# davnords/octic-vits

Measured on AMD Instinct MI355X. Metric: images/sec Hybrid Octic ViT-H/14 224² bf16 train step @1/2/4/8 MI355X, higher is better.
Workload: dtype bf16; 1 GPU; hybrid_deit_huge_patch14 (16 octic + 16 standard blocks, drop_path 0.5) DeiT-III train step: bf16-autocast fwd + bwd + LAMB + EMA, 224x224, batch 64/GPU (BASELINE configs[1]), data parallel over 1 GPU(s); global_batch=64, per_gpu_batch=64, accum_steps=1, parallelism=dp1, library_gemm_table=True, launch=hipGraph replay (whole step)

## Files before the change

include/octic_hip.h:

```cpp
#ifndef OCTIC_HIP_H
#define OCTIC_HIP_H

#include <stdint.h>

#ifdef __cplusplus
extern "C" {
#endif

#define OCTIC_ABI_VERSION 20

enum { OCTIC_F32 = 0, OCTIC_BF16 = 1, OCTIC_U8 = 2  };

enum {
  OCTIC_OK = 0,
  OCTIC_ESHAPE = -1,
  OCTIC_EALIGN = -2,
  OCTIC_EDTYPE = -3,
  OCTIC_ENULL = -4,
  OCTIC_EWORKSPACE = -5
};

typedef struct {
  void* ptr[5];
  int64_t ld[5];
} octic_view;

int octic_abi_version(void);
const char* octic_strerror(int code);

enum {
  OCTIC_ROUTE_DENSE_TILE = 0,
  OCTIC_ROUTE_DENSE_SPLIT = 1,
  OCTIC_ROUTE_WGRAD_SLABS = 2,
  OCTIC_ROUTE_WGRAD_TILE = 3,
  OCTIC_ROUTE_LINEAR_RING = 4,
  OCTIC_ROUTE_RING_EVEN = 5,
  OCTIC_ROUTE_ATTN_LEGACY = 6,
  OCTIC_ROUTE_ATTN_ONLINE = 7,
  OCTIC_ROUTE_ATTN_BWD_PAIR = 8,
  OCTIC_ROUTE_DENSE_IMAGE = 9,
  OCTIC_ROUTE_DENSE_CLS2 = 10,
  OCTIC_ROUTE_ATTN_STREAM = 11,
  OCTIC_ROUTE_COUNT = 12
};
int octic_route_override(int knob, int value);

int octic_gelu_d8_fwd(const octic_view* x, const octic_view* y, int64_t M, int c, int dtype, void* stream);
int octic_gelu_d8_bwd(const octic_view* g, const octic_view* x, const octic_view* gin, int64_t M, int c,
                      int dtype, void* stream);
int octic_gelu_d8_fwd_skip(const octic_view* x, const octic_view* y, int64_t M, int c, int dtype,
                           const float* sample_scale, int64_t rows_per_sample, void* stream);
int octic_gelu_d8_bwd_skip(const octic_view* g, const octic_view* x, const octic_view* gin, int64_t M, int c, int dtype,
                           const float* sample_scale, int64_t rows_per_sample, void* stream);

int octic_layernorm_d8_fwd(const octic_view* x, const octic_view* y, const float* const alpha[5],
                           const float* beta, float* stats, int64_t M, int c, float eps, int out_dtype,
                           void* stream);
int octic_layernorm_d8_bwd_blocks(int64_t M);
int octic_layernorm_d8_bwd(const octic_view* g, const octic_view* x, const float* stats,
                           const float* const alpha[5], const octic_view* dres, const octic_view* dx,
                           float* partials, int64_t M, int c, int g_dtype, void* stream);
int octic_layernorm_d8_bwd_cast(const octic_view* g, const octic_view* x, const float* stats, const float* const alpha[5],
                                const octic_view* dres, const octic_view* dx, float* partials, int64_t M, int c,
                                const float* rs, int64_t rows_per_sample, void* gcast, void* stream);
int octic_layernorm_d8_bwd_skip(const octic_view* g, const octic_view* x, const float* stats, const float* const alpha[5],
                                const octic_view* dres, const octic_view* dx, float* partials, int64_t M, int c, int g_dtype,
                                const float* sample_scale, int64_t rows_per_sample, void* stream);
int octic_layernorm_d8_bwd_cast_skip(const octic_view* g, const octic_view* x, const float* stats,
                                     const float* const alpha[5], const octic_view* dres, const octic_view* dx,
                                     float* partials, int64_t M, int c, const float* rs, int64_t rows_per_scale, void* gcast,
                                     const float* sample_scale, int64_t rows_per_sample, void* stream);
int octic_layernorm_d8_bwd_finish(const float* partials, int nblk, int c, float* const dalpha[5], float* dbeta,
                                  void* stream);
typedef struct octic_ln_finish_job {
  const float* partials;
  float* dalpha[5];
  float* dbeta;
  int nblk;
  int c;
} octic_ln_finish_job;
int octic_layernorm_d8_bwd_finish_batch(const octic_ln_finish_job* jobs, int njobs, void* stream);

int octic_sample_blocks(const void* src, void* dst, const int64_t* idx, int64_t n, int64_t block_bytes, int scatter,
                        void* stream);

int octic_linear_d8_fwd(const octic_view* x, const void* const w[5], const float* bias, const octic_view* y,
                        const octic_view* resid, const float* rs, int64_t rows_per_sample,
                        const float* const cs[5], int64_t M, int cin, int cout, int dtype, int out_dtype,
                        void* stream);
int octic_linear_d8_fwd_skip(const octic_view* x, const void* const w[5], const float* bias, const octic_view* y,
                             const octic_view* resid, const float* rs, int64_t rows_per_sample,
                             const float* const cs[5], int64_t M, int cin, int cout, int dtype, int out_dtype,
                             const float* sample_scale, int64_t skip_rows_per_sample, void* stream);
int octic_linear_d8_fwd_dropped(const octic_view* x, const void* const w[5], const float* bias, const octic_view* y,
                                const octic_view* resid, const float* rs, int64_t rows_per_sample,
                                const float* const cs[5], int64_t M, int cin, int cout, int dtype, int out_dtype,
                                const float* dropped, int64_t dropped_rows_per_sample, void* stream);

int octic_linear_d8_prep(const float* const w32[5], const float* const cs[5], int cin, int cout, void* wb, void* wt,
                         int dtype, void* stream);
typedef struct octic_prep_item {
  const float* w[5];
  const float* cs[5];
  void* wb;
  void* wt;
  int32_t cin, cout;
  int32_t block_begin, block_count;
} octic_prep_item;
int octic_linear_d8_prep_batch_blocks(int cin, int cout);
int octic_linear_d8_prep_batch(const octic_prep_item* items_dev, int n_items, int total_blocks, int dtype, void* stream);

int octic_linear_d8_tile_n(int64_t M, int cin, int cout);
enum {
  OCTIC_LINEAR_WREG = 0,
  OCTIC_LINEAR_RING = 1,
  OCTIC_LINEAR_CLASSIC = 2
};
int octic_linear_d8_plan(int64_t M, int cin, int cout, int dtype, int out_dtype, int fused, int out[4]);
int octic_linear_d8_ring_order(int ngroups, const int* items, const int* ksteps, int slots_per_xcd, int* out_group,
                               int* out_item);
int octic_linear_d8_ring_order_dropped(int ngroups, const int* items, const int* ksteps, int slots_per_xcd, const int* n_chunks,
                                       const unsigned char* dead_long, const unsigned char* dead_short, int* out_group,
                                       int* out_item, int* out_dead);

int octic_linear_d8_wgrad_has_colsum(int cin, int cout, int dtype);
enum {
  OCTIC_WGRAD_RING = 0,
  OCTIC_WGRAD_TILED = 1
};
int octic_linear_d8_wgrad_plan(int64_t M, int cin, int cout, int dtype, int out[4]);
int64_t octic_linear_d8_wgrad_workspace_bytes(int cin, int cout, int splits);
int octic_linear_d8_wgrad_splits(int64_t M, int cin, int cout);
int octic_linear_d8_wgrad_tile(int64_t M, int cin, int cout);
int octic_linear_d8_wgrad(const octic_view* x, const octic_view* dy, int64_t M, int cin, int cout, int dtype,
                          float* workspace, int splits, void* stream);
int octic_linear_d8_wgrad_finish(const float* workspace, int splits, int cin, int cout,
                                 const float* const w32[5], const float* const cs[5], const float* bias,
                                 const float* dysum, float* const dw[5], float* const dcs[5], float* dbias,
                                 void* stream);
typedef struct octic_wgrad_finish_job {
  const float* workspace;
  const float* w32[5];
  const float* cs[5];
  const float* bias;
  const float* dysum;
  float* dw[5];
  float* dcs[5];
  float* dbias;
  int splits, cin, cout, has_cs;
} octic_wgrad_finish_job;
int octic_linear_d8_wgrad_finish_batch(const octic_wgrad_finish_job* jobs, int njobs, void* stream);

int octic_colsum_blocks(int64_t M);
int octic_colsum_a1(const octic_view* dy, int64_t M, int c, int dtype, float* partials, float* out, void* stream);
// ... 17 lines not shown
int octic_attn_fwd_f32(const void* q, const void* k, const void* v, void* o, float* lse, int64_t B, int H, int T, int hd,
                       int64_t sB, int64_t sH, int64_t sT, int64_t oB, int64_t oH, int64_t oT, float scale, void* stream);
int octic_attn_bwd_f32(const void* q, const void* k, const void* v, const void* o, const void* dout, const float* lse,
                       float* delta, void* dq, void* dk, void* dv, int64_t B, int H, int T, int hd, int64_t sB, int64_t sH,
                       int64_t sT, int64_t oB, int64_t oH, int64_t oT, int64_t gB, int64_t gH, int64_t gT, float scale,
                       int phase, void* stream);

int octic_attn_fwd_packed(const void* qkv, void* o, float* lse, int64_t B, int H, int T, int c, int64_t ld_qkv,
                          int64_t ld_o, float scale, void* stream);
int octic_attn_bwd_packed(const void* qkv, const void* o, const void* dout, const float* lse, float* delta, void* dqkv,
                          int64_t B, int H, int T, int c, int64_t ld_qkv, int64_t ld_o, int64_t ld_g, float scale,
                          int phase, void* stream);

enum {
  OCTIC_ATTN_FWD_PERSIST = 0,
  OCTIC_ATTN_FWD_A80_ONESHOT = 1,
  OCTIC_ATTN_FWD_A80_ONLINE = 2,
  OCTIC_ATTN_FWD_RESIDENT = 3,
  OCTIC_ATTN_FWD_STREAM = 4,
  OCTIC_ATTN_FWD_F32 = 5
};
enum {
  OCTIC_ATTN_BWD_SINGLE = 0,
  OCTIC_ATTN_BWD_PAIR = 1,
  OCTIC_ATTN_BWD_STREAM = 2,
  OCTIC_ATTN_BWD_F32 = 3
};
int octic_attn_plan(int dtype, int T, int hd, int64_t ld_in, int64_t ld_out, int64_t ld_grad, int out[4]);
int octic_attn_skip_plan(int dtype, int T, int hd, int64_t ld_in, int64_t ld_out, int64_t ld_grad, int out[4]);

int octic_attn_fwd_skip(const void* q, const void* k, const void* v, void* o, float* lse, int64_t B, int H, int T, int hd,
                        int64_t sB, int64_t sH, int64_t sT, int64_t oB, int64_t oH, int64_t oT, float scale,
                        const float* sample_scale, void* stream);
int octic_attn_bwd_skip(const void* q, const void* k, const void* v, const void* o, const void* dout, const float* lse,
                        float* delta, void* dq, void* dk, void* dv, int64_t B, int H, int T, int hd, int64_t sB, int64_t sH,
                        int64_t sT, int64_t oB, int64_t oH, int64_t oT, int64_t gB, int64_t gH, int64_t gT, float scale,
                        int phase, const float* sample_scale, void* stream);
int octic_attn_fwd_packed_skip(const void* qkv, void* o, float* lse, int64_t B, int H, int T, int c, int64_t ld_qkv,
                               int64_t ld_o, float scale, const float* sample_scale, void* stream);
int octic_attn_bwd_packed_skip(const void* qkv, const void* o, const void* dout, const float* lse, float* delta, void* dqkv,
                               int64_t B, int H, int T, int c, int64_t ld_qkv, int64_t ld_o, int64_t ld_g, float scale,
                               int phase, const float* sample_scale, void* stream);

int octic_handoff_cat_fwd(const octic_view* x, void* dense, int64_t M, int c, int out_dtype, void* stream);
int octic_handoff_cat_bwd(const float* ddense, const octic_view* dx, int64_t M, int c, void* stream);
int octic_power_spectrum_fwd(const octic_view* x, void* dense, int64_t M, int c, int out_dtype, void* stream);
int octic_power_spectrum_bwd(const float* ddense, const octic_view* x, const octic_view* dx, int64_t M, int c,
                             void* stream);

int octic_im2col_patches(const float* img, void* patches, int64_t B, int Cin, int Himg, int Wimg, int p,
                         int Kpad, int dtype, void* stream);
int octic_lift_gemm(const void* patches, const void* w, const float* bias, const float* pos, float* out,
                    int64_t B, int64_t n_patches, int tok0, int Kpad, int D, int dtype, void* stream);
int64_t octic_lift_wgrad_workspace_bytes(int Kpad, int D, int splits);
int octic_lift_wgrad(const void* patches, const void* dout, float* dw, float* workspace, int splits, int64_t rows,
                     int Kpad, int D, int dtype, void* stream);

int64_t octic_lamb_workspace_floats(int ntensors, int nchunks);
int octic_lamb_step(void* const* p, void* const* g, void* const* m, void* const* v, void* const* ema, const float* wd,
                    const int* chunk_tensor, const int64_t* chunk_off, const int* chunk_len,
                    const int* tensor_chunk_begin, int ntensors, int nchunks, float* workspace, float lr, float beta1,
                    float beta2, float eps, float max_grad_norm, int step, float ema_decay, void* const* bf16_shadow,
                    void* stream);
int octic_adamw_step(void* const* p, void* const* g, void* const* m, void* const* v, void* const* ema, const float* wd,
                     const int* chunk_tensor, const int64_t* chunk_off, const int* chunk_len,
                     const int* tensor_chunk_begin, int ntensors, int nchunks, float* workspace, float lr, float beta1,
                     float beta2, float eps, float max_grad_norm, int step, float ema_decay, void* const* bf16_shadow,
                     void* stream);
int octic_lamb_step_hp(void* const* p, void* const* g, void* const* m, void* const* v, void* const* ema, const float* wd,
                       const int* chunk_tensor, const int64_t* chunk_off, const int* chunk_len,
                       const int* tensor_chunk_begin, int ntensors, int nchunks, float* workspace, const float* lr,
                       float beta1, float beta2, float eps, float max_grad_norm, int step, const float* ema_decay,
                       void* const* bf16_shadow, void* stream);
int octic_adamw_step_hp(void* const* p, void* const* g, void* const* m, void* const* v, void* const* ema, const float* wd,
                        const int* chunk_tensor, const int64_t* chunk_off, const int* chunk_len,
                        const int* tensor_chunk_begin, int ntensors, int nchunks, float* workspace, const float* lr,
                        float beta1, float beta2, float eps, float max_grad_norm, int step, const float* ema_decay,
                        void* const* bf16_shadow, void* stream);

int octic_dense_blocks(int64_t rows);
int octic_dense_resid_layernorm_fwd(const float* x, const void* yb, int yb_dtype, const float* gamma, const float* rs,
                                    int64_t rows_per_scale, float* xout, void* y, int y_dtype, const float* w,
                                    const float* b, float* stats, int64_t rows, int d, float eps, void* stream);
int octic_dense_layernorm_fwd(const float* x, void* y, int y_dtype, const float* w, const float* b, float* stats,
                              int64_t rows, int d, float eps, void* stream);
int octic_dense_layernorm_bwd(const void* gy, int g_dtype, const float* x, const float* w, const float* stats,
                              const float* dres, float* dx, float* partials, int64_t rows, int d, void* stream);
int octic_dense_finish(const float* partials, int nblocks, int d, float* out0, float* out1, const float* scale1,
                       void* stream);
typedef struct octic_finish_job {
  const float* partials;
  float* out0;
  float* out1;
  const float* scale1;
  int nblocks;
  int d;
} octic_finish_job;
int octic_dense_finish_batch(const octic_finish_job* jobs, int njobs, void* stream);
int octic_dense_layernorm_bwd_tail(const void* gy, const float* x, const float* w, const float* stats, const float* dres,
                                   float* dx, float* partials, const void* yb, const float* gamma, const float* rs,
                                   int64_t rows_per_scale, void* gyb, float* partials2, int64_t rows, int d, void* stream);
int octic_dense_layernorm_bwd_tail_skip(const void* gy, const float* x, const float* w, const float* stats,
                                        const float* dres, float* dx, float* partials, const void* yb, const float* gamma,
                                        const float* rs, int64_t rows_per_scale, void* gyb, float* partials2, int64_t rows,
                                        int d, const float* sample_scale, int64_t rows_per_sample, void* stream);
int octic_dense_gelu_blocks(void);
int octic_dense_gelu_bwd(const void* h, const void* g, void* dh, float* partials, int64_t rows, int d, void* stream);
int octic_dense_colsum(const void* g, int64_t rows, int d, int64_t ld, float* partials, void* stream);
int octic_dense_colsum_skip(const void* g, int64_t rows, int d, int64_t ld, float* partials, const float* sample_scale,
                            int64_t rows_per_sample, void* stream);
int octic_swiglu_blocks(void);
int octic_swiglu_fwd(const void* x12, int64_t ld12, void* a, int64_t lda, int64_t rows, int H, void* stream);
int octic_swiglu_bwd(const void* x12, int64_t ld12, const void* ga, int64_t ldg, void* dx12, int64_t ldd, float* partials,
                     int64_t rows, int H, void* stream);
int octic_scale_residual_fwd(const float* x, const void* y, int y_dtype, const float* gamma, const float* rs,
                             int64_t rows_per_scale, float* out, int64_t rows, int d, void* stream);
int octic_scale_residual_bwd(const float* gout, const void* y, int y_dtype, const float* gamma, const float* rs,
                             int64_t rows_per_scale, void* gy, float* partials, int64_t rows, int d, void* stream);

int octic_dense_layernorm_fwd_rows(const float* x, void* y, int y_dtype, const float* w, const float* b, float* stats,
                                   int64_t rows, int d, float eps, const int* rowmap, float* xcopy, void* stream);
int octic_dense_layernorm_bwd_rows(const void* gy, int g_dtype, const float* x, const float* w, const float* stats,
                                   const float* dres, float* dx, float* partials, int64_t rows, int d, const int* rowmap,
                                   void* stream);
int octic_scale_residual_fwd_rows(const float* x, const void* y, int y_dtype, const float* gamma, const float* rs,
                                  int64_t rows_per_scale, float* out, int64_t rows, int d, const int* rowmap, void* stream);
int octic_scale_residual_bwd_rows(const float* gout, const void* y, int y_dtype, const float* gamma, const float* rs,
                                  int64_t rows_per_scale, void* gy, float* partials, int64_t rows, int d, const int* rowmap,
                                  void* stream);

typedef struct octic_dense_prep_item {
  const void* src;
  void* wb;
  void* wt;
  int32_t N, K;
  int32_t block_begin, pad;
} octic_dense_prep_item;
int octic_dense_prep_batch_blocks(int N, int K);
int octic_dense_prep_batch(const octic_dense_prep_item* items_dev, int n_items, int total_blocks, int src_dtype, void* stream);

int64_t octic_dense_gemm_workspace_bytes(int M, int N, int K);
int octic_dense_gemm_colsum_rows(int M, int N, int K);
int octic_dense_gemm_tile(int M, int N, int K, int mode);
int octic_dense_gemm_nt(const void* A, const void* B, int M, int N, int K, int64_t lda, int64_t ldb, int mode, void* C,
                        void* C2, int64_t ldc, const float* bias, const float* gamma, const float* rs,
                        int64_t rows_per_sample, const float* X, float* OUT, const void* H, float* colsum,
                        void* workspace, void* stream);
int octic_dense_gemm_nt_tokens(const void* A, const void* B, int M, int N, int K, int64_t lda, int64_t ldb, int mode, void* C,
                               void* C2, int64_t ldc, const float* bias, const float* gamma, const float* rs,
                               int64_t rows_per_sample, const float* X, float* OUT, const void* H, float* colsum,
                               void* workspace, int tokens, void* stream);
int octic_dense_gemm_plan(int M, int N, int K, int mode, int tokens, int* out4);
int octic_dense_gemm_nt_tokens_skip(const void* A, const void* B, int M, int N, int K, int64_t lda, int64_t ldb, int mode, void* C,
                                    void* C2, int64_t ldc, const float* bias, const float* gamma, const float* rs,
                                    int64_t rows_per_sample_rs, const float* X, float* OUT, const void* H, float* colsum,
                                    const float* sample_scale, int rows_per_sample, void* workspace, int tokens,
                                    void* stream);
int octic_dense_gemm_plan_dropped(int M, int N, int K, int mode, int tokens, int rows_per_sample, int* out4);
int octic_dense_gemm_order_dropped(int M, int N, int K, int mode, int tokens, const float* sample_scale, int rows_per_sample,
                                   int cap, int* out_tm, int* out_tn, int* out_part, int* out_split, int* out_dead);
int octic_dense_gemm_nt_tokens_adaptive(const void* A, const void* B, int M, int N, int K, int64_t lda, int64_t ldb, int mode,
                                        void* C, void* C2, int64_t ldc, const float* bias, const float* gamma, const float* rs,
                                        int64_t rows_per_sample_rs, const float* X, float* OUT, const void* H, float* colsum,
                                        const float* sample_scale, int rows_per_sample, void* workspace, int tokens,
                                        void* stream);
int octic_dense_gemm_plan_adaptive(int M, int N, int K, int mode, int tokens, int rows_per_sample, int* out5);
int octic_dense_gemm_order_adaptive(int M, int N, int K, int mode, int tokens, const float* sample_scale, int rows_per_sample,
                                    int cap, int* out_tm, int* out_tn, int* out_dead, int* out_width);
int octic_dense_gemm_nt_tokens_adaptive_cls(const void* A, const void* B, int M, int N, int K, int64_t lda, int64_t ldb, int mode,
                                            void* C, void* C2, int64_t ldc, const float* bias, const float* gamma, const float* rs,
                                            int64_t rows_per_sample_rs, const float* X, float* OUT, const void* H, float* colsum,
                                            const float* sample_scale, int rows_per_sample, void* workspace, int tokens,
                                            int fold_cls, void* stream);
int octic_dense_gemm_plan_adaptive_cls(int M, int N, int K, int mode, int tokens, int rows_per_sample, int* out5);
int octic_dense_gemm_order_adaptive_cls(int M, int N, int K, int mode, int tokens, const float* sample_scale, int rows_per_sample,
                                        int cap, int* out_tm, int* out_tn, int* out_dead, int* out_width, int cls_cap,
                                        int* out_cls_rt, int* out_cls_ct);

int octic_dense_gemm_nt_tokens_image(const void* A, const void* B, int M, int N, int K, int64_t lda, int64_t ldb, int mode,
                                     void* C, void* C2, int64_t ldc, const float* bias, const float* gamma, const float* rs,
                                     int64_t rows_per_sample_rs, const float* X, float* OUT, const void* H, float* colsum,
                                     const float* sample_scale, int rows_per_sample, void* workspace, int tokens,
                                     int fold_cls, double drop, void* stream);
int octic_dense_gemm_plan_image(int M, int N, int K, int mode, int tokens, int rows_per_sample, int masked, double drop, int* out8);
int octic_dense_gemm_order_image(int M, int N, int K, int mode, int tokens, const float* sample_scale, int rows_per_sample, double drop,
                                 int cap, int* out_tm, int* out_tn, int* out_dead, int cls_cap, int* out_cls_rt, int* out_cls_ct);

int64_t octic_dense_wgrad_workspace_bytes(int M, int N, int K);
// ... 190 lines not shown
```

octic_vits_amd/_lib.py:

```python
import ctypes
import os
import re

HERE = os.path.dirname(os.path.abspath(__file__))
LIB_PATH = os.environ.get("OCTIC_LIB") or os.path.join(HERE, "liboctic_hip.so")
HEADER_PATH = os.path.join(HERE, "..", "include", "octic_hip.h")

F32, BF16, U8 = 0, 1, 2
ABI_VERSION = 20
(ROUTE_DENSE_TILE, ROUTE_DENSE_SPLIT, ROUTE_WGRAD_SLABS, ROUTE_WGRAD_TILE, ROUTE_LINEAR_RING, ROUTE_RING_EVEN,
 ROUTE_ATTN_LEGACY, ROUTE_ATTN_ONLINE, ROUTE_ATTN_BWD_PAIR, ROUTE_DENSE_IMAGE, ROUTE_DENSE_CLS2, ROUTE_ATTN_STREAM) = range(12)

DENSE_ADAPT_WIDE, DENSE_ADAPT_NARROW = 16, 32
DENSE_IMAGE_ALWAYS, DENSE_IMAGE_CLS_APART, DENSE_IMAGE_NEVER = 4, 8, 16

(ATTN_FWD_PERSIST, ATTN_FWD_A80_ONESHOT, ATTN_FWD_A80_ONLINE, ATTN_FWD_RESIDENT, ATTN_FWD_STREAM, ATTN_FWD_F32) = range(6)
ATTN_BWD_SINGLE, ATTN_BWD_PAIR, ATTN_BWD_STREAM, ATTN_BWD_F32 = range(4)
LINEAR_WREG, LINEAR_RING, LINEAR_CLASSIC = range(3)
WGRAD_RING, WGRAD_TILED = range(2)
DENSE_F32_NT, DENSE_F32_NN, DENSE_F32_TN = range(3)

c_i64, c_int, c_float, c_void_p = ctypes.c_int64, ctypes.c_int, ctypes.c_float, ctypes.c_void_p
c_double = ctypes.c_double


class OcticView(ctypes.Structure):
    _fields_ = [("ptr", c_void_p * 5), ("ld", c_i64 * 5)]


PtrArray5 = c_void_p * 5
VP = ctypes.POINTER(OcticView)

_PROTOS = {
    "octic_abi_version": (c_int, []),
    "octic_strerror": (ctypes.c_char_p, [c_int]),
    "octic_route_override": (c_int, [c_int, c_int]),
    "octic_gelu_d8_fwd": (c_int, [VP, VP, c_i64, c_int, c_int, c_void_p]),
    "octic_gelu_d8_bwd": (c_int, [VP, VP, VP, c_i64, c_int, c_int, c_void_p]),
    "octic_gelu_d8_fwd_skip": (c_int, [VP, VP, c_i64, c_int, c_int, c_void_p, c_i64, c_void_p]),
    "octic_gelu_d8_bwd_skip": (c_int, [VP, VP, VP, c_i64, c_int, c_int, c_void_p, c_i64, c_void_p]),
    "octic_layernorm_d8_fwd": (c_int, [VP, VP, c_void_p, c_void_p, c_void_p, c_i64, c_int, c_float, c_int, c_void_p]),
    "octic_layernorm_d8_bwd_blocks": (c_int, [c_i64]),
    "octic_layernorm_d8_bwd": (c_int, [VP, VP, c_void_p, c_void_p, VP, VP, c_void_p, c_i64, c_int, c_int, c_void_p]),
    "octic_layernorm_d8_bwd_cast": (c_int, [VP, VP, c_void_p, c_void_p, VP, VP, c_void_p, c_i64, c_int, c_void_p, c_i64,
                                            c_void_p, c_void_p]),
    "octic_layernorm_d8_bwd_skip": (c_int, [VP, VP, c_void_p, c_void_p, VP, VP, c_void_p, c_i64, c_int, c_int, c_void_p, c_i64,
                                            c_void_p]),
    "octic_layernorm_d8_bwd_cast_skip": (c_int, [VP, VP, c_void_p, c_void_p, VP, VP, c_void_p, c_i64, c_int, c_void_p, c_i64,
                                                 c_void_p, c_void_p, c_i64, c_void_p]),
    "octic_layernorm_d8_bwd_finish": (c_int, [c_void_p, c_int, c_int, c_void_p, c_void_p, c_void_p]),
    "octic_layernorm_d8_bwd_finish_batch": (c_int, [c_void_p, c_int, c_void_p]),
    "octic_sample_blocks": (c_int, [c_void_p, c_void_p, c_void_p, c_i64, c_i64, c_int, c_void_p]),
    "octic_linear_d8_fwd": (c_int, [VP, c_void_p, c_void_p, VP, VP, c_void_p, c_i64, c_void_p, c_i64, c_int, c_int,
                                    c_int, c_int, c_void_p]),
    "octic_linear_d8_fwd_skip": (c_int, [VP, c_void_p, c_void_p, VP, VP, c_void_p, c_i64, c_void_p, c_i64, c_int, c_int,
                                         c_int, c_int, c_void_p, c_i64, c_void_p]),
    "octic_linear_d8_fwd_dropped": (c_int, [VP, c_void_p, c_void_p, VP, VP, c_void_p, c_i64, c_void_p, c_i64, c_int, c_int,
                                            c_int, c_int, c_void_p, c_i64, c_void_p]),
    "octic_linear_d8_tile_n": (c_int, [c_i64, c_int, c_int]),
    "octic_linear_d8_plan": (c_int, [c_i64, c_int, c_int, c_int, c_int, c_int, ctypes.POINTER(c_int)]),
    "octic_linear_d8_ring_order": (c_int, [c_void_p, c_void_p, c_void_p, c_int, c_void_p, c_void_p]),
    "octic_linear_d8_ring_order_dropped": (c_int, [c_int, c_void_p, c_void_p, c_int, c_void_p, c_void_p, c_void_p, c_void_p,
                                                   c_void_p, c_void_p]),
    "octic_linear_d8_wgrad_tile": (c_int, [c_i64, c_int, c_int]),
    "octic_linear_d8_wgrad_workspace_bytes": (c_i64, [c_int, c_int, c_int]),
    "octic_linear_d8_wgrad_splits": (c_int, [c_i64, c_int, c_int]),
    "octic_linear_d8_wgrad": (c_int, [VP, VP, c_i64, c_int, c_int, c_int, c_void_p, c_int, c_void_p]),
    "octic_linear_d8_wgrad_finish": (c_int, [c_void_p, c_int, c_int, c_int, c_void_p, c_void_p, c_void_p, c_void_p,
                                             c_void_p, c_void_p, c_void_p, c_void_p]),
    "octic_linear_d8_wgrad_finish_batch": (c_int, [c_void_p, c_int, c_void_p]),
    "octic_linear_d8_wgrad_has_colsum": (c_int, [c_int, c_int, c_int]),
    "octic_linear_d8_wgrad_plan": (c_int, [c_i64, c_int, c_int, c_int, ctypes.POINTER(c_int)]),
    "octic_lamb_workspace_floats": (c_i64, [c_int, c_int]),
    "octic_lamb_step": (c_int, [c_void_p] * 10 + [c_int, c_int, c_void_p, c_float, c_float, c_float, c_float, c_float,
                                                  c_int, c_float, c_void_p, c_void_p]),
    "octic_adamw_step": (c_int, [c_void_p] * 10 + [c_int, c_int, c_void_p, c_float, c_float, c_float, c_float, c_float,
                                                   c_int, c_float, c_void_p, c_void_p]),
    "octic_lamb_step_hp": (c_int, [c_void_p] * 10 + [c_int, c_int, c_void_p, c_void_p, c_float, c_float, c_float, c_float,
                                                     c_int, c_void_p, c_void_p, c_void_p]),
    "octic_adamw_step_hp": (c_int, [c_void_p] * 10 + [c_int, c_int, c_void_p, c_void_p, c_float, c_float, c_float, c_float,
                                                      c_int, c_void_p, c_void_p, c_void_p]),
    "octic_dense_blocks": (c_int, [c_i64]),
    "octic_dense_layernorm_fwd": (c_int, [c_void_p, c_void_p, c_int, c_void_p, c_void_p, c_void_p, c_i64, c_int,
                                          c_float, c_void_p]),
    "octic_dense_resid_layernorm_fwd": (c_int, [c_void_p, c_void_p, c_int, c_void_p, c_void_p, c_i64, c_void_p, c_void_p, c_int,
                                                c_void_p, c_void_p, c_void_p, c_i64, c_int, c_float, c_void_p]),
    "octic_dense_layernorm_bwd": (c_int, [c_void_p, c_int, c_void_p, c_void_p, c_void_p, c_void_p, c_void_p, c_void_p,
                                          c_i64, c_int, c_void_p]),
    "octic_dense_layernorm_bwd_tail": (c_int, [c_void_p] * 10 + [c_i64, c_void_p, c_void_p, c_i64, c_int, c_void_p]),
    "octic_dense_layernorm_bwd_tail_skip": (c_int, [c_void_p] * 10 + [c_i64, c_void_p, c_void_p, c_i64, c_int, c_void_p, c_i64,
                                                                      c_void_p]),
    "octic_dense_finish": (c_int, [c_void_p, c_int, c_int, c_void_p, c_void_p, c_void_p, c_void_p]),
    "octic_dense_finish_batch": (c_int, [c_void_p, c_int, c_void_p]),
    "octic_dense_gelu_blocks": (c_int, []),
    "octic_dense_gelu_bwd": (c_int, [c_void_p, c_void_p, c_void_p, c_void_p, c_i64, c_int, c_void_p]),
    "octic_swiglu_blocks": (c_int, []),
    "octic_swiglu_fwd": (c_int, [c_void_p, c_i64, c_void_p, c_i64, c_i64, c_int, c_void_p]),
    "octic_swiglu_bwd": (c_int, [c_void_p, c_i64, c_void_p, c_i64, c_void_p, c_i64, c_void_p, c_i64, c_int, c_void_p]),
    "octic_dense_layernorm_fwd_rows": (c_int, [c_void_p, c_void_p, c_int, c_void_p, c_void_p, c_void_p, c_i64, c_int, c_float,
                                               c_void_p, c_void_p, c_void_p]),
    "octic_dense_layernorm_bwd_rows": (c_int, [c_void_p, c_int, c_void_p, c_void_p, c_void_p, c_void_p, c_void_p, c_void_p, c_i64,
                                               c_int, c_void_p, c_void_p]),
    "octic_scale_residual_fwd_rows": (c_int, [c_void_p, c_void_p, c_int, c_void_p, c_void_p, c_i64, c_void_p, c_i64, c_int,
                                              c_void_p, c_void_p]),
    "octic_scale_residual_bwd_rows": (c_int, [c_void_p, c_void_p, c_int, c_void_p, c_void_p, c_i64, c_void_p, c_void_p, c_i64,
                                              c_int, c_void_p, c_void_p]),
    "octic_softmax_center": (c_int, [c_void_p, c_int, c_i64, c_void_p, c_float, c_void_p, c_i64, c_int, c_void_p]),
    "octic_soft_ce_fwd": (c_int, [c_void_p, c_int, c_i64, c_void_p, c_i64, c_float, c_void_p, c_void_p, c_void_p, c_i64, c_int,
                                  c_void_p]),
    "octic_soft_ce_bwd": (c_int, [c_void_p, c_int, c_i64, c_void_p, c_i64, c_float, c_void_p, c_void_p, c_void_p, c_void_p, c_i64,
                                  c_i64, c_int, c_void_p]),
    "octic_sinkhorn_slabs": (c_int, [c_i64]),
    "octic_sinkhorn_protos": (c_int, [c_void_p, c_int, c_i64, c_float, c_void_p, c_void_p, c_void_p, c_void_p, c_i64, c_int,
                                      c_void_p]),
    "octic_sinkhorn_rows": (c_int, [c_void_p, c_int, c_i64, c_float, c_void_p, c_void_p, c_void_p, c_i64, c_int, c_void_p]),
    "octic_sinkhorn_final": (c_int, [c_void_p, c_int, c_i64, c_float, c_void_p, c_void_p, c_i64, c_int, c_void_p]),
    "octic_scale_residual_fwd": (c_int, [c_void_p, c_void_p, c_int, c_void_p, c_void_p, c_i64, c_void_p, c_i64, c_int,
                                         c_void_p]),
    "octic_scale_residual_bwd": (c_int, [c_void_p, c_void_p, c_int, c_void_p, c_void_p, c_i64, c_void_p, c_void_p,
                                         c_i64, c_int, c_void_p]),
    "octic_colsum_blocks": (c_int, [c_i64]),
    "octic_colsum_a1": (c_int, [VP, c_i64, c_int, c_int, c_void_p, c_void_p, c_void_p]),
    "octic_cast_rowscale": (c_int, [VP, VP, c_void_p, c_i64, c_i64, c_int, c_int, c_void_p]),
    "octic_linear_d8_prep": (c_int, [c_void_p, c_void_p, c_int, c_int, c_void_p, c_void_p, c_int, c_void_p]),
    "octic_linear_d8_prep_batch_blocks": (c_int, [c_int, c_int]),
    "octic_linear_d8_prep_batch": (c_int, [c_void_p, c_int, c_int, c_int, c_void_p]),
    "octic_attn_fwd": (c_int, [c_void_p, c_void_p, c_void_p, c_void_p, c_void_p, c_i64, c_int, c_int, c_int,
                               c_i64, c_i64, c_i64, c_i64, c_i64, c_i64, c_float, c_void_p]),
    "octic_attn_fwd_packed": (c_int, [c_void_p] * 3 + [c_i64, c_int, c_int, c_int, c_i64, c_i64, c_float, c_void_p]),
    "octic_attn_bwd_packed": (c_int, [c_void_p] * 6 + [c_i64, c_int, c_int, c_int, c_i64, c_i64, c_i64, c_float, c_int, c_void_p]),
    "octic_attn_bwd": (c_int, [c_void_p] * 10 + [c_i64, c_int, c_int, c_int] + [c_i64] * 9 + [c_float, c_int, c_void_p]),
    "octic_attn_fwd_skip": (c_int, [c_void_p] * 5 + [c_i64, c_int, c_int, c_int] + [c_i64] * 6 + [c_float, c_void_p, c_void_p]),
    "octic_attn_bwd_skip": (c_int, [c_void_p] * 10 + [c_i64, c_int, c_int, c_int] + [c_i64] * 9 + [c_float, c_int, c_void_p, c_void_p]),
    "octic_attn_fwd_packed_skip": (c_int, [c_void_p] * 3 + [c_i64, c_int, c_int, c_int, c_i64, c_i64, c_float, c_void_p, c_void_p]),
    "octic_attn_bwd_packed_skip": (c_int, [c_void_p] * 6 + [c_i64, c_int, c_int, c_int, c_i64, c_i64, c_i64, c_float, c_int, c_void_p, c_void_p]),
    "octic_attn_fwd_f32": (c_int, [c_void_p] * 5 + [c_i64, c_int, c_int, c_int] + [c_i64] * 6 + [c_float, c_void_p]),
    "octic_attn_bwd_f32": (c_int, [c_void_p] * 10 + [c_i64, c_int, c_int, c_int] + [c_i64] * 9 + [c_float, c_int, c_void_p]),
    "octic_attn_plan": (c_int, [c_int, c_int, c_int, c_i64, c_i64, c_i64, ctypes.POINTER(c_int)]),
    "octic_attn_skip_plan": (c_int, [c_int, c_int, c_int, c_i64, c_i64, c_i64, ctypes.POINTER(c_int)]),
    "octic_attn_pack_heads": (c_int, [VP, c_void_p, c_i64, c_i64, c_int, c_int, c_int, c_int, c_void_p]),
    "octic_attn_unpack_heads": (c_int, [c_void_p, VP, c_i64, c_i64, c_int, c_int, c_int, c_int, c_void_p]),
    "octic_handoff_cat_fwd": (c_int, [VP, c_void_p, c_i64, c_int, c_int, c_void_p]),
    "octic_handoff_cat_bwd": (c_int, [c_void_p, VP, c_i64, c_int, c_void_p]),
    "octic_power_spectrum_fwd": (c_int, [VP, c_void_p, c_i64, c_int, c_int, c_void_p]),
    "octic_power_spectrum_bwd": (c_int, [c_void_p, VP, VP, c_i64, c_int, c_void_p]),
    "octic_im2col_patches": (c_int, [c_void_p, c_void_p, c_i64, c_int, c_int, c_int, c_int, c_int, c_int, c_void_p]),
    "octic_lift_gemm": (c_int, [c_void_p, c_void_p, c_void_p, c_void_p, c_void_p, c_i64, c_i64, c_int, c_int, c_int,
                                c_int, c_void_p]),
    "octic_lift_wgrad_workspace_bytes": (c_i64, [c_int, c_int, c_int]),
    "octic_lift_wgrad": (c_int, [c_void_p, c_void_p, c_void_p, c_void_p, c_int, c_i64, c_int, c_int, c_int, c_void_p]),
    "octic_dense_prep_batch_blocks": (c_int, [c_int, c_int]),
    "octic_dense_prep_batch": (c_int, [c_void_p, c_int, c_int, c_int, c_void_p]),
    "octic_dense_gemm_workspace_bytes": (c_i64, [c_int, c_int, c_int]),
    "octic_dense_gemm_colsum_rows": (c_int, [c_int, c_int, c_int]),
    "octic_dense_gemm_tile": (c_int, [c_int, c_int, c_int, c_int]),
    "octic_dense_gemm_nt": (c_int, [c_void_p, c_void_p, c_int, c_int, c_int, c_i64, c_i64, c_int, c_void_p, c_void_p, c_i64,
                                    c_void_p, c_void_p, c_void_p, c_i64, c_void_p, c_void_p, c_void_p, c_void_p, c_void_p,
                                    c_void_p]),
    "octic_dense_gemm_nt_tokens": (c_int, [c_void_p, c_void_p, c_int, c_int, c_int, c_i64, c_i64, c_int, c_void_p, c_void_p,
                                           c_i64, c_void_p, c_void_p, c_void_p, c_i64, c_void_p, c_void_p, c_void_p, c_void_p,
                                           c_void_p, c_int, c_void_p]),
    "octic_dense_gemm_plan": (c_int, [c_int, c_int, c_int, c_int, c_int, ctypes.POINTER(c_int)]),
    "octic_dense_gemm_nt_tokens_skip": (c_int, [c_void_p, c_void_p, c_int, c_int, c_int, c_i64, c_i64, c_int, c_void_p, c_void_p,
                                                c_i64, c_void_p, c_void_p, c_void_p, c_i64, c_void_p, c_void_p, c_void_p, c_void_p,
                                                c_void_p, c_int, c_void_p, c_int, c_void_p]),
    "octic_dense_gemm_plan_dropped": (c_int, [c_int, c_int, c_int, c_int, c_int, c_int, ctypes.POINTER(c_int)]),
    "octic_dense_gemm_order_dropped": (c_int, [c_int, c_int, c_int, c_int, c_int, c_void_p, c_int, c_int, c_void_p, c_void_p,
                                               c_void_p, c_void_p, c_void_p]),
    "octic_dense_gemm_nt_tokens_adaptive": (c_int, [c_void_p, c_void_p, c_int, c_int, c_int, c_i64, c_i64, c_int, c_void_p, c_void_p,
                                                    c_i64, c_void_p, c_void_p, c_void_p, c_i64, c_void_p, c_void_p, c_void_p,
                                                    c_void_p, c_void_p, c_int, c_void_p, c_int, c_void_p]),
    "octic_dense_gemm_plan_adaptive": (c_int, [c_int, c_int, c_int, c_int, c_int, c_int, ctypes.POINTER(c_int)]),
    "octic_dense_gemm_order_adaptive": (c_int, [c_int, c_int, c_int, c_int, c_int, c_void_p, c_int, c_int, c_void_p, c_void_p,
                                                c_void_p, c_void_p]),
# ... 168 lines not shown
```

octic_vits_amd/csrc/dense.hip:

```cpp
#include "octic_common.hpp"

namespace octic {

constexpr int kDenseWaves = 16;
constexpr int kDenseMaxBlocks = 256;

template <typename T> struct Row4;
template <> struct Row4<float> {
  typedef f32x4 vec;
  static __device__ inline f32x4 load(const float* p) { return *(const f32x4*)p; }
  static __device__ inline f32x4 load_raw(const float* p) { return *(const f32x4*)p; }
  static __device__ inline f32x4 widen(f32x4 v) { return v; }
  static __device__ inline void store(float* p, f32x4 v) { *(f32x4*)p = v; }
};
template <> struct Row4<bf16> {
  typedef bf16x4 vec;
  static __device__ inline f32x4 load(const bf16* p) {
    bf16x4 h = *(const bf16x4*)p;
    return f32x4{(float)h[0], (float)h[1], (float)h[2], (float)h[3]};
  }
  static __device__ inline bf16x4 load_raw(const bf16* p) { return *(const bf16x4*)p; }
  static __device__ inline f32x4 widen(bf16x4 h) { return f32x4{(float)h[0], (float)h[1], (float)h[2], (float)h[3]}; }
  static __device__ inline void store(bf16* p, f32x4 v) {
    *(bf16x4*)p = bf16x4{(bf16)v[0], (bf16)v[1], (bf16)v[2], (bf16)v[3]};
  }
};

__device__ inline float hsum(f32x4 v) { return (v[0] + v[1]) + (v[2] + v[3]); }

template <typename TOUT, int NV>
__global__ __launch_bounds__(256) void dense_ln_fwd_kernel(const float* __restrict__ x, TOUT* __restrict__ y,
                                                           const float* __restrict__ w, const float* __restrict__ b,
                                                           float* __restrict__ stats, long rows, int d, float eps,
                                                           const int* __restrict__ rowmap = nullptr,
                                                           float* __restrict__ xcopy = nullptr) {
  const int lane = threadIdx.x & 63;
  const long nw = (long)gridDim.x * 4;
  f32x4 wv[NV], bv[NV];
  bool ok[NV];
#pragma unroll
  for (int i = 0; i < NV; ++i) {
    const int col = (i * 64 + lane) * 4;
    ok[i] = col < d;
    wv[i] = (ok[i] && w) ? *(const f32x4*)(w + col) : f32x4{1.f, 1.f, 1.f, 1.f};
    bv[i] = (ok[i] && b) ? *(const f32x4*)(b + col) : f32x4{0.f, 0.f, 0.f, 0.f};
  }
  const float inv_d = 1.0f / (float)d;
  for (long r = (long)blockIdx.x * 4 + (threadIdx.x >> 6); r < rows; r += nw) {
    const float* xr = x + (rowmap ? (long)rowmap[r] : r) * d;
    f32x4 xv[NV];
    float s = 0.f;
#pragma unroll
    for (int i = 0; i < NV; ++i) {
      xv[i] = ok[i] ? *(const f32x4*)(xr + (i * 64 + lane) * 4) : f32x4{0.f, 0.f, 0.f, 0.f};
      s += hsum(xv[i]);
    }
    if (xcopy) {
#pragma unroll
      for (int i = 0; i < NV; ++i)
        if (ok[i]) *(f32x4*)(xcopy + r * d + (i * 64 + lane) * 4) = xv[i];
    }
    const float mean = wave_total(s) * inv_d;
    float q = 0.f;
#pragma unroll
    for (int i = 0; i < NV; ++i) {
      f32x4 c = xv[i] - mean;
      xv[i] = c;
      if (ok[i]) q += hsum(c * c);
    }
    const float rstd = rsqrtf(wave_total(q) * inv_d + eps);
    TOUT* yr = y + r * d;
#pragma unroll
    for (int i = 0; i < NV; ++i)
      if (ok[i]) Row4<TOUT>::store(yr + (i * 64 + lane) * 4, xv[i] * rstd * wv[i] + bv[i]);
    if (lane == 0) {
      stats[2 * r] = mean;
      stats[2 * r + 1] = rstd;
    }
  }
}

template <typename TY, typename TOUT, int NV>
__global__ __launch_bounds__(256) void dense_resid_ln_fwd_kernel(const float* __restrict__ x, const TY* __restrict__ yb,
                                                                 const float* __restrict__ gamma, const float* __restrict__ rs,
                                                                 long rps, float* __restrict__ xout, TOUT* __restrict__ y,
                                                                 const float* __restrict__ w, const float* __restrict__ b,
                                                                 float* __restrict__ stats, long rows, int d, float eps) {
  const int lane = threadIdx.x & 63;
  const long nw = (long)gridDim.x * 4;
  f32x4 wv[NV], bv[NV], gm[NV];
  bool ok[NV];
#pragma unroll
  for (int i = 0; i < NV; ++i) {
    const int col = (i * 64 + lane) * 4;
    ok[i] = col < d;
    wv[i] = (ok[i] && w) ? *(const f32x4*)(w + col) : f32x4{1.f, 1.f, 1.f, 1.f};
    bv[i] = (ok[i] && b) ? *(const f32x4*)(b + col) : f32x4{0.f, 0.f, 0.f, 0.f};
    gm[i] = (ok[i] && gamma) ? *(const f32x4*)(gamma + col) : f32x4{1.f, 1.f, 1.f, 1.f};
  }
  const float inv_d = 1.0f / (float)d;
  for (long r = (long)blockIdx.x * 4 + (threadIdx.x >> 6); r < rows; r += nw) {
    const float* xr = x + r * d;
    const TY* yr_in = yb + r * d;
    float* xo = xout + r * d;
    f32x4 xv[NV];
    float s = 0.f;
    const float rsv = rs ? rs[r / rps] : 1.f;
    if (NV <= 6 && d == NV * 256) {
      typename Row4<TY>::vec yv[NV];
#pragma unroll
      for (int i = 0; i < NV; ++i) xv[i] = *(const f32x4*)(xr + (i * 64 + lane) * 4);
#pragma unroll
      for (int i = 0; i < NV; ++i) yv[i] = Row4<TY>::load_raw(yr_in + (i * 64 + lane) * 4);
#pragma unroll
      for (int i = 0; i < NV; ++i) {
        f32x4 sc = gm[i];
        if (rs) sc *= rsv;
        xv[i] = xv[i] + sc * Row4<TY>::widen(yv[i]);
        *(f32x4*)(xo + (i * 64 + lane) * 4) = xv[i];
        s += hsum(xv[i]);
      }
    } else {
#pragma unroll
      for (int i = 0; i < NV; ++i) {
        xv[i] = f32x4{0.f, 0.f, 0.f, 0.f};
        if (ok[i]) {
          const int col = (i * 64 + lane) * 4;
          f32x4 sc = gm[i];
          if (rs) sc *= rsv;
          xv[i] = *(const f32x4*)(xr + col) + sc * Row4<TY>::load(yr_in + col);
          *(f32x4*)(xo + col) = xv[i];
        }
        s += hsum(xv[i]);
      }
    }
    const float mean = wave_total(s) * inv_d;
    float q = 0.f;
#pragma unroll
    for (int i = 0; i < NV; ++i) {
      f32x4 c = xv[i] - mean;
      xv[i] = c;
      if (ok[i]) q += hsum(c * c);
    }
    const float rstd = rsqrtf(wave_total(q) * inv_d + eps);
    TOUT* yr = y + r * d;
#pragma unroll
    for (int i = 0; i < NV; ++i)
      if (ok[i]) Row4<TOUT>::store(yr + (i * 64 + lane) * 4, xv[i] * rstd * wv[i] + bv[i]);
    if (lane == 0) {
      stats[2 * r] = mean;
      stats[2 * r + 1] = rstd;
    }
  }
}

template <int NV>
__device__ inline void slab_reduce(float* lds, float* slab, const f32x4 (&p0)[NV], const f32x4 (&p1)[NV],
                                   const bool (&ok)[NV], int d) {
  const int lane = threadIdx.x & 63, wave = threadIdx.x >> 6, nwaves = blockDim.x >> 6;
  for (int wv = 0; wv < nwaves; ++wv) {
    if (wave == wv) {
#pragma unroll
      for (int i = 0; i < NV; ++i)
        if (ok[i]) {
          const int col = (i * 64 + lane) * 4;
          f32x4* a = (f32x4*)(lds + col);
          f32x4* c = (f32x4*)(lds + d + col);
          if (wv == 0) {
            *a = p0[i];
            *c = p1[i];
          } else {
            *a += p0[i];
            *c += p1[i];
          }
        }
    }
    __syncthreads();
  }
  for (int j = threadIdx.x * 4; j < 2 * d; j += blockDim.x * 4) *(f32x4*)(slab + j) = *(const f32x4*)(lds + j);
}

template <typename TG, int NV>
__global__ __launch_bounds__(kDenseWaves * 64, 4) void dense_ln_bwd_kernel(
    const TG* __restrict__ gy, const float* __restrict__ x, const float* __restrict__ w,
    const float* __restrict__ stats, const float* __restrict__ dres, float* __restrict__ dx,
    float* __restrict__ partials, long rows, int d, const int* __restrict__ rowmap = nullptr) {
  extern __shared__ float lds[];
  const int lane = threadIdx.x & 63;
  const long nw = (long)gridDim.x * kDenseWaves;
  float* wl = lds + 2 * d;
  for (int j = threadIdx.x; j < d; j += kDenseWaves * 64) wl[j] = w ? w[j] : 1.f;
  f32x4 pw[NV], pb[NV];
  bool ok[NV];
#pragma unroll
  for (int i = 0; i < NV; ++i) {
    ok[i] = (i * 64 + lane) * 4 < d;
    pw[i] = pb[i] = f32x4{0.f, 0.f, 0.f, 0.f};
  }
  __syncthreads();
  const float inv_d = 1.0f / (float)d;
  for (long r = (long)blockIdx.x * kDenseWaves + (threadIdx.x >> 6); r < rows; r += nw) {
    const float mean = stats[2 * r], rstd = stats[2 * r + 1];
    f32x4 xh[NV], g[NV];
    float s1 = 0.f, s2 = 0.f;
#pragma unroll
    for (int i = 0; i < NV; ++i) {
      const long o = r * d + (i * 64 + lane) * 4;
      if (ok[i]) {
        xh[i] = (*(const f32x4*)(x + o) - mean) * rstd;
        f32x4 gyv = Row4<TG>::load(gy + o);
        pw[i] += gyv * xh[i];
        pb[i] += gyv;
        g[i] = gyv * *(const f32x4*)(wl + (i * 64 + lane) * 4);
        s1 += hsum(g[i]);
        s2 += hsum(g[i] * xh[i]);
      }
    }
    const float m1 = wave_total(s1) * inv_d, m2 = wave_total(s2) * inv_d;
#pragma unroll
    for (int i = 0; i < NV; ++i)
      if (ok[i]) {
        const long o = (rowmap ? (long)rowmap[r] : r) * d + (i * 64 + lane) * 4;
        f32x4 v = (g[i] - m1 - xh[i] * m2) * rstd;
        if (dres) v += *(const f32x4*)(dres + o);
        *(f32x4*)(dx + o) = v;
      }
  }
  if (partials) slab_reduce<NV>(lds, partials + (long)blockIdx.x * 2 * d, pw, pb, ok, d);
}

template <typename TG, int NV>
#ifndef OCTIC_DLNBWD_WAVES
#define OCTIC_DLNBWD_WAVES 8
#endif
__global__ __launch_bounds__(OCTIC_DLNBWD_WAVES * 64, OCTIC_DLNBWD_WAVES / 4) void dense_ln_bwd_wide_kernel(
    const TG* __restrict__ gy, const float* __restrict__ x, const float* __restrict__ w,
    const float* __restrict__ stats, const float* __restrict__ dres, float* __restrict__ dx,
    float* __restrict__ partials, long rows, int d, const int* __restrict__ rowmap = nullptr) {
  extern __shared__ float lds[];
  const int lane = threadIdx.x & 63, nwaves = blockDim.x >> 6;
  const long nw = (long)gridDim.x * nwaves;
  float* wl = lds + 2 * d;
  for (int j = threadIdx.x; j < d; j += blockDim.x) wl[j] = w ? w[j] : 1.f;
  f32x4 pw[NV], pb[NV];
  bool ok[NV];
#pragma unroll
  for (int i = 0; i < NV; ++i) {
    ok[i] = true;
    pw[i] = pb[i] = f32x4{0.f, 0.f, 0.f, 0.f};
  }
  __syncthreads();
  const float inv_d = 1.0f / (float)d;
  for (long r = (long)blockIdx.x * nwaves + (threadIdx.x >> 6); r < rows; r += nw) {
    const long o = r * d + lane * 4;
    const long om = (rowmap ? (long)rowmap[r] : r) * d + lane * 4;
    f32x4 xh[NV], g[NV], dr[NV];
    typename Row4<TG>::vec gr[NV];
#pragma unroll
    for (int i = 0; i < NV; ++i) xh[i] = *(const f32x4*)(x + o + i * 256);
#pragma unroll
    for (int i = 0; i < NV; ++i) gr[i] = Row4<TG>::load_raw(gy + o + i * 256);
#pragma unroll
    for (int i = 0; i < NV; ++i) dr[i] = dres ? *(const f32x4*)(dres + om + i * 256) : f32x4{0.f, 0.f, 0.f, 0.f};
    const float mean = stats[2 * r], rstd = stats[2 * r + 1];
    float s1 = 0.f, s2 = 0.f;
#pragma unroll
    for (int i = 0; i < NV; ++i) {
      xh[i] = (xh[i] - mean) * rstd;
      const f32x4 gyv = Row4<TG>::widen(gr[i]);
      pw[i] += gyv * xh[i];
      pb[i] += gyv;
      g[i] = gyv * *(const f32x4*)(wl + (i * 64 + lane) * 4);
      s1 += hsum(g[i]);
      s2 += hsum(g[i] * xh[i]);
    }
    const float m1 = wave_total(s1) * inv_d, m2 = wave_total(s2) * inv_d;
#pragma unroll
    for (int i = 0; i < NV; ++i) {
      f32x4 v = (g[i] - m1 - xh[i] * m2) * rstd;
      if (dres) v += dr[i];
      *(f32x4*)(dx + om + i * 256) = v;
    }
  }
  if (partials) slab_reduce<NV>(lds, partials + (long)blockIdx.x * 2 * d, pw, pb, ok, d);
}

template <typename TG, int NV, bool SKIP = false, typename... MASK>
__global__ __launch_bounds__(512, 2) void dense_ln_bwd_tail_kernel(
    const TG* __restrict__ gy, const float* __restrict__ x, const float* __restrict__ w,
    const float* __restrict__ stats, const float* __restrict__ dres, float* __restrict__ dx,
    float* __restrict__ partials, const TG* __restrict__ yb, const float* __restrict__ gamma,
    const float* __restrict__ rs, long rps, TG* __restrict__ gyb, float* __restrict__ partials2, long rows, int d,
    MASK... mask) {
  extern __shared__ float lds[];
  const float* __restrict__ ns = mask_scale(mask...);
  const long nrps = mask_rows(mask...);
  const int lane = threadIdx.x & 63, nwaves = blockDim.x >> 6;
  const long nw = (long)gridDim.x * nwaves;
  float* wl = lds + 2 * d;
  float* gl = lds + 3 * d;
  for (int j = threadIdx.x; j < d; j += blockDim.x) {
    wl[j] = w ? w[j] : 1.f;
    gl[j] = gamma ? gamma[j] : 1.f;
  }
  f32x4 pw[NV], pb[NV], p0[NV], p1[NV];
  bool ok[NV];
#pragma unroll
  for (int i = 0; i < NV; ++i) {
    ok[i] = true;
    pw[i] = pb[i] = p0[i] = p1[i] = f32x4{0.f, 0.f, 0.f, 0.f};
  }
  __syncthreads();
  const float inv_d = 1.0f / (float)d;
  for (long r = (long)blockIdx.x * nwaves + (threadIdx.x >> 6); r < rows; r += nw) {
    const long o = r * d + lane * 4;
    f32x4 xh[NV], g[NV], dr[NV];
    typename Row4<TG>::vec gr[NV], yr[NV];
    float mean = 0.f, rstd = 0.f, sc = 1.f;
    bool live = true, tail = true;
    if constexpr (SKIP) {
      sc = rs ? rs[r / rps] : 1.f;
      live = mask_live(ns[r / nrps]);
      tail = mask_live(sc);
    }
    if (live) {
#pragma unroll
      for (int i = 0; i < NV; ++i) xh[i] = *(const f32x4*)(x + o + i * 256);
#pragma unroll
      for (int i = 0; i < NV; ++i) gr[i] = Row4<TG>::load_raw(gy + o + i * 256);
    } else {
#pragma unroll
      for (int i = 0; i < NV; ++i) {
        xh[i] = f32x4{0.f, 0.f, 0.f, 0.f};
        gr[i] = typename Row4<TG>::vec{};
      }
    }
#pragma unroll
    for (int i = 0; i < NV; ++i) dr[i] = dres ? *(const f32x4*)(dres + o + i * 256) : f32x4{0.f, 0.f, 0.f, 0.f};
    if (tail) {
#pragma unroll
      for (int i = 0; i < NV; ++i) yr[i] = Row4<TG>::load_raw(yb + o + i * 256);
    } else {
#pragma unroll
      for (int i = 0; i < NV; ++i) yr[i] = typename Row4<TG>::vec{};
    }
    if (live) {
      mean = stats[2 * r];
      rstd = stats[2 * r + 1];
    }
    if constexpr (!SKIP) sc = rs ? rs[r / rps] : 1.f;
    float s1 = 0.f, s2 = 0.f;
#pragma unroll
    for (int i = 0; i < NV; ++i) {
      xh[i] = (xh[i] - mean) * rstd;
      const f32x4 gyv = Row4<TG>::widen(gr[i]);
      pw[i] += gyv * xh[i];
      pb[i] += gyv;
      g[i] = gyv * *(const f32x4*)(wl + (i * 64 + lane) * 4);
      s1 += hsum(g[i]);
      s2 += hsum(g[i] * xh[i]);
    }
    const float m1 = wave_total(s1) * inv_d, m2 = wave_total(s2) * inv_d;
#pragma unroll
    for (int i = 0; i < NV; ++i) {
      f32x4 v = (g[i] - m1 - xh[i] * m2) * rstd;
      if (dres) v += dr[i];
      *(f32x4*)(dx + o + i * 256) = v;
      const f32x4 t = v * sc;
      p1[i] += t;
      p0[i] += t * Row4<TG>::widen(yr[i]);
      Row4<TG>::store(gyb + o + i * 256, t * *(const f32x4*)(gl + (i * 64 + lane) * 4));
    }
  }
  if (partials) slab_reduce<NV>(lds, partials + (long)blockIdx.x * 2 * d, pw, pb, ok, d);
  __syncthreads();
  if (partials2) slab_reduce<NV>(lds, partials2 + (long)blockIdx.x * 2 * d, p0, p1, ok, d);
}

template <typename TY>
__global__ __launch_bounds__(256) void scale_residual_fwd_kernel(const float* __restrict__ x, const TY* __restrict__ y,
                                                                 const float* __restrict__ gamma,
                                                                 const float* __restrict__ rs, long rps,
                                                                 float* __restrict__ out, long rows, int d,
                                                                 const int* __restrict__ rowmap = nullptr) {
  const int d4 = d >> 2;
  const long n4 = rows * d4;
  for (long i = (long)blockIdx.x * blockDim.x + threadIdx.x; i < n4; i += (long)gridDim.x * blockDim.x) {
    const long r = i / d4;
    const int col = (int)(i - r * d4) * 4;
    f32x4 s = gamma ? *(const f32x4*)(gamma + col) : f32x4{1.f, 1.f, 1.f, 1.f};
    if (rs) s *= rs[r / rps];
    const long io = rowmap ? (long)rowmap[r] * d + col : i * 4;
    *(f32x4*)(out + io) = *(const f32x4*)(x + i * 4) + s * Row4<TY>::load(y + i * 4);
  }
}

template <typename TY, int NV>
__global__ __launch_bounds__(kDenseWaves * 64) void scale_residual_bwd_kernel(
    const float* __restrict__ gout, const TY* __restrict__ y, const float* __restrict__ gamma,
    const float* __restrict__ rs, long rps, TY* __restrict__ gy, float* __restrict__ partials, long rows, int d,
    const int* __restrict__ rowmap = nullptr) {
  extern __shared__ float lds[];
  const int lane = threadIdx.x & 63;
  const long nw = (long)gridDim.x * kDenseWaves;
  f32x4 gm[NV], p0[NV], p1[NV];
  bool ok[NV];
#pragma unroll
  for (int i = 0; i < NV; ++i) {
    const int col = (i * 64 + lane) * 4;
    ok[i] = col < d;
    gm[i] = (ok[i] && gamma) ? *(const f32x4*)(gamma + col) : f32x4{1.f, 1.f, 1.f, 1.f};
    p0[i] = p1[i] = f32x4{0.f, 0.f, 0.f, 0.f};
  }
  if (NV <= 5 && d == NV * 256 && partials) {
    for (long r = (long)blockIdx.x * kDenseWaves + (threadIdx.x >> 6); r < rows; r += nw) {
      const float s = rs ? rs[r / rps] : 1.f;
      const long o = r * d + lane * 4;
      const long og = (rowmap ? (long)rowmap[r] : r) * d + lane * 4;
      f32x4 g[NV];
      typename Row4<TY>::vec yv[NV];
#pragma unroll
      for (int i = 0; i < NV; ++i) g[i] = *(const f32x4*)(gout + og + i * 256);
#pragma unroll
      for (int i = 0; i < NV; ++i) yv[i] = Row4<TY>::load_raw(y + o + i * 256);
#pragma unroll
      for (int i = 0; i < NV; ++i) {
        g[i] *= s;
        p1[i] += g[i];
        p0[i] += g[i] * Row4<TY>::widen(yv[i]);
        Row4<TY>::store(gy + o + i * 256, g[i] * gm[i]);
      }
    }
  } else {
    for (long r = (long)blockIdx.x * kDenseWaves + (threadIdx.x >> 6); r < rows; r += nw) {
      const float s = rs ? rs[r / rps] : 1.f;
#pragma unroll
      for (int i = 0; i < NV; ++i)
        if (ok[i]) {
          const long o = r * d + (i * 64 + lane) * 4;
          f32x4 g = *(const f32x4*)(gout + (rowmap ? (long)rowmap[r] : r) * d + (i * 64 + lane) * 4) * s;
          p1[i] += g;
          if (partials) p0[i] += g * Row4<TY>::load(y + o);
          Row4<TY>::store(gy + o, g * gm[i]);
        }
    }
  }
  if (partials) slab_reduce<NV>(lds, partials + (long)blockIdx.x * 2 * d, p0, p1, ok, d);
}

__global__ __launch_bounds__(256) void dense_finish_kernel(const float* __restrict__ partials, int nblocks, int d,
                                                           float* __restrict__ out0, float* __restrict__ out1,
                                                           const float* __restrict__ scale1) {
  __shared__ float red[16][17];
  const int cx = threadIdx.x & 15, gy = threadIdx.x >> 4;
// ... 159 lines not shown
  switch (nv) {                   \
    case 1: { constexpr int NV = 1; CALL; } break; \
    case 2: { constexpr int NV = 2; CALL; } break; \
    case 3: { constexpr int NV = 3; CALL; } break; \
    case 4: { constexpr int NV = 4; CALL; } break; \
    case 5: { constexpr int NV = 5; CALL; } break; \
    case 6: { constexpr int NV = 6; CALL; } break; \
    case 7: { constexpr int NV = 7; CALL; } break; \
    default: { constexpr int NV = 8; CALL; } break; \
  }

template <typename TS>
__global__ __launch_bounds__(256) void dense_prep_batch_kernel(const octic_dense_prep_item* __restrict__ items, int n_items) {
  __shared__ float tile[64][65];
  const int b = blockIdx.x;
  int cnt = 0;
  for (int i0 = 0; i0 < n_items; i0 += 256) {
    const int i = i0 + (int)threadIdx.x;
    cnt += __syncthreads_count(i < n_items && b >= items[i].block_begin);
  }
  const int it = cnt > 0 ? cnt - 1 : 0;
  const octic_dense_prep_item& I = items[it];
  const int N = I.N, K = I.K;
  const int lt = b - I.block_begin;
  const int kt = (K + 63) / 64;
  const int n0 = (lt / kt) * 64, k0 = (lt % kt) * 64;
  const TS* w = (const TS*)I.src;
  bf16* wb = (bf16*)I.wb;
  bf16* wt = (bf16*)I.wt;
  const bool vec = (N % 8) == 0 && (K % 8) == 0;
  if (vec) {
    const int c8 = (threadIdx.x & 7) * 8, r = threadIdx.x >> 3;
#pragma unroll
    for (int h = 0; h < 2; ++h) {
      const int n = n0 + r + 32 * h, k = k0 + c8;
      float v[8] = {0, 0, 0, 0, 0, 0, 0, 0};
      if (n < N && k < K) {
        load8<TS>(w + (int64_t)n * K + k, v);
        if (wb) store8<bf16>(wb + (int64_t)n * K + k, v);
      }
#pragma unroll
      for (int e = 0; e < 8; ++e) tile[r + 32 * h][c8 + e] = v[e];
    }
    __syncthreads();
    if (wt) {
#pragma unroll
      for (int h = 0; h < 2; ++h) {
        const int k = k0 + r + 32 * h, n = n0 + c8;
        if (k < K && n < N) {
          float v[8];
#pragma unroll
          for (int e = 0; e < 8; ++e) v[e] = tile[c8 + e][r + 32 * h];
          store8<bf16>(wt + (int64_t)k * N + n, v);
        }
      }
    }
    return;
  }
  const int tx = threadIdx.x & 63, ty = threadIdx.x >> 6;
#pragma unroll 4
  for (int r = ty; r < 64; r += 4) {
    const int n = n0 + r, k = k0 + tx;
    float v = 0.f;
    if (n < N && k < K) {
      v = (float)w[(int64_t)n * K + k];
      if (wb) wb[(int64_t)n * K + k] = (bf16)v;
    }
    tile[r][tx] = v;
  }
  __syncthreads();
  if (wt) {
#pragma unroll 4
    for (int r = ty; r < 64; r += 4) {
      const int k = k0 + r, n = n0 + tx;
      if (k < K && n < N) wt[(int64_t)k * N + n] = (bf16)tile[tx][r];
    }
  }
}

}

using namespace octic;

extern "C" {

int octic_dense_layernorm_fwd(const float* x, void* y, int y_dtype, const float* w, const float* b, float* stats,
                              int64_t rows, int d, float eps, void* stream) {
  return octic_dense_layernorm_fwd_rows(x, y, y_dtype, w, b, stats, rows, d, eps, nullptr, nullptr, stream);
}

int octic_dense_layernorm_fwd_rows(const float* x, void* y, int y_dtype, const float* w, const float* b, float* stats,
                                   int64_t rows, int d, float eps, const int* rowmap, float* xcopy, void* stream) {
  if (rows == 0) return OCTIC_OK;
  if (!x || !y || !stats) return OCTIC_ENULL;
  if (int e = dense_check(rows, d)) return e;
  if (y_dtype != OCTIC_F32 && y_dtype != OCTIC_BF16) return OCTIC_EDTYPE;
  long blocks = (rows + 15) / 16;
  if (blocks > 4096) blocks = 4096;
  hipStream_t s = (hipStream_t)stream;
  if (y_dtype == OCTIC_BF16) {
    DENSE_NV_SWITCH(dense_nv(d), (dense_ln_fwd_kernel<bf16, NV><<<dim3((unsigned)blocks), dim3(256), 0, s>>>(x, (bf16*)y, w, b, stats, rows, d, eps, rowmap, xcopy)));
  } else {
    DENSE_NV_SWITCH(dense_nv(d), (dense_ln_fwd_kernel<float, NV><<<dim3((unsigned)blocks), dim3(256), 0, s>>>(x, (float*)y, w, b, stats, rows, d, eps, rowmap, xcopy)));
  }
  return launch_status();
}

int octic_dense_resid_layernorm_fwd(const float* x, const void* yb, int yb_dtype, const float* gamma, const float* rs,
                                    int64_t rows_per_scale, float* xout, void* y, int y_dtype, const float* w,
                                    const float* b, float* stats, int64_t rows, int d, float eps, void* stream) {
  if (rows == 0) return OCTIC_OK;
  if (!x || !yb || !xout || !y || !stats) return OCTIC_ENULL;
  if (int e = dense_check(rows, d)) return e;
  if ((yb_dtype != OCTIC_F32 && yb_dtype != OCTIC_BF16) || (y_dtype != OCTIC_F32 && y_dtype != OCTIC_BF16)) return OCTIC_EDTYPE;
  if (rs && rows_per_scale <= 0) return OCTIC_ESHAPE;
  long blocks = (rows + 7) / 8;
  if (blocks > 8192) blocks = 8192;
  hipStream_t s = (hipStream_t)stream;
  const long rps = rs ? rows_per_scale : 1;
#define OCTIC_RLN(TYB, TO) \
  DENSE_NV_SWITCH(dense_nv(d), (dense_resid_ln_fwd_kernel<TYB, TO, NV><<<dim3((unsigned)blocks), dim3(256), 0, s>>>( \
      x, (const TYB*)yb, gamma, rs, rps, xout, (TO*)y, w, b, stats, rows, d, eps)))
  if (yb_dtype == OCTIC_BF16 && y_dtype == OCTIC_BF16) { OCTIC_RLN(bf16, bf16); }
  else if (yb_dtype == OCTIC_BF16) { OCTIC_RLN(bf16, float); }
  else if (y_dtype == OCTIC_BF16) { OCTIC_RLN(float, bf16); }
  else { OCTIC_RLN(float, float); }
#undef OCTIC_RLN
  return launch_status();
}

int octic_dense_blocks(int64_t rows) { return dense_blocks(rows); }

int octic_dense_layernorm_bwd(const void* gy, int g_dtype, const float* x, const float* w, const float* stats,
                              const float* dres, float* dx, float* partials, int64_t rows, int d, void* stream) {
  return octic_dense_layernorm_bwd_rows(gy, g_dtype, x, w, stats, dres, dx, partials, rows, d, nullptr, stream);
}

int octic_dense_layernorm_bwd_rows(const void* gy, int g_dtype, const float* x, const float* w, const float* stats,
                                   const float* dres, float* dx, float* partials, int64_t rows, int d, const int* rowmap,
                                   void* stream) {
  if (rows == 0) return OCTIC_OK;
  if (!gy || !x || !stats || !dx) return OCTIC_ENULL;
  if (int e = dense_check(rows, d)) return e;
  if (g_dtype != OCTIC_F32 && g_dtype != OCTIC_BF16) return OCTIC_EDTYPE;
  const int blocks = dense_blocks(rows);
  const size_t lds = (size_t)3 * d * sizeof(float);
  hipStream_t s = (hipStream_t)stream;
  if (d == dense_nv(d) * 256 && dense_nv(d) <= 6) {
    if (g_dtype == OCTIC_BF16) {
      DENSE_NV_SWITCH(dense_nv(d), (dense_ln_bwd_wide_kernel<bf16, NV><<<dim3(blocks), dim3(OCTIC_DLNBWD_WAVES * 64), lds, s>>>((const bf16*)gy, x, w, stats, dres, dx,
                                                            partials, rows, d, rowmap)));
    } else {
      DENSE_NV_SWITCH(dense_nv(d), (dense_ln_bwd_wide_kernel<float, NV><<<dim3(blocks), dim3(OCTIC_DLNBWD_WAVES * 64), lds, s>>>((const float*)gy, x, w, stats, dres, dx,
                                                             partials, rows, d, rowmap)));
    }
    return launch_status();
  }
  if (g_dtype == OCTIC_BF16) {
    DENSE_NV_SWITCH(dense_nv(d), (dense_ln_bwd_kernel<bf16, NV><<<dim3(blocks), dim3(kDenseWaves * 64), lds, s>>>((const bf16*)gy, x, w, stats, dres,
                                                     dx, partials, rows, d, rowmap)));
  } else {
    DENSE_NV_SWITCH(dense_nv(d), (dense_ln_bwd_kernel<float, NV><<<dim3(blocks), dim3(kDenseWaves * 64), lds, s>>>((const float*)gy, x, w, stats,
                                                     dres, dx, partials, rows, d, rowmap)));
  }
  return launch_status();
}

int octic_dense_layernorm_bwd_tail(const void* gy, const float* x, const float* w, const float* stats, const float* dres,
                                   float* dx, float* partials, const void* yb, const float* gamma, const float* rs,
                                   int64_t rows_per_scale, void* gyb, float* partials2, int64_t rows, int d, void* stream) {
  return octic_dense_layernorm_bwd_tail_skip(gy, x, w, stats, dres, dx, partials, yb, gamma, rs, rows_per_scale, gyb,
                                             partials2, rows, d, nullptr, 0, stream);
}

int octic_dense_layernorm_bwd_tail_skip(const void* gy, const float* x, const float* w, const float* stats,
                                        const float* dres, float* dx, float* partials, const void* yb, const float* gamma,
                                        const float* rs, int64_t rows_per_scale, void* gyb, float* partials2, int64_t rows,
                                        int d, const float* sample_scale, int64_t rows_per_sample, void* stream) {
  if (sample_scale && (rows_per_sample <= 0 || rows % rows_per_sample)) return OCTIC_ESHAPE;
  if (rows == 0) return OCTIC_OK;
  if (!gy || !x || !stats || !dx || !yb || !gyb) return OCTIC_ENULL;
  if (int e = dense_check(rows, d)) return e;
  if (d != dense_nv(d) * 256 || dense_nv(d) > 5) return OCTIC_ESHAPE;
  if (rs && rows_per_scale <= 0) return OCTIC_ESHAPE;
  const int blocks = dense_blocks(rows);
  const size_t lds = (size_t)4 * d * sizeof(float);
  hipStream_t s = (hipStream_t)stream;
  const long rps = rs ? rows_per_scale : 1;
  if (sample_scale) {
    DENSE_NV_SWITCH(dense_nv(d), (dense_ln_bwd_tail_kernel<bf16, NV, true><<<dim3(blocks), dim3(512), lds, s>>>(
        (const bf16*)gy, x, w, stats, dres, dx, partials, (const bf16*)yb, gamma, rs, rps, (bf16*)gyb, partials2, rows, d,
        sample_scale, (long)rows_per_sample)));
    return launch_status();
  }
  DENSE_NV_SWITCH(dense_nv(d), (dense_ln_bwd_tail_kernel<bf16, NV><<<dim3(blocks), dim3(512), lds, s>>>(
      (const bf16*)gy, x, w, stats, dres, dx, partials, (const bf16*)yb, gamma, rs, rps, (bf16*)gyb, partials2, rows, d)));
  return launch_status();
}

int octic_dense_finish(const float* partials, int nblocks, int d, float* out0, float* out1, const float* scale1,
                       void* stream) {
  if (!partials) return OCTIC_ENULL;
  if (nblocks <= 0 || d <= 0) return OCTIC_ESHAPE;
  hipLaunchKernelGGL(dense_finish_kernel, dim3((2 * d + 15) / 16), dim3(256), 0, (hipStream_t)stream, partials, nblocks,
                     d, out0, out1, scale1);
  return launch_status();
}

int octic_dense_finish_batch(const octic_finish_job* jobs, int njobs, void* stream) {
  if (!jobs) return OCTIC_ENULL;
  if (njobs < 0) return OCTIC_ESHAPE;
  for (int i = 0; i < njobs; ++i) {
    if (!jobs[i].partials) return OCTIC_ENULL;
    if (jobs[i].nblocks <= 0 || jobs[i].d <= 0) return OCTIC_ESHAPE;
  }
  for (int i0 = 0; i0 < njobs; i0 += 64) {
    const int n = njobs - i0 < 64 ? njobs - i0 : 64;
    FinishPack pack = {};
    int dmax = 0;
    for (int i = 0; i < n; ++i) {
      pack.j[i] = jobs[i0 + i];
      dmax = jobs[i0 + i].d > dmax ? jobs[i0 + i].d : dmax;
    }
    hipLaunchKernelGGL(dense_finish_batch_kernel, dim3((2 * dmax + 15) / 16, n), dim3(256), 0, (hipStream_t)stream, pack);
  }
  return launch_status();
}

int octic_dense_gelu_blocks(void) { return kGeluRowBlocks; }

int octic_dense_colsum(const void* g, int64_t rows, int d, int64_t ld, float* partials, void* stream) {
  return octic_dense_colsum_skip(g, rows, d, ld, partials, nullptr, 0, stream);
}

int octic_dense_colsum_skip(const void* g, int64_t rows, int d, int64_t ld, float* partials, const float* sample_scale,
                            int64_t rows_per_sample, void* stream) {
  if (!g || !partials) return OCTIC_ENULL;
  if (rows <= 0 || d <= 0 || (d & 7) || (ld & 7) || ld < d) return OCTIC_ESHAPE;
  if (sample_scale && (rows_per_sample <= 0 || rows % rows_per_sample)) return OCTIC_ESHAPE;
  if (((uintptr_t)g) & 15) return OCTIC_EALIGN;
  const dim3 grid((d / 8 + 63) / 64, kGeluRowBlocks);
  if (sample_scale && rows < ((int64_t)1 << 32))
    dense_colsum_kernel<true><<<grid, dim3(256), 0, (hipStream_t)stream>>>((const bf16*)g, partials, rows, d, ld,
                                                                           sample_scale, (unsigned)rows_per_sample);
  else
    dense_colsum_kernel<false><<<grid, dim3(256), 0, (hipStream_t)stream>>>((const bf16*)g, partials, rows, d, ld);
  return launch_status();
}

int octic_dense_gelu_bwd(const void* h, const void* g, void* dh, float* partials, int64_t rows, int d, void* stream) {
  if (rows == 0) return OCTIC_OK;
  if (!h || !g || !dh) return OCTIC_ENULL;
  if (rows < 0 || d <= 0 || (d & 7)) return OCTIC_ESHAPE;
  if ((((uintptr_t)h) | ((uintptr_t)g) | ((uintptr_t)dh)) & 15) return OCTIC_EALIGN;
  dense_gelu_bwd_kernel<<<dim3((d / 8 + 63) / 64, kGeluRowBlocks), dim3(256), 0, (hipStream_t)stream>>>(
      (const bf16*)h, (const bf16*)g, (bf16*)dh, partials, rows, d);
  return launch_status();
}

int octic_scale_residual_fwd(const float* x, const void* y, int y_dtype, const float* gamma, const float* rs,
                             int64_t rows_per_scale, float* out, int64_t rows, int d, void* stream) {
  return octic_scale_residual_fwd_rows(x, y, y_dtype, gamma, rs, rows_per_scale, out, rows, d, nullptr, stream);
}

int octic_scale_residual_fwd_rows(const float* x, const void* y, int y_dtype, const float* gamma, const float* rs,
                                  int64_t rows_per_scale, float* out, int64_t rows, int d, const int* rowmap, void* stream) {
  if (rows == 0) return OCTIC_OK;
  if (!x || !y || !out) return OCTIC_ENULL;
  if (int e = dense_check(rows, d)) return e;
  if (y_dtype != OCTIC_F32 && y_dtype != OCTIC_BF16) return OCTIC_EDTYPE;
  if (rs && rows_per_scale <= 0) return OCTIC_ESHAPE;
  const long n4 = rows * (d >> 2);
  long blocks = (n4 + 1023) / 1024;
  if (blocks > 8192) blocks = 8192;
  hipStream_t s = (hipStream_t)stream;
  if (y_dtype == OCTIC_BF16)
    scale_residual_fwd_kernel<bf16><<<dim3((unsigned)blocks), dim3(256), 0, s>>>(x, (const bf16*)y,
                       gamma, rs, rows_per_scale, out, rows, d, rowmap);
  else
    scale_residual_fwd_kernel<float><<<dim3((unsigned)blocks), dim3(256), 0, s>>>(x, (const float*)y,
                       gamma, rs, rows_per_scale, out, rows, d, rowmap);
  return launch_status();
// ... 41 lines not shown
```

octic_vits_amd/csrc/layernorm.hip:

```cpp
#include <stdlib.h>
#include <type_traits>
#include "octic_common.hpp"

namespace octic {

template <typename T>
__device__ inline f32x4 load4(const T* p);
template <>
__device__ inline f32x4 load4<float>(const float* p) { return *(const f32x4*)p; }
template <>
__device__ inline f32x4 load4<bf16>(const bf16* p) {
  bf16x4 a = *(const bf16x4*)p;
  f32x4 r = {(float)a[0], (float)a[1], (float)a[2], (float)a[3]};
  return r;
}
template <typename T>
__device__ inline void store4(T* p, f32x4 v);
template <>
__device__ inline void store4<float>(float* p, f32x4 v) { *(f32x4*)p = v; }
template <>
__device__ inline void store4<bf16>(bf16* p, f32x4 v) {
  bf16x4 a = {(bf16)v[0], (bf16)v[1], (bf16)v[2], (bf16)v[3]};
  *(bf16x4*)p = a;
}
// ... 279 lines not shown
struct LnFinishPack {
  octic_ln_finish_job j[48];
};
__global__ __launch_bounds__(256) void ln_bwd_finish_batch_kernel(LnFinishPack pack) {
  const octic_ln_finish_job& job = pack.j[blockIdx.y];
  if ((int)blockIdx.x * 16 >= 7 * job.c) return;
  ln_bwd_finish_body(job.partials, job.nblk, job.c, job.dalpha[0], job.dalpha[1], job.dalpha[2], job.dalpha[3], job.dalpha[4],
                     job.dbeta);
}

struct LaneGroup {
  bool isE;
  int seg, col0, acol0;
  static constexpr int step4 = 32;
};
__device__ inline LaneGroup lane_group(int lane, int c) {
  LaneGroup lg;
  const int o = lane >> 3, j = lane & 7;
  lg.isE = o >= 4;
  lg.seg = lg.isE ? 4 + ((o - 4) >> 1) : o;
  lg.col0 = o * c + j * 4;
  lg.acol0 = (lg.isE ? (o & 1) * c : 0) + j * 4;
  return lg;
}
__device__ inline const float* pick_alpha(const LaneGroup& lg, const float* a0, const float* a1, const float* a2,
                                          const float* a3, const float* a4) {
  const float* p = a0;
  p = lg.seg == 1 ? a1 : p;
  p = lg.seg == 2 ? a2 : p;
  p = lg.seg == 3 ? a3 : p;
  return lg.seg >= 4 ? a4 : p;
}

template <typename TOUT, int NV>
__global__ __launch_bounds__(256, 4) void ln_fwd_g8_kernel(const float* __restrict__ x, int64_t ldx,
                                                           TOUT* __restrict__ y, int64_t ldy, const float* a0,
                                                           const float* a1, const float* a2, const float* a3,
                                                           const float* a4, const float* beta,
                                                           float* __restrict__ stats, int64_t M, int c, float eps) {
  const int lane = threadIdx.x & 63;
  const int64_t nwaves = (int64_t)gridDim.x * 4;
  const LaneGroup lg = lane_group(lane, c);
  const float* ap = pick_alpha(lg, a0, a1, a2, a3, a4);
  f32x4 av[NV], bv[NV];
#pragma unroll
  for (int i = 0; i < NV; ++i) {
    av[i] = a0 ? *(const f32x4*)(ap + lg.acol0 + i * lg.step4) : f32x4{1.f, 1.f, 1.f, 1.f};
    bv[i] = (beta && lg.seg == 0) ? *(const f32x4*)(beta + lg.acol0 + i * lg.step4) : f32x4{0.f, 0.f, 0.f, 0.f};
  }
  const float inv_n = lg.isE ? 1.0f / (float)(2 * c) : 1.0f / (float)c;
  const float wq = lg.isE ? 0.5f * inv_n : inv_n;
  const int stat_idx = (lg.acol0 == 0) ? lg.seg : (lane == 1 ? 6 : (lane == 2 ? 7 : -1));
  for (int64_t m = (int64_t)blockIdx.x * 4 + (threadIdx.x >> 6); m < M; m += nwaves) {
    const float* xr = x + m * ldx + lg.col0;
    f32x4 xv[NV];
    float s = 0.f;
#pragma unroll
    for (int i = 0; i < NV; ++i) {
      xv[i] = *(const f32x4*)(xr + i * lg.step4);
      s += (xv[i][0] + xv[i][1]) + (xv[i][2] + xv[i][3]);
    }
    const float s8 = sum8(s);
    const float s16 = sum16_from8(s8);
    const float mean = (lg.isE ? s16 : s8) * inv_n;
    float q = 0.f;
#pragma unroll
    for (int i = 0; i < NV; ++i) {
      xv[i] -= mean;
      const f32x4 sq = xv[i] * xv[i];
      q += (sq[0] + sq[1]) + (sq[2] + sq[3]);
    }
    const float S = eps + wave_total(q * wq);
    const float rstd = 1.0f / (kSqrt2Over4 * sqrtf(S));
    TOUT* yr = y + m * ldy + lg.col0;
#pragma unroll
    for (int i = 0; i < NV; ++i) store4<TOUT>(yr + i * lg.step4, xv[i] * rstd * av[i] + bv[i]);
    if (stats && stat_idx >= 0) stats[m * 8 + stat_idx] = (stat_idx == 6) ? rstd : (stat_idx == 7 ? 0.f : mean);
  }
}

#ifndef OCTIC_LNBWD_WIDE
#define OCTIC_LNBWD_WIDE 1
#endif
template <typename TG, int NV, bool WIDE = false, bool SKIP = false, typename... MASK>
__global__ __launch_bounds__(kLnBwdWaves * 64, WIDE ? 2 : OCTIC_LNBWD_OCC) void ln_bwd_g8_kernel(
    const TG* __restrict__ g, int64_t ldg, const float* __restrict__ x, int64_t ldx, const float* __restrict__ stats,
    const float* a0, const float* a1, const float* a2, const float* a3, const float* a4,
    const float* __restrict__ dres, int64_t ldr, float* __restrict__ dx, int64_t ldd, float* __restrict__ partials,
    int64_t M, int c, const float* __restrict__ crs = nullptr, int64_t crps = 1, bf16* __restrict__ cg = nullptr,
    int64_t ldc = 0, MASK... mask) {
  static_assert(WIDE || !SKIP, "the sample mask exists in the wide kernel only");
  const float* __restrict__ ns = mask_scale(mask...);
  const int64_t nrps = mask_rows(mask...);
  extern __shared__ __attribute__((aligned(16))) float smem[];
  const int lane = threadIdx.x & 63, wid = threadIdx.x >> 6;
  const int64_t nwaves = (int64_t)gridDim.x * kLnBwdWaves;
  const int D = 8 * c;
  float* alds = smem + 2 * D;
  float* pbl = smem + 3 * D + wid * c;
  const LaneGroup lg = lane_group(lane, c);
  for (int e = threadIdx.x; e < D; e += kLnBwdWaves * 64) {
    float v = 1.f;
    if (a0) {
      const int sg = e < 4 * c ? e / c : 4;
      const float* ap = sg == 0 ? a0 : (sg == 1 ? a1 : (sg == 2 ? a2 : (sg == 3 ? a3 : a4)));
      v = ap[sg < 4 ? e - sg * c : (e - 4 * c) % (2 * c)];
    }
    alds[e] = v;
  }
  f32x4 pa[NV];
#pragma unroll
  for (int i = 0; i < NV; ++i) {
    pa[i] = f32x4{0.f, 0.f, 0.f, 0.f};
    if (lg.seg == 0) *(f32x4*)(pbl + lg.acol0 + i * 32) = f32x4{0.f, 0.f, 0.f, 0.f};
  }
  __syncthreads();
  const float inv_n = lg.isE ? 1.0f / (float)(2 * c) : 1.0f / (float)c;
  const float coefw = lg.isE ? inv_n : 2.0f * inv_n;
  for (int64_t m = (int64_t)blockIdx.x * kLnBwdWaves + wid; m < M; m += nwaves) {
    bool live = true;
    if constexpr (SKIP) live = mask_live(ns[m / nrps]);
    float mu = 0.f, rstd = 0.f;
    if (live) {
      mu = stats[m * 8 + lg.seg];
      rstd = stats[m * 8 + 6];
    }
    f32x4 xc[NV], gh[NV];
    f32x4 dr[WIDE ? NV : 1];
    typedef typename std::conditional<std::is_same<TG, float>::value, f32x4, bf16x4>::type graw;
    graw gr[WIDE ? NV : 1];
    if constexpr (WIDE) {
      if (live) {
#pragma unroll
        for (int i = 0; i < NV; ++i) xc[i] = *(const f32x4*)(x + m * ldx + lg.col0 + i * lg.step4);
#pragma unroll
        for (int i = 0; i < NV; ++i) gr[i] = *(const graw*)(g + m * ldg + lg.col0 + i * lg.step4);
      } else {
#pragma unroll
        for (int i = 0; i < NV; ++i) {
          xc[i] = f32x4{0.f, 0.f, 0.f, 0.f};
          gr[i] = graw{};
        }
      }
#pragma unroll
      for (int i = 0; i < NV; ++i)
        dr[i] = dres ? *(const f32x4*)(dres + m * ldr + lg.col0 + i * lg.step4) : f32x4{0.f, 0.f, 0.f, 0.f};
    }
    float dot = 0.f, t = 0.f;
#pragma unroll
    for (int i = 0; i < NV; ++i) {
      f32x4 gv;
      if constexpr (WIDE) {
        xc[i] = xc[i] - mu;
        if constexpr (std::is_same<TG, float>::value) gv = gr[i];
        else gv = f32x4{(float)gr[i][0], (float)gr[i][1], (float)gr[i][2], (float)gr[i][3]};
      } else {
        xc[i] = *(const f32x4*)(x + m * ldx + lg.col0 + i * lg.step4) - mu;
        gv = load4<TG>(g + m * ldg + lg.col0 + i * lg.step4);
      }
      const f32x4 xh = xc[i] * rstd;
      gh[i] = *(const f32x4*)(alds + lg.col0 + i * lg.step4) * gv;
      pa[i] += gv * xh;
      if (lg.seg == 0) *(f32x4*)(pbl + lg.acol0 + i * 32) += gv;
      const f32x4 d = gh[i] * xh;
      dot += (d[0] + d[1]) + (d[2] + d[3]);
      t += (gh[i][0] + gh[i][1]) + (gh[i][2] + gh[i][3]);
    }
    const float t8 = sum8(t);
    const float mg = (lg.isE ? sum16_from8(t8) : t8) * inv_n;
    const float dS = -rstd * wave_total(dot) * rstd * (1.0f / 16.0f);
    const float coef = coefw * dS;
#pragma unroll
    for (int i = 0; i < NV; ++i) {
      f32x4 o = (gh[i] - mg) * rstd + xc[i] * coef;
      if constexpr (WIDE) {
        o += dr[i];
        if (cg) {
          const float cs_ = crs ? crs[m / crps] : 1.0f;
          const f32x4 sc = o * cs_;
          *(bf16x4*)(cg + m * ldc + lg.col0 + i * lg.step4) = bf16x4{(bf16)sc[0], (bf16)sc[1], (bf16)sc[2], (bf16)sc[3]};
        }
      } else {
        if (dres) o += *(const f32x4*)(dres + m * ldr + lg.col0 + i * lg.step4);
      }
      *(f32x4*)(dx + m * ldd + lg.col0 + i * lg.step4) = o;
    }
  }
  for (int w = 0; w < kLnBwdWaves; ++w) {
    if (wid == w) {
#pragma unroll
      for (int i = 0; i < NV; ++i) {
        f32x4* qa = (f32x4*)(smem + lg.col0 + i * lg.step4);
        if (w == 0) *qa = pa[i];
        else *qa += pa[i];
        if (lg.seg == 0) {
          f32x4* qb = (f32x4*)(smem + D + lg.acol0 + i * 32);
          const f32x4 mine = *(const f32x4*)(pbl + lg.acol0 + i * 32);
          if (w == 0) *qb = mine;
          else *qb += mine;
        }
      }
    }
    __syncthreads();
  }
  float* outp = partials + (size_t)blockIdx.x * 2 * D;
  for (int e = threadIdx.x * 4; e < D + c; e += kLnBwdWaves * 64 * 4) *(f32x4*)(outp + e) = *(const f32x4*)(smem + e);
}

inline int ln_blocks(int64_t M) {
  int64_t b = (M + kLnBwdWaves - 1) / kLnBwdWaves;
#ifndef OCTIC_LNBWD_CAP
#define OCTIC_LNBWD_CAP 256
#endif
  const int64_t cap = OCTIC_LNBWD_CAP;
  return (int)(b < 1 ? 1 : (b > cap ? cap : b));
}
inline int ln_fwd_blocks(int64_t M) {
  int64_t b = (M + 15) / 16;
  return (int)(b < 1 ? 1 : (b > 4096 ? 4096 : b));
}

inline int pick_nv(int c) {
  const int need = (2 * c + 63) / 64;
  return need <= 2 ? 2 : (need <= 4 ? 4 : (need <= 5 ? 5 : (need <= 8 ? 8 : 0)));
}

inline bool view_is_packed(const View& v, int c, int es) {
  for (int g = 1; g < 5; ++g)
    if (v.ld[g] != v.ld[0] || v.p[g] != v.p[0] + (int64_t)g * c * es) return false;
  return true;
}

template <typename TOUT, bool PK>
void launch_ln_fwd(int nv, int grid, hipStream_t s, View vx, View vy, const float* const a[5], const float* beta,
                   float* stats, int64_t M, int c, float eps) {
  switch (nv) {
    case 2: ln_fwd_kernel<TOUT, 2, PK><<<grid, 256, 0, s>>>(vx, vy, a[0], a[1], a[2], a[3], a[4], beta, stats, M, c, eps); break;
    case 4: ln_fwd_kernel<TOUT, 4, PK><<<grid, 256, 0, s>>>(vx, vy, a[0], a[1], a[2], a[3], a[4], beta, stats, M, c, eps); break;
    case 5: ln_fwd_kernel<TOUT, 5, PK><<<grid, 256, 0, s>>>(vx, vy, a[0], a[1], a[2], a[3], a[4], beta, stats, M, c, eps); break;
    default: ln_fwd_kernel<TOUT, 8, PK><<<grid, 256, 0, s>>>(vx, vy, a[0], a[1], a[2], a[3], a[4], beta, stats, M, c, eps); break;
  }
}

template <typename TG, bool PK>
void launch_ln_bwd(int nv, int grid, size_t smem, hipStream_t s, View vg, View vx, const float* stats,
                   const float* const a[5], View vr, int has_dres, View vd, float* partials, int64_t M, int c) {
  switch (nv) {
    case 2: ln_bwd_kernel<TG, 2, PK><<<grid, kLnBwdWaves * 64, smem, s>>>(vg, vx, stats, a[0], a[1], a[2], a[3], a[4], vr, has_dres, vd, partials, M, c); break;
    case 4: ln_bwd_kernel<TG, 4, PK><<<grid, kLnBwdWaves * 64, smem, s>>>(vg, vx, stats, a[0], a[1], a[2], a[3], a[4], vr, has_dres, vd, partials, M, c); break;
    case 5: ln_bwd_kernel<TG, 5, PK><<<grid, kLnBwdWaves * 64, smem, s>>>(vg, vx, stats, a[0], a[1], a[2], a[3], a[4], vr, has_dres, vd, partials, M, c); break;
    default: ln_bwd_kernel<TG, 8, PK><<<grid, kLnBwdWaves * 64, smem, s>>>(vg, vx, stats, a[0], a[1], a[2], a[3], a[4], vr, has_dres, vd, partials, M, c); break;
  }
}

}

using namespace octic;

extern "C" {

int octic_layernorm_d8_fwd(const octic_view* x, const octic_view* y, const float* const alpha[5], const float* beta,
                           float* stats, int64_t M, int c, float eps, int out_dtype, void* stream) {
  int e;
  if ((e = check_c(c)) || (e = check_view(x, c, OCTIC_F32)) || (e = check_view(y, c, out_dtype))) return e;
  const int nv = pick_nv(c);
  if (M <= 0 || nv == 0) return OCTIC_ESHAPE;
  const float* a[5] = {nullptr, nullptr, nullptr, nullptr, nullptr};
  if (alpha && alpha[0]) {
    for (int i = 0; i < 5; ++i) {
      if (!alpha[i]) return OCTIC_ENULL;
      a[i] = alpha[i];
    }
  }
  View vx = make_view<void>(x), vy = make_view<void>(y);
  const int grid = ln_fwd_blocks(M);
  hipStream_t s = (hipStream_t)stream;
  if (out_dtype != OCTIC_F32 && out_dtype != OCTIC_BF16) return OCTIC_EDTYPE;
  const bool pk = view_is_packed(vx, c, 4) && view_is_packed(vy, c, elem_size(out_dtype));
  if (pk && (c % 32) == 0 && c <= 256) {
    const float* xp = (const float*)vx.p[0];
#define LN_FWD_G8(T, N) ln_fwd_g8_kernel<T, N><<<grid, 256, 0, s>>>(xp, vx.ld[0], (T*)vy.p[0], vy.ld[0], a[0], a[1], a[2], a[3], a[4], beta, stats, M, c, eps)
#define LN_FWD_G8_NV(T) switch (c / 32) { case 1: LN_FWD_G8(T, 1); break; case 2: LN_FWD_G8(T, 2); break; case 3: LN_FWD_G8(T, 3); break; \
    case 4: LN_FWD_G8(T, 4); break; case 5: LN_FWD_G8(T, 5); break; case 6: LN_FWD_G8(T, 6); break; case 7: LN_FWD_G8(T, 7); break; default: LN_FWD_G8(T, 8); break; }
    if (out_dtype == OCTIC_F32) { LN_FWD_G8_NV(float) } else { LN_FWD_G8_NV(bf16) }
    return launch_status();
  }
  if (out_dtype == OCTIC_F32) {
    if (pk) launch_ln_fwd<float, true>(nv, grid, s, vx, vy, a, beta, stats, M, c, eps);
    else launch_ln_fwd<float, false>(nv, grid, s, vx, vy, a, beta, stats, M, c, eps);
  } else {
    if (pk) launch_ln_fwd<bf16, true>(nv, grid, s, vx, vy, a, beta, stats, M, c, eps);
    else launch_ln_fwd<bf16, false>(nv, grid, s, vx, vy, a, beta, stats, M, c, eps);
  }
  return launch_status();
}

int octic_layernorm_d8_bwd_blocks(int64_t M) { return ln_blocks(M); }

static int ln_bwd_impl(const octic_view* g, const octic_view* x, const float* stats, const float* const alpha[5],
                       const octic_view* dres, const octic_view* dx, float* partials, int64_t M, int c, int g_dtype,
                       void* stream, const float* crs, int64_t crps, void* cg, const float* ns = nullptr,
                       int64_t nrps = 0) {
  int e;
  if (ns && (nrps <= 0 || M % nrps)) return OCTIC_ESHAPE;
  if ((e = check_c(c)) || (e = check_view(g, c, g_dtype)) || (e = check_view(x, c, OCTIC_F32)) ||
      (e = check_view(dx, c, OCTIC_F32)))
    return e;
  if (dres && (e = check_view(dres, c, OCTIC_F32))) return e;
  if (!stats || !partials) return OCTIC_ENULL;
  const int nv = pick_nv(c);
  if (M <= 0 || nv == 0) return OCTIC_ESHAPE;
  const float* a[5] = {nullptr, nullptr, nullptr, nullptr, nullptr};
  if (alpha && alpha[0]) {
    for (int i = 0; i < 5; ++i) {
      if (!alpha[i]) return OCTIC_ENULL;
      a[i] = alpha[i];
    }
  }
  View vg = make_view<void>(g), vx = make_view<void>(x), vd = make_view<void>(dx);
  View vr = dres ? make_view<void>(dres) : vd;
  const int grid = ln_blocks(M);
  const size_t smem = (size_t)2 * 8 * c * sizeof(float);
  hipStream_t s = (hipStream_t)stream;
  if (g_dtype != OCTIC_F32 && g_dtype != OCTIC_BF16) return OCTIC_EDTYPE;
  const bool pk = view_is_packed(vg, c, elem_size(g_dtype)) && view_is_packed(vx, c, 4) && view_is_packed(vd, c, 4) &&
                  view_is_packed(vr, c, 4);
  const int hd = dres ? 1 : 0;
  if (pk && (c % 32) == 0 && c <= 256) {
    const float* rp = dres ? (const float*)vr.p[0] : nullptr;
    const size_t smem_g8 = (size_t)(3 * 8 * c + kLnBwdWaves * c) * sizeof(float);
#define LN_BWD_G8(T, N) ln_bwd_g8_kernel<T, N><<<grid, kLnBwdWaves * 64, smem_g8, s>>>((const T*)vg.p[0], vg.ld[0], (const float*)vx.p[0], vx.ld[0], stats, a[0], a[1], a[2], a[3], a[4], rp, vr.ld[0], (float*)vd.p[0], vd.ld[0], partials, M, c)
#define LN_BWD_G8_NV(T) switch (c / 32) { case 1: LN_BWD_G8(T, 1); break; case 2: LN_BWD_G8(T, 2); break; case 3: LN_BWD_G8(T, 3); break; \
    case 4: LN_BWD_G8(T, 4); break; case 5: LN_BWD_G8(T, 5); break; case 6: LN_BWD_G8(T, 6); break; case 7: LN_BWD_G8(T, 7); break; default: LN_BWD_G8(T, 8); break; }
    if (OCTIC_LNBWD_WIDE && g_dtype == OCTIC_BF16 && c / 32 <= 5) {
#define LN_BWD_G8W(N) ln_bwd_g8_kernel<bf16, N, true><<<grid, kLnBwdWaves * 64, smem_g8, s>>>((const bf16*)vg.p[0], vg.ld[0], (const float*)vx.p[0], vx.ld[0], stats, a[0], a[1], a[2], a[3], a[4], rp, vr.ld[0], (float*)vd.p[0], vd.ld[0], partials, M, c, crs, crs ? crps : 1, (bf16*)cg, (int64_t)8 * c)
#define LN_BWD_G8S(N) ln_bwd_g8_kernel<bf16, N, true, true><<<grid, kLnBwdWaves * 64, smem_g8, s>>>((const bf16*)vg.p[0], vg.ld[0], (const float*)vx.p[0], vx.ld[0], stats, a[0], a[1], a[2], a[3], a[4], rp, vr.ld[0], (float*)vd.p[0], vd.ld[0], partials, M, c, crs, crs ? crps : 1, (bf16*)cg, (int64_t)8 * c, ns, nrps)
      if (ns) {
        switch (c / 32) { case 1: LN_BWD_G8S(1); break; case 2: LN_BWD_G8S(2); break; case 3: LN_BWD_G8S(3); break;
                          case 4: LN_BWD_G8S(4); break; default: LN_BWD_G8S(5); break; }
        return launch_status();
      }
      switch (c / 32) { case 1: LN_BWD_G8W(1); break; case 2: LN_BWD_G8W(2); break; case 3: LN_BWD_G8W(3); break;
                        case 4: LN_BWD_G8W(4); break; default: LN_BWD_G8W(5); break; }
#undef LN_BWD_G8S
#undef LN_BWD_G8W
      return launch_status();
    }
    if (cg) return OCTIC_ESHAPE;
    if (g_dtype == OCTIC_F32) { LN_BWD_G8_NV(float) } else { LN_BWD_G8_NV(bf16) }
    return launch_status();
  }
  if (cg) return OCTIC_ESHAPE;
  if (g_dtype == OCTIC_F32) {
    if (pk) launch_ln_bwd<float, true>(nv, grid, smem, s, vg, vx, stats, a, vr, hd, vd, partials, M, c);
    else launch_ln_bwd<float, false>(nv, grid, smem, s, vg, vx, stats, a, vr, hd, vd, partials, M, c);
  } else {
    if (pk) launch_ln_bwd<bf16, true>(nv, grid, smem, s, vg, vx, stats, a, vr, hd, vd, partials, M, c);
    else launch_ln_bwd<bf16, false>(nv, grid, smem, s, vg, vx, stats, a, vr, hd, vd, partials, M, c);
  }
  return launch_status();
}

int octic_layernorm_d8_bwd(const octic_view* g, const octic_view* x, const float* stats, const float* const alpha[5],
                           const octic_view* dres, const octic_view* dx, float* partials, int64_t M, int c, int g_dtype,
                           void* stream) {
  return ln_bwd_impl(g, x, stats, alpha, dres, dx, partials, M, c, g_dtype, stream, nullptr, 1, nullptr);
}

int octic_layernorm_d8_bwd_skip(const octic_view* g, const octic_view* x, const float* stats, const float* const alpha[5],
                                const octic_view* dres, const octic_view* dx, float* partials, int64_t M, int c, int g_dtype,
                                const float* sample_scale, int64_t rows_per_sample, void* stream) {
  return ln_bwd_impl(g, x, stats, alpha, dres, dx, partials, M, c, g_dtype, stream, nullptr, 1, nullptr, sample_scale,
                     rows_per_sample);
}

int octic_layernorm_d8_bwd_cast(const octic_view* g, const octic_view* x, const float* stats, const float* const alpha[5],
                                const octic_view* dres, const octic_view* dx, float* partials, int64_t M, int c,
                                const float* rs, int64_t rows_per_sample, void* gcast, void* stream) {
  return octic_layernorm_d8_bwd_cast_skip(g, x, stats, alpha, dres, dx, partials, M, c, rs, rows_per_sample, gcast, nullptr,
                                          0, stream);
}

int octic_layernorm_d8_bwd_cast_skip(const octic_view* g, const octic_view* x, const float* stats,
                                     const float* const alpha[5], const octic_view* dres, const octic_view* dx,
                                     float* partials, int64_t M, int c, const float* rs, int64_t rows_per_scale, void* gcast,
                                     const float* sample_scale, int64_t rows_per_sample, void* stream) {
  if (!gcast) return OCTIC_ENULL;
  if (rs && rows_per_scale <= 0) return OCTIC_ESHAPE;
  if (((uintptr_t)gcast) & 15) return OCTIC_EALIGN;
  return ln_bwd_impl(g, x, stats, alpha, dres, dx, partials, M, c, OCTIC_BF16, stream, rs, rows_per_scale, gcast,
                     sample_scale, rows_per_sample);
}

int octic_layernorm_d8_bwd_finish(const float* partials, int nblk, int c, float* const dalpha[5], float* dbeta,
                                  void* stream) {
  if (!partials) return OCTIC_ENULL;
  if (nblk <= 0 || check_c(c)) return OCTIC_ESHAPE;
  float* d[5] = {nullptr, nullptr, nullptr, nullptr, nullptr};
  if (dalpha)
    for (int i = 0; i < 5; ++i) d[i] = dalpha[i];
  ln_bwd_finish_kernel<<<(7 * c + 15) / 16, 256, 0, (hipStream_t)stream>>>(partials, nblk, c, d[0], d[1], d[2], d[3], d[4], dbeta);
  return launch_status();
}

int octic_layernorm_d8_bwd_finish_batch(const octic_ln_finish_job* jobs, int njobs, void* stream) {
  if (!jobs) return OCTIC_ENULL;
  if (njobs < 0) return OCTIC_ESHAPE;
  for (int i = 0; i < njobs; ++i) {
    if (!jobs[i].partials) return OCTIC_ENULL;
    if (jobs[i].nblk <= 0 || check_c(jobs[i].c)) return OCTIC_ESHAPE;
  }
  for (int i0 = 0; i0 < njobs; i0 += 48) {
    const int n = njobs - i0 < 48 ? njobs - i0 : 48;
    LnFinishPack pack = {};
    int cmax = 0;
    for (int i = 0; i < n; ++i) {
      pack.j[i] = jobs[i0 + i];
      cmax = jobs[i0 + i].c > cmax ? jobs[i0 + i].c : cmax;
    }
    ln_bwd_finish_batch_kernel<<<dim3((7 * cmax + 15) / 16, n), 256, 0, (hipStream_t)stream>>>(pack);
  }
  return launch_status();
}

}
```

octic_vits_amd/functional.py:

```python
import os

import torch

from . import ops


class Octic(tuple):

    def __new__(cls, packed: torch.Tensor, c: int):
        self = super().__new__(cls, ops.split_packed(packed, c))
        self.packed, self.c = packed, c
        return self


def as_packed(xs):
    if isinstance(xs, Octic):
        return xs.packed, xs.c
    if len(xs) != 5:
        raise AssertionError("Input should be a 5-tuple")
    c = xs[0].shape[-1]
    if xs[4].shape[-2:] != (2, 2 * c):
        raise ValueError(f"E irrep must be [..., 2, {2 * c}], got {tuple(xs[4].shape)}")
    return torch.cat([xs[0], xs[1], xs[2], xs[3], xs[4].flatten(-2)], dim=-1), c

# ... 219 lines not shown
        if dx.dtype != x_in_dtype:
            dx = dx.to(x_in_dtype)
    dysum = ops.colsum_a1(gv, M, cout, dtype, x) if (has_bias and not ops.wgrad_has_colsum(cin, cout, dtype)) else None
    w32 = [_c(w.detach().float()) for w in w5] if has_cs else None
    f32_masters = all(w.dtype == torch.float32 for w in w5)
    dw, dcs, dbias = ops.linear_wgrad(xv, gv, M, cin, cout, dtype, x, w32=w32, cs5=cs32, bias=b32, dysum=dysum,
                                      want_bias=has_bias, may_defer=f32_masters, wparams=w5 if f32_masters else None)
    if not f32_masters:
        dw = [d.to(w.dtype) for d, w in zip(dw, w5)]
    return dx, dw, dbias, (dcs if has_cs else [None] * 5)


class LinearD8Fn(torch.autograd.Function):

    @staticmethod
    def forward(ctx, x, wA1, wA2, wB1, wB2, wE, bias, resid, rs, sA1, sA2, sB1, sB2, sE, cin, cout, rps, dtype, prep,
                skip_out=None, skip_dx=None, zero_dx=None):
        w5 = (wA1, wA2, wB1, wB2, wE)
        cs5 = None if sA1 is None else (sA1, sA2, sB1, sB2, sE)
        fused = resid is not None
        out_dtype = resid.dtype if fused else dtype
        handed = x
        x, wb, M, y, b32, cs32, rs32 = _linear_d8_fwd_prep(ctx, x, w5, cs5, bias, rs, cin, cout, rps, dtype, out_dtype, prep)
        rv = ops.pview(_c(resid), cout) if fused else None
        plain = not fused and rs32 is None and cs32 is None
        ss_out = linear_skip_scale(skip_out, rps, M) if plain else None
        dropped = ring_skip_scale(rs32, rps, M) if fused else None
        ops.linear_fwd(ops.pview(x, cin), wb, b32, ops.pview(y, cout), M, cin, cout, dtype, out_dtype, x,
                       resid_v=rv, rs=rs32, rps=rps, cs5=cs32, sample_scale=ss_out, skip_rps=rps, dropped=dropped, dropped_rps=rps)
        ss_dx = linear_skip_scale(skip_dx, rps, M)
        z_dx = ring_skip_scale(zero_dx, rps, M) if (plain and ss_dx is None) else None
        row_skip_fill(handed, row_skip_scale(zero_dx, rps, M) if (plain and ss_dx is None) else None, rps, M)
        ctx.save_for_backward(x, rs32, b32, ss_dx, z_dx, *w5, *(cs32 or []))
        ctx.fused = fused
        return y

    @staticmethod
    def backward(ctx, dy):
        cin, cout, rps, dtype, has_cs = ctx.lin[:5]
        x, rs32, b32, ss_dx, z_dx, *rest = ctx.saved_tensors
        w5, cs32 = rest[:5], (rest[5:] if has_cs else None)
        dy = _c(dy)
        if ctx.fused or rs32 is not None or dy.dtype != dtype:
            g = ops.cast_rowscale(_c(dy.float()), rs32, rps, dtype, cout)
        else:
            g = dy
        dx, dw, dbias, dcs = _linear_d8_grads(ctx, x, g, w5, cs32, b32, ss_dx, z_dx)
        return (dx, *dw, dbias, dy if ctx.fused else None, None, *dcs, None, None, None, None, None, None, None, None)


class LinearD8NormFn(torch.autograd.Function):

    @staticmethod
    def forward(ctx, x, wA1, wA2, wB1, wB2, wE, bias, resid, rs, sA1, sA2, sB1, sB2, sE, cin, cout, rps, dtype, prep,
                a1, a2, b1, b2, ae, beta, eps, skip_dx=None):
        w5 = (wA1, wA2, wB1, wB2, wE)
        cs5 = None if sA1 is None else (sA1, sA2, sB1, sB2, sE)
        x, wb, M, y, b32, cs32, rs32 = _linear_d8_fwd_prep(ctx, x, w5, cs5, bias, rs, cin, cout, rps, dtype, resid.dtype, prep)
        ops.linear_fwd(ops.pview(x, cin), wb, b32, ops.pview(y, cout), M, cin, cout, dtype, resid.dtype, x,
                       resid_v=ops.pview(_c(resid), cout), rs=rs32, rps=rps, cs5=cs32, dropped=ring_skip_scale(rs32, rps, M),
                       dropped_rps=rps)
        alpha = None if a1 is None else [_c(t.float()) for t in (a1, a2, b1, b2, ae)]
        yn, stats = ops.layernorm_fwd(y, alpha, None if beta is None else _c(beta.float()), eps, dtype, cout)
        ctx.save_for_backward(x, rs32, b32, y, stats, linear_skip_scale(skip_dx, rps, M), *w5, *(cs32 or []), *(alpha or []))
        ctx.has_affine, ctx.has_beta = alpha is not None, beta is not None
        ctx.set_materialize_grads(False)
        row_skip_attach(ctx, yn)
        return y, yn

    @staticmethod
    def backward(ctx, dy, dyn):
        cin, cout, rps, dtype, has_cs = ctx.lin[:5]
        has_affine = ctx.has_affine
        x, rs32, b32, y, stats, ss_dx, *rest = ctx.saved_tensors
        w5 = rest[:5]
        cs32 = rest[5:10] if has_cs else None
        alpha = rest[(10 if has_cs else 5):] if has_affine else None
        M = x.numel() // (8 * cin)
        dal, dbeta, g = [None] * 5, None, None
        if dyn is not None:
            dres = None if dy is None else _c(dy.float())
            gn = _c(dyn)
            ns, nrps = row_skip_get(ctx, M)
            if ops.layernorm_bwd_cast_ok(gn, y, cout) and dtype == torch.bfloat16:
                dy, dal_, dbeta, g = ops.layernorm_bwd_cast(gn, y, stats, alpha, dres, cout, rs32, rps,
                                                            want_param_grads=has_affine, sample_scale=ns, rows_per_sample=nrps)
            else:
                dy, dal_, dbeta = ops.layernorm_bwd(gn, y, stats, alpha, dres, cout, want_param_grads=has_affine,
                                                    sample_scale=ns, rows_per_sample=nrps)
            dal = dal_ if dal_ is not None else dal
        dy = _c(dy)
        if g is None:
            g = ops.cast_rowscale(_c(dy.float()), rs32, rps, dtype, cout)
        dx, dw, dbias, dcs = _linear_d8_grads(ctx, x, g, w5, cs32, b32, ss_dx)
        return (dx, *dw, dbias, dy, None, *dcs, None, None, None, None, None, *dal, dbeta if ctx.has_beta else None, None, None)


class PackHeadsFn(torch.autograd.Function):

    @staticmethod
    def forward(ctx, qkv, H, c):
        B, T = qkv.shape[0], qkv.shape[1]
        ctx.meta = (B, T, H, c)
        q, k, v = ops.pack_heads(_c(qkv), B, T, H, c, 3)
        return q, k, v

    @staticmethod
    def backward(ctx, gq, gk, gv):
        B, T, H, c = ctx.meta
        return ops.unpack_heads([gq, gk, gv], B, T, H, c), None, None


class UnpackHeadsFn(torch.autograd.Function):
    @staticmethod
    def forward(ctx, o, c):
        B, H, T, _ = o.shape
        ctx.meta = (B, T, H, c)
        return ops.unpack_heads([o], B, T, H, c)

    @staticmethod
    def backward(ctx, g):
        B, T, H, c = ctx.meta
        return ops.pack_heads(_c(g), B, T, H, c, 1)[0], None


class AttnFn(torch.autograd.Function):

    @staticmethod
    def forward(ctx, q, k, v, scale):
        q, k, v = _c(q), _c(k), _c(v)
        o, lse = ops.attn_fwd(q, k, v, scale)
        ctx.save_for_backward(q, k, v, o, lse)
        ctx.scale = scale
        return o

    @staticmethod
    def backward(ctx, do):
        q, k, v, o, lse = ctx.saved_tensors
        do = _c(do)
        dq, dk, dv = torch.empty_like(q), torch.empty_like(k), torch.empty_like(v)
        ops.attn_bwd(q, k, v, o, do, lse, ctx.scale, dq, dk, dv)
        return dq, dk, dv, None


def _skip_from_env(name):
    return os.environ.get(name, "1").strip() != "0"


ATTN_SKIP_DROPPED = _skip_from_env("OCTIC_ATTN_SKIP")


def skip_scale(rs, B):
    if (not ATTN_SKIP_DROPPED or rs is None or not rs.is_cuda or rs.dtype != torch.float32 or rs.dim() != 1
            or rs.numel() != B or not rs.is_contiguous()):
        return None
    return rs.detach()


WGRAD_SKIP_DROPPED = _skip_from_env("OCTIC_WGRAD_SKIP")


def whole_sample_mask(rs, rps, M, rows_to=None):
    if (rs is None or rows_to is not None or torch.compiler.is_compiling() or not rs.is_cuda
            or rs.dtype != torch.float32 or rs.dim() != 1 or not rs.is_contiguous() or rps < 2 or rs.numel() * rps != M):
        return None
    return rs.detach()


def wgrad_skip_scale(rs, rps, M, rows_to=None):
    return whole_sample_mask(rs, rps, M, rows_to) if WGRAD_SKIP_DROPPED else None


DENSE_NT_SKIP_DROPPED = _skip_from_env("OCTIC_DENSE_SKIP")


DENSE_NARROW_DROPPED = _skip_from_env("OCTIC_DENSE_NARROW")


DENSE_CLS_FOLD = _skip_from_env("OCTIC_DENSE_CLS_FOLD")
DENSE_CLS_FOLD_MIN_DROP = 0.4


def dense_cls_fold(drop_prob):
    return bool(DENSE_CLS_FOLD and DENSE_NARROW_DROPPED and drop_prob is not None and float(drop_prob) >= DENSE_CLS_FOLD_MIN_DROP)


DENSE_IMAGE_DROPPED = _skip_from_env("OCTIC_DENSE_IMAGE_SKIP")


def dense_skip_scale(rs, rps, M, rows_to=None):
    return whole_sample_mask(rs, rps, M, rows_to) if DENSE_NT_SKIP_DROPPED else None


LINEAR_SKIP_DROPPED = _skip_from_env("OCTIC_LINEAR_SKIP")


def linear_skip_scale(rs, rps, M, rows_to=None):
    return whole_sample_mask(rs, rps, M, rows_to) if LINEAR_SKIP_DROPPED else None


RING_SKIP_DROPPED = _skip_from_env("OCTIC_RING_SKIP")


def ring_skip_scale(rs, rps, M):
    return linear_skip_scale(rs, rps, M) if RING_SKIP_DROPPED else None


ROW_SKIP_DROPPED = _skip_from_env("OCTIC_ROW_SKIP")


def row_skip_scale(rs, rps, M, rows_to=None):
    return whole_sample_mask(rs, rps, M, rows_to) if ROW_SKIP_DROPPED else None


class RowSkipSlot:
    __slots__ = ("scale", "rps", "rows", "fills")

    def __init__(self):
        self.scale, self.rps, self.rows, self.fills = None, 0, 0, 0

    def get(self, rows):
        if self.fills != 1 or self.scale is None or self.rows != rows:
            return None, 0
        return self.scale, self.rps


def row_skip_attach(ctx, yn):
    ctx.row_skip = yn._octic_row_skip = RowSkipSlot()


def row_skip_fill(x, scale, rps, rows):
    slot = getattr(x, "_octic_row_skip", None)
    if slot is not None:
        slot.fills += 1
        slot.scale, slot.rps, slot.rows = scale, rps, rows


def row_skip_get(ctx, rows):
    slot = getattr(ctx, "row_skip", None)
    return (None, 0) if slot is None else slot.get(rows)


class AttnPackedFn(torch.autograd.Function):

    @staticmethod
    def forward(ctx, qkv, H, c, scale, sample_scale=None):
        qkv = _c(qkv)
        ss = skip_scale(sample_scale, qkv.shape[0])
        o, lse = ops.attn_fwd_packed(qkv, H, c, scale, sample_scale=ss)
        ctx.save_for_backward(qkv, o, lse, ss)
        ctx.meta = (H, c, scale)
        return o

    @staticmethod
    def backward(ctx, do):
        qkv, o, lse, ss = ctx.saved_tensors
        H, c, scale = ctx.meta
        return ops.attn_bwd_packed(qkv, o, _c(do), lse, H, c, scale, sample_scale=ss), None, None, None, None


class AttnFusedQKVFn(torch.autograd.Function):

    @staticmethod
    def forward(ctx, qkv, scale, sample_scale=None):
        qkv = _c(qkv)
        B, T, _, H, hd = qkv.shape
        ss = skip_scale(sample_scale, B) if qkv.dtype == torch.bfloat16 else None
        q, k, v = (qkv[:, :, i].permute(0, 2, 1, 3) for i in range(3))
        o = torch.empty((B, T, H, hd), dtype=qkv.dtype, device=qkv.device)
        ov = o.permute(0, 2, 1, 3)
        _, lse = ops.attn_fwd(q, k, v, scale, out=ov, sample_scale=ss)
        ctx.save_for_backward(qkv, o, lse, ss)
        ctx.scale = scale
        return o.view(B, T, H * hd)

    @staticmethod
    def backward(ctx, do):
        qkv, o, lse, ss = ctx.saved_tensors
        B, T, _, H, hd = qkv.shape
        do = _c(do).view(B, T, H, hd)
        dqkv = torch.empty_like(qkv)
        q, k, v = (qkv[:, :, i].permute(0, 2, 1, 3) for i in range(3))
        dq, dk, dv = (dqkv[:, :, i].permute(0, 2, 1, 3) for i in range(3))
        ops.attn_bwd(q, k, v, o.permute(0, 2, 1, 3), do.permute(0, 2, 1, 3), lse, ctx.scale, dq, dk, dv, sample_scale=ss)
        return dqkv, None, None


def attention_core(q, k, v, dropout_p=0.0):
    B, H, T, hd = q.shape
    if dropout_p == 0.0 and q.is_cuda and (ops.attn_supported(T, hd, q.dtype) or ops.attn_f32_supported(T, hd, q.dtype)):
        return AttnFn.apply(q, k, v, hd ** -0.5)
    o = torch.nn.functional.scaled_dot_product_attention(q, k, v, dropout_p=dropout_p)
    return o if o.dtype == q.dtype else o.to(q.dtype)


class DenseWeightCache:

    def __init__(self):
        self.key = None
        self.w = self.b = None
        self.wt = self.wt_key = None
        self.static = False
        self.static_wt = False

    def static_nt(self):
        if self.static and self.w is not None and self.w.dtype == torch.bfloat16:
            return self.w, (self.wt if self.static_wt else None)
        return None, None

    @staticmethod
    def _key(w, b, dtype):
        return (dtype, w.data_ptr(), w._version, None if b is None else (b.data_ptr(), b._version))

    def get(self, w, b, dtype):
        key = self._key(w, b, dtype)
        if key != self.key:
            with torch.no_grad():
                self.w = _c(w.detach().to(dtype))
                self.b = None if b is None else _c(b.detach().to(dtype))
            self.key = key
            self.wt, self.wt_key = None, None
            self.static = self.static_wt = False
        return self.w, self.b
# ... 313 lines not shown
        return _timed_lib("dgrad", lambda: a2 @ b, a2.shape[0], b.shape[1], b.shape[0])


def _linear_lib(x2, wb, bias):
    if dense_f32_hip_ok(x2.shape[0], wb.shape[0], wb.shape[-1], x2, wb) and (bias is None or bias.dtype == torch.float32):
        return ops.dense_f32_nt(x2, wb, None if bias is None else _c(bias))
    with torch.autocast("cuda", enabled=False):
        return _timed_lib("fwd", lambda: torch.nn.functional.linear(x2, wb, bias), x2.shape[0], wb.shape[0], wb.shape[1])


WGRAD_PAIRED = True
GELU_FACTOR = True


class WgradPair:
    __slots__ = ("pending",)

    def __init__(self):
        self.pending = None

    def park(self, g2, x2, wparam=None, sample_scale=None, rps=0):
        shape = (g2.shape[1], x2.shape[1])
        dw = ops.grad_dest(wparam, shape)
        landed = wparam if dw is not None else None
        if dw is None:
            dw = torch.empty(shape, dtype=torch.float32, device=g2.device)
        self.pending = (g2, x2, dw.untyped_storage(), dw.data_ptr(), tuple(dw.shape), dw.storage_offset(), landed,
                        sample_scale, rps)
        ops.DEFERRED_FINISHES.add_pair(self)
        return dw

    def take(self):
        p, self.pending = self.pending, None
        if p is None:
            return None
        g2, x2, storage, ptr, shape, offset, landed, ss, rps = p
        dw = torch.empty(0, dtype=torch.float32, device=g2.device).set_(storage, offset, shape)
        assert dw.data_ptr() == ptr
        return g2, x2, dw, landed, ss, rps

    def flush(self):
        p = self.take()
        if p is not None:
            g2, x2, dw, landed, ss, rps = p
            dw.copy_(_wgrad_lib(g2, x2, sample_scale=ss, rps=rps))
            ops.grad_written(landed)


def _pair_ready(pair, g2, x2):
    return (pair is not None and WGRAD_PAIRED and WGRAD_HIP and ops.DEFERRED_FINISHES.enabled
            and ops.DEFERRED_FINISHES.allow_pairs and ops._in_backward()
            and g2.is_cuda and g2.dtype == torch.bfloat16 and x2.dtype == torch.bfloat16 and g2.stride(1) == 1
            and x2.stride(1) == 1)


def _tok(shape):
    return int(shape[-2]) if len(shape) >= 3 else 0


def _gemm_fwd(tag, x2, wb, b, cache, name, tokens, ss=None, rps=0, drop=None):
    if tag in DENSE_HIP:
        return ops.dense_gemm_nt(x2, wb, 0, bias=_f32(b), name=f"dense_nt_kernel<{name}>", tokens=tokens, sample_scale=ss,
                                 rows_per_sample=rps, fold_cls=ss is not None and dense_cls_fold(drop), drop=drop)
    return _linear_lib(x2, wb, None if b is None else cache.b)


def _gemm_dgrad(g2, wt, wb, shape, dtype, ss=None, rps=0, drop=None):
    gx = (ops.dense_gemm_nt(g2, wt, 0, name="dense_nt_kernel<dgrad>", tokens=_tok(shape), sample_scale=ss, rows_per_sample=rps,
                            fold_cls=ss is not None and dense_cls_fold(drop))
          if wt is not None else _mm_lib(g2, wb))
    return gx.view(shape).to(dtype)


def _resid_tail_fwd(ctx, x, tag, a2, wb, b, cache, tokens, g32, rs32, rps, nw, nb, neps, rows_to, stream, ds, drop=None):
    ctx.rows_to, ctx.x_shape = rows_to, x.shape
    ctx.tail = (neps is not None, rps, b is not None, nw is not None, nb is not None)
    x2 = x.view(-1, wb.shape[0])
    if neps is None and rows_to is None and tag in DENSE_HIP and DENSE_RESID_FUSED:
        br, out = ops.dense_gemm_nt(a2, wb, 2, bias=_f32(b), gamma=g32, rs=rs32, rps=rps, x=x2, name="dense_nt_kernel<resid>")
        return out.view(x.shape), (br, g32, rs32)
    br = _gemm_fwd(tag, a2, wb, b, cache, tag, tokens, ds, rps, drop)
    if neps is not None:
        nw32, nb32 = _f32(nw), _f32(nb)
        out, yn, stats = ops.dense_resid_layernorm_fwd(x2, br, g32, rs32, rps, nw32, nb32, neps, torch.bfloat16)
        ctx.set_materialize_grads(False)
        yn = yn.view(x.shape)
        row_skip_attach(ctx, yn)
        return (out.view(x.shape), yn), (br, g32, rs32, out, stats, nw32)
    if rows_to is not None:
        ops.scale_residual_fwd_rows_(stream, rows_to.rowmap, x2, br, g32, rs32, rps)
        ctx.mark_dirty(stream)
        return stream, (br, g32, rs32, rows_to.rowmap)
    return ops.scale_residual_fwd(x2, br, g32, rs32, rps).view(x.shape), (br, g32, rs32)


def _resid_tail_bwd(ctx, tail, gout, gyn, want_norm):
    norm, rps, has_b, has_nw, has_nb = ctx.tail
    br, g32, rs32, *rest = tail
    has_gamma = g32 is not None
    dnw = dnb = gbr = None
    if norm:
        out, stats, nw32 = rest
        if gyn is not None:
            want = has_nw and want_norm
            dres = None if gout is None else _c(gout.float()).view(out.shape)
            g2 = _c(gyn).view(out.shape)
            if LN_TAIL_FUSED and ops.dense_ln_bwd_tail_ok(g2, br, out.shape[-1]):
                ns, nrps = row_skip_get(ctx, g2.shape[0])
                gout, dnw, dnb, gbr, dgamma, colsum = ops.dense_layernorm_bwd_tail(
                    g2, out, nw32, stats, dres, br, g32, rs32, rps, want_param_grads=want, want_gamma=has_gamma,
                    want_colsum=has_b, sample_scale=ns, rows_per_sample=nrps)
            else:
                gout, dnw, dnb = ops.dense_layernorm_bwd(g2, out, nw32, stats, dres, want_param_grads=want)
            dnw, dnb = (dnw if has_nw else None), (dnb if has_nb else None)
    elif ctx.rows_to is not None:
        gout = _c(gout.float())
        ctx.rows_to.link.g = gout
        gbr, dgamma, colsum = ops.scale_residual_bwd(gout, br, g32, rs32, rps, want_gamma=has_gamma, want_colsum=has_b,
                                                     rowmap=rest[0])
    if gbr is None:
        gout = _c(gout.float())
        gbr, dgamma, colsum = ops.scale_residual_bwd(gout.view(br.shape), br, g32, rs32, rps, want_gamma=has_gamma,
                                                     want_colsum=has_b)
    gx = None if ctx.rows_to is not None else gout.view(ctx.x_shape)
    return gx, gbr, dgamma, colsum, dnw, dnb


class DenseLinearNTFn(torch.autograd.Function):

    @staticmethod
    def forward(ctx, x, w, b, cache, tag, pair=None, rs=None, rps=0, drop=None):
        ctx.pair = pair
        ctx.drop = drop
        ctx.wparam = w
        xb = _c(x if x.dtype == torch.bfloat16 else x.to(torch.bfloat16))
        wb, wt = cache.get_nt(w, b, ("d" + tag) in DENSE_HIP and ctx.needs_input_grad[0])
        x2 = xb.reshape(-1, wb.shape[1])
        mask = whole_sample_mask(rs, rps, x2.shape[0])
        ds = mask if DENSE_NT_SKIP_DROPPED else None
        y = _gemm_fwd(tag, x2, wb, b, cache, "plain", _tok(x.shape), ds, rps, drop)
        ss = mask if WGRAD_SKIP_DROPPED else None
        rk = mask if ROW_SKIP_DROPPED else None
        row_skip_fill(x, rk, rps, x2.shape[0])
        ctx.rps = rps
        ctx.save_for_backward(x2, wb, wt, ss, ds, rk)
        ctx.meta = (b is not None, x.dtype, x.shape, tag)
        return y.view(*x.shape[:-1], wb.shape[0])

    @staticmethod
    def backward(ctx, gy):
        x2, wb, wt, ss, ds, rk = ctx.saved_tensors
        has_b, x_dtype, x_shape, tag = ctx.meta
        g2 = _c(gy).reshape(-1, wb.shape[0])
        gx = _gemm_dgrad(g2, wt, wb, x_shape, x_dtype, ds, ctx.rps, ctx.drop) if ctx.needs_input_grad[0] else None
        gb = None
        if has_b:
            gb = (ops.dense_colsum(g2, rk, ctx.rps)
                  if g2.is_cuda and g2.dtype == torch.bfloat16 and g2.shape[1] % 8 == 0
                  else g2.sum(0, dtype=torch.float32))
        pair = ctx.pair
        if pair is not None and pair.pending is not None:
            pg, px = pair.pending[0], pair.pending[1]
            if (_pair_ready(pair, g2, x2) and pg.shape[0] == g2.shape[0] and px.shape[1] == x2.shape[1]
                    and ops.dense_wgrad_pair_ok(g2.shape[0], g2.shape[1], pg.shape[1], x2.shape[1])):
                pg, px, pdw, landed, pss, prps = pair.take()
                dest = ops.grad_dest(ctx.wparam, (g2.shape[1], x2.shape[1]))
                both = ss if (ss is not None and pss is not None and prps == ctx.rps and pss.data_ptr() == ss.data_ptr()
                              and pss.numel() == ss.numel()) else None
                dw, _ = ops.dense_wgrad_tn_pair(g2, x2, pg, px, dw1=pdw, dw0=dest, sample_scale=both, rows_per_sample=ctx.rps)
                ops.grad_written(landed, ctx.wparam if dest is not None else None)
                return gx, dw, gb, None, None, None, None, None, None
            pair.flush()
        return gx, _wgrad_lib(g2, x2, ctx.wparam, ss, ctx.rps), gb, None, None, None, None, None, None


class DenseProjResidFn(torch.autograd.Function):

    @staticmethod
    def forward(ctx, x, a, w, b, gamma, rs, rps, cache, nw=None, nb=None, neps=None, pair=None, rows_to=None, stream=None,
                drop=None):
        ctx.pair = pair
        ctx.drop = drop
        ctx.wparam = w
        x = _c(x)
        ab = _c(a if a.dtype == torch.bfloat16 else a.to(torch.bfloat16))
        wb, wt = cache.get_nt(w, b, "dproj" in DENSE_HIP and ctx.needs_input_grad[1])
        a2 = ab.reshape(-1, wb.shape[1])
        rs32 = _f32(rs)
        outs, tail = _resid_tail_fwd(ctx, x, "proj", a2, wb, b, cache, _tok(a.shape), _f32(gamma), rs32, rps,
                                     nw, nb, neps, rows_to, stream, dense_skip_scale(rs32, rps, a2.shape[0], rows_to), drop)
        ctx.save_for_backward(a2, wb, wt, *tail)
        ctx.meta = (a.dtype, a.shape)
        return outs

# ... 183 lines not shown
```

octic_vits_amd/ops.py:

```python
import ctypes
import operator

import torch

from . import _lib
from ._lib import BF16, F32, OcticView, PtrArray5, check, lib

_DT = {torch.float32: F32, torch.bfloat16: BF16}
_DTN = {torch.float32: "f32", torch.bfloat16: "bf16"}


class KernelTimer:

    def __init__(self):
        self.on = False
        self.records = []
        self.overhead_us = 0.0

    def enable(self):
        self.on, self.records = True, []
        pairs = []
        for _ in range(64):
            e0, e1 = torch.cuda.Event(enable_timing=True), torch.cuda.Event(enable_timing=True)
            e0.record()
# ... 149 lines not shown
                         "operands' device")
    return sample_scale, rps


def gelu_fwd(xv, yv, M, c, dtype, ref, sample_scale=None, rows_per_sample=0):
    ss, rps = _sample_scale(sample_scale, rows_per_sample, M, ref, "gelu_fwd")
    t = KERNEL_TIMER.start()
    check(lib().octic_gelu_d8_fwd_skip(ctypes.byref(xv), ctypes.byref(yv), M, c, dt_code(dtype), _p(ss), rps, _stream(ref)))
    KERNEL_TIMER.stop(t, f"gelu_fwd_kernel<{_DTN[dtype]}>", 2 * M * 8 * c * ref.element_size())


def gelu_bwd(gv, xv, ov, M, c, dtype, ref, sample_scale=None, rows_per_sample=0):
    ss, rps = _sample_scale(sample_scale, rows_per_sample, M, ref, "gelu_bwd")
    t = KERNEL_TIMER.start()
    check(lib().octic_gelu_d8_bwd_skip(ctypes.byref(gv), ctypes.byref(xv), ctypes.byref(ov), M, c, dt_code(dtype), _p(ss), rps,
                                       _stream(ref)))
    KERNEL_TIMER.stop(t, f"gelu_bwd_kernel<{_DTN[dtype]}>", 3 * M * 8 * c * ref.element_size())


def layernorm_fwd(x, alpha5, beta, eps, out_dtype, c, want_stats=True):
    M = x.numel() // (8 * c)
    y = torch.empty(x.shape, dtype=out_dtype, device=x.device)
    stats = torch.empty((M, 8), dtype=torch.float32, device=x.device) if want_stats else None
    xv, yv = pview(x, c), pview(y, c)
    t = KERNEL_TIMER.start()
    check(lib().octic_layernorm_d8_fwd(ctypes.byref(xv), ctypes.byref(yv), _arr5(alpha5), _p(beta), _p(stats), M, c,
                                       float(eps), dt_code(out_dtype), _stream(x)))
    KERNEL_TIMER.stop(t, f"ln_fwd_kernel<{_DTN[out_dtype]}>", M * 8 * c * (4 + y.element_size()))
    return y, stats


def layernorm_bwd(g, x, stats, alpha5, dres, c, want_param_grads=True, sample_scale=None, rows_per_sample=0):
    M = x.numel() // (8 * c)
    ss, srps = _sample_scale(sample_scale, rows_per_sample, M, x, "layernorm_bwd")
    dx = torch.empty_like(x)
    nblk = lib().octic_layernorm_d8_bwd_blocks(M)
    partials = torch.empty((nblk, 2, 8 * c), dtype=torch.float32, device=x.device)
    gv, xv, dv = pview(g, c), pview(x, c), pview(dx, c)
    rv = pview(dres, c) if dres is not None else None
    t = KERNEL_TIMER.start()
    check(lib().octic_layernorm_d8_bwd_skip(ctypes.byref(gv), ctypes.byref(xv), _p(stats), _arr5(alpha5),
                                            ctypes.byref(rv) if rv is not None else None, ctypes.byref(dv), _p(partials),
                                            M, c, dt_code(g.dtype), _p(ss), srps, _stream(x)))
    KERNEL_TIMER.stop(t, f"ln_bwd_kernel<{_DTN[g.dtype]}>", M * 8 * c * (g.element_size() + 8 + (4 if dres is not None else 0)))
    if not want_param_grads or alpha5 is None:
        return dx, None, None
    dal = [torch.empty_like(a) for a in alpha5]
    dbeta = torch.empty(c, dtype=torch.float32, device=x.device)
    _ln_finish(partials, nblk, c, dal, dbeta, _stream(x))
    return dx, dal, dbeta


def sample_blocks_ok(full, compact, idx):
    return (full.is_cuda and full.is_contiguous() and compact.is_contiguous() and full.dtype == compact.dtype
            and idx.dtype == torch.int64 and idx.is_cuda and full.dim() >= 2 and full.shape[1:] == compact.shape[1:]
            and (full[0].numel() * full.element_size()) % 16 == 0 and 0 < idx.numel() == compact.shape[0] <= 65535)


def gather_samples(full, idx, out=None):
    if out is None:
        out = torch.empty((idx.numel(),) + tuple(full.shape[1:]), dtype=full.dtype, device=full.device)
    check(lib().octic_sample_blocks(_p(full), _p(out), _p(idx), idx.numel(), full[0].numel() * full.element_size(), 0,
                                    _stream(full)))
    return out


def scatter_samples_(full, idx, compact):
    check(lib().octic_sample_blocks(_p(compact), _p(full), _p(idx), idx.numel(), full[0].numel() * full.element_size(), 1,
                                    _stream(full)))
    return full


def _ln_finish(partials, nblk, c, dal, dbeta, stream):
    if DEFERRED_FINISHES.enabled and _in_backward():
        DEFERRED_FINISHES.add_ln(partials, nblk, c, dal, dbeta, stream)
        return
    check(lib().octic_layernorm_d8_bwd_finish(_p(partials), nblk, c, _arr5(dal), _p(dbeta), stream))


def layernorm_bwd_cast_ok(g, x, c):
    return g.dtype == torch.bfloat16 and x.dtype == torch.float32 and c % 32 == 0 and c <= 160


def layernorm_bwd_cast(g, x, stats, alpha5, dres, c, rs, rps, want_param_grads=True, sample_scale=None, rows_per_sample=0):
    M = x.numel() // (8 * c)
    ss, srps = _sample_scale(sample_scale, rows_per_sample, M, x, "layernorm_bwd_cast")
    dx = torch.empty_like(x)
    gc = torch.empty(x.shape, dtype=torch.bfloat16, device=x.device)
    nblk = lib().octic_layernorm_d8_bwd_blocks(M)
    partials = torch.empty((nblk, 2, 8 * c), dtype=torch.float32, device=x.device)
    gv, xv, dv = pview(g, c), pview(x, c), pview(dx, c)
    rv = pview(dres, c) if dres is not None else None
    t = KERNEL_TIMER.start()
    check(lib().octic_layernorm_d8_bwd_cast_skip(ctypes.byref(gv), ctypes.byref(xv), _p(stats), _arr5(alpha5),
                                                 ctypes.byref(rv) if rv is not None else None, ctypes.byref(dv), _p(partials),
                                                 M, c, _p(rs), int(rps), _p(gc), _p(ss), srps, _stream(x)))
    KERNEL_TIMER.stop(t, "ln_bwd_kernel<bf16>", M * 8 * c * (2 + 8 + (4 if dres is not None else 0) + 2))
    if not want_param_grads or alpha5 is None:
        return dx, None, None, gc
    dal = [torch.empty_like(a) for a in alpha5]
    dbeta = torch.empty(c, dtype=torch.float32, device=x.device)
    _ln_finish(partials, nblk, c, dal, dbeta, _stream(x))
    return dx, dal, dbeta, gc


_DW_WS = {}


def dense_gemm_ok(rows, N, K):
    return K % 64 == 0 and K >= 128 and N % 64 == 0 and N >= 128 and rows * max(N, K) * 2 < 2 ** 31


DENSE_WGRAD_MAX_BLOCKS = 256


@torch.compiler.assume_constant_result
def _dense_wgrad_query(M, N0, N1, K, ld_max):
    return _lib.plan("octic_dense_wgrad_plan", M, N0, N1, K, ld_max)


def _dense_wgrad_plan(M, N0, N1, K, ld_max):
    return _dense_wgrad_query(operator.index(M), N0, N1, K, ld_max)


def dense_wgrad_ok(M, N, K, ld_max=0):
    plan = _dense_wgrad_plan(M, N, 0, K, ld_max)
    return plan is not None and (plan[0] == 64 or (N // 256) * (K // 256) <= DENSE_WGRAD_MAX_BLOCKS)


GRAD_DEST = None


def grad_dest(param, shape):
    if GRAD_DEST is None or param is None:
        return None
    d = GRAD_DEST.get(param.data_ptr())
    if d is None or param.grad is not None or tuple(d.shape) != tuple(shape) or d.dtype != torch.float32 or not d.is_contiguous():
        return None
    return d.detach()


def grad_written(*params):
    w = getattr(GRAD_DEST, "written", None)
    if w is not None:
        for prm in params:
            if prm is not None:
                w(prm.data_ptr())


def dense_wgrad_tn(dy, x, name=None, out=None, sample_scale=None, rows_per_sample=0):
    _require_cuda(dy)
    M, N = dy.shape
    K = x.shape[1]
    if dy.stride(1) != 1 or x.stride(1) != 1 or x.shape[0] != M:
        raise ValueError("dense_wgrad_tn: operands must be [M,N] / [M,K] row-major")
    ss, rps = _sample_scale(sample_scale, rows_per_sample, M, dy, "dense_wgrad_tn")
    need = int(lib().octic_dense_wgrad_workspace_bytes(M, N, K))
    ws = _DW_WS.get(dy.device)
    if ws is None or ws.numel() < need:
        ws = _DW_WS[dy.device] = torch.zeros(need, dtype=torch.uint8, device=dy.device)
    dw = out if out is not None else torch.empty((N, K), dtype=torch.float32, device=dy.device)
    t = KERNEL_TIMER.start()
    check(lib().octic_dense_wgrad_tn_skip(_p(dy), _p(x), M, N, K, dy.stride(0), x.stride(0), _p(dw), _p(ss), rps, _p(ws),
                                          _stream(dy)))
    KERNEL_TIMER.stop(t, name or f"dense_tn_kernel<{N}x{K}>", 2 * (M * N + M * K) + 4 * N * K, 2.0 * M * N * K)
    return dw


def dense_wgrad_pair_ok(M, N0, N1, K):
    return (N1 > 0 and _dense_wgrad_plan(M, N0, N1, K, 0) is not None
            and ((N0 + N1) // 256) * (K // 256) <= DENSE_WGRAD_MAX_BLOCKS)


def dense_wgrad_tn_pair(dy0, x0, dy1, x1, dw1=None, dw0=None, sample_scale=None, rows_per_sample=0):
    _require_cuda(dy0)
    M, N0 = dy0.shape
    N1, K = dy1.shape[1], x0.shape[1]
    if not (dy1.shape[0] == M and x0.shape[0] == M and x1.shape == (M, K) and all(t.stride(1) == 1 for t in (dy0, x0, dy1, x1))):
        raise ValueError("dense_wgrad_tn_pair: operands must be [M,N0] / [M,K] / [M,N1] / [M,K] row-major")
# ... 426 lines not shown
            arr[i].partials = partials.data_ptr()
            arr[i].out0 = o0
            arr[i].out1 = o1
            arr[i].scale1 = sc.data_ptr() if sc is not None else None
            arr[i].nblocks = nblk
            arr[i].d = d
        t = KERNEL_TIMER.start()
        check(lib().octic_dense_finish_batch(ctypes.cast(arr, ctypes.c_void_p), len(jobs), jobs[0][7]))
        KERNEL_TIMER.stop(t, "dense_finish_batch_kernel", sum(j[1] * 2 * j[2] * 4 for j in jobs))


DEFERRED_FINISHES = _DeferredFinishes()


def _in_backward():
    try:
        return torch._C._current_graph_task_id() != -1
    except Exception:
        return False


def _finish(partials, nblk, d, out0, out1, scale1, stream, out1_ptr=None):
    o0 = out0.data_ptr() if out0 is not None else None
    o1 = out1_ptr if out1_ptr is not None else (out1.data_ptr() if out1 is not None else None)
    if DEFERRED_FINISHES.enabled and _in_backward():
        keep = tuple(t.untyped_storage() for t in (out0, out1) if t is not None)
        DEFERRED_FINISHES.add(partials, nblk, d, o0, o1, scale1, keep, stream)
        return
    check(lib().octic_dense_finish(_p(partials), nblk, d, ctypes.c_void_p(o0) if o0 else None,
                                   ctypes.c_void_p(o1) if o1 else None, _p(scale1), stream))


def dense_layernorm_fwd(x, w, b, eps, out_dtype):
    _require_cuda(x)
    d = x.shape[-1]
    rows = x.numel() // d
    y = torch.empty(x.shape, dtype=out_dtype, device=x.device)
    stats = torch.empty((rows, 2), dtype=torch.float32, device=x.device)
    t = KERNEL_TIMER.start()
    check(lib().octic_dense_layernorm_fwd(_p(x), _p(y), dt_code(out_dtype), _p(w), _p(b), _p(stats), rows, d, float(eps),
                                          _stream(x)))
    KERNEL_TIMER.stop(t, f"dense_ln_fwd_kernel<{_DTN[out_dtype]}>", rows * d * (4 + y.element_size()))
    return y, stats


def _check_rowmap(rowmap, rows):
    if rowmap.dtype != torch.int32 or not rowmap.is_contiguous() or rowmap.numel() != rows:
        raise ValueError("row map: a contiguous int32 tensor with one entry per compact row")


def dense_layernorm_fwd_rows(x, rowmap, w, b, eps, out_dtype):
    _require_cuda(x)
    d = x.shape[-1]
    rows = rowmap.numel()
    _check_rowmap(rowmap, rows)
    y = torch.empty((1, rows, d), dtype=out_dtype, device=x.device)
    xa = torch.empty((1, rows, d), dtype=torch.float32, device=x.device)
    stats = torch.empty((rows, 2), dtype=torch.float32, device=x.device)
    t = KERNEL_TIMER.start()
    check(lib().octic_dense_layernorm_fwd_rows(_p(x), _p(y), dt_code(out_dtype), _p(w), _p(b), _p(stats), rows, d, float(eps),
                                               _p(rowmap), _p(xa), _stream(x)))
    KERNEL_TIMER.stop(t, f"dense_ln_fwd_kernel<{_DTN[out_dtype]},rows>", rows * d * (8 + y.element_size()))
    return y, stats, xa


def dense_layernorm_bwd_rows_(gy, xa, w, stats, g, rowmap, want_param_grads=True):
    d = xa.shape[-1]
    rows = rowmap.numel()
    _check_rowmap(rowmap, rows)
    nblk = lib().octic_dense_blocks(rows)
    partials = torch.empty((nblk, 2, d), dtype=torch.float32, device=xa.device) if want_param_grads else None
    t = KERNEL_TIMER.start()
    check(lib().octic_dense_layernorm_bwd_rows(_p(gy), dt_code(gy.dtype), _p(xa), _p(w), _p(stats), _p(g), _p(g), _p(partials),
                                               rows, d, _p(rowmap), _stream(xa)))
    KERNEL_TIMER.stop(t, f"dense_ln_bwd_kernel<{_DTN[gy.dtype]},rows>", rows * d * (gy.element_size() + 12))
    if not want_param_grads:
        return None, None
    dw = torch.empty(d, dtype=torch.float32, device=xa.device)
    db = torch.empty(d, dtype=torch.float32, device=xa.device)
    _finish(partials, nblk, d, dw, db, None, _stream(xa))
    return dw, db


def dense_resid_layernorm_fwd(x, yb, gamma, rs, rps, w, b, eps, out_dtype):
    _require_cuda(x)
    d = x.shape[-1]
    rows = x.numel() // d
    xout = torch.empty_like(x)
    y = torch.empty(x.shape, dtype=out_dtype, device=x.device)
    stats = torch.empty((rows, 2), dtype=torch.float32, device=x.device)
    t = KERNEL_TIMER.start()
    check(lib().octic_dense_resid_layernorm_fwd(_p(x), _p(yb), dt_code(yb.dtype), _p(gamma), _p(rs), int(rps), _p(xout), _p(y),
                                                dt_code(out_dtype), _p(w), _p(b), _p(stats), rows, d, float(eps), _stream(x)))
    KERNEL_TIMER.stop(t, f"dense_resid_ln_fwd_kernel<{_DTN[out_dtype]}>", rows * d * (8 + yb.element_size() + y.element_size()))
    return xout, y, stats


def dense_layernorm_bwd(gy, x, w, stats, dres, want_param_grads=True):
    d = x.shape[-1]
    rows = x.numel() // d
    dx = torch.empty_like(x)
    nblk = lib().octic_dense_blocks(rows)
    partials = torch.empty((nblk, 2, d), dtype=torch.float32, device=x.device) if want_param_grads else None
    t = KERNEL_TIMER.start()
    check(lib().octic_dense_layernorm_bwd(_p(gy), dt_code(gy.dtype), _p(x), _p(w), _p(stats), _p(dres), _p(dx),
                                          _p(partials), rows, d, _stream(x)))
    KERNEL_TIMER.stop(t, f"dense_ln_bwd_kernel<{_DTN[gy.dtype]}>",
                      rows * d * (gy.element_size() + 8 + (4 if dres is not None else 0)))
    if not want_param_grads:
        return dx, None, None
    dw = torch.empty(d, dtype=torch.float32, device=x.device)
    db = torch.empty(d, dtype=torch.float32, device=x.device)
    _finish(partials, nblk, d, dw, db, None, _stream(x))
    return dx, dw, db


def dense_ln_bwd_tail_ok(gy, yb, d):
    return gy.dtype == torch.bfloat16 and yb.dtype == torch.bfloat16 and d % 256 == 0 and d <= 1280


def dense_layernorm_bwd_tail(gy, x, w, stats, dres, yb, gamma, rs, rps, want_param_grads=True, want_gamma=True,
                             want_colsum=True, sample_scale=None, rows_per_sample=0):
    d = x.shape[-1]
    rows = x.numel() // d
    ss, srps = _sample_scale(sample_scale, rows_per_sample, rows, x, "dense_layernorm_bwd_tail")
    dx = torch.empty_like(x)
    gyb = torch.empty(x.shape, dtype=yb.dtype, device=x.device)
    nblk = lib().octic_dense_blocks(rows)
    p1 = torch.empty((nblk, 2, d), dtype=torch.float32, device=x.device) if want_param_grads else None
    want2 = want_gamma or want_colsum
    p2 = torch.empty((nblk, 2, d), dtype=torch.float32, device=x.device) if want2 else None
    t = KERNEL_TIMER.start()
    check(lib().octic_dense_layernorm_bwd_tail_skip(_p(gy), _p(x), _p(w), _p(stats), _p(dres), _p(dx), _p(p1), _p(yb), _p(gamma),
                                                    _p(rs), int(rps), _p(gyb), _p(p2), rows, d, _p(ss), srps, _stream(x)))
    KERNEL_TIMER.stop(t, "dense_ln_bwd_tail_kernel<bf16>", rows * d * (2 + 8 + (4 if dres is not None else 0) + 4))
    dw = db = dgamma = colsum = None
    if want_param_grads:
        dw = torch.empty(d, dtype=torch.float32, device=x.device)
        db = torch.empty(d, dtype=torch.float32, device=x.device)
        _finish(p1, nblk, d, dw, db, None, _stream(x))
    if want2:
        dgamma = torch.empty(d, dtype=torch.float32, device=x.device) if want_gamma else None
        colsum = torch.empty(d, dtype=torch.float32, device=x.device) if want_colsum else None
        _finish(p2, nblk, d, dgamma, colsum, gamma, _stream(x))
    return dx, dw, db, gyb, dgamma, colsum


def _rows2d(t):
    K = t.shape[-1]
    t2 = t.reshape(-1, K)
    if t2.stride(1) != 1 or (t2.shape[0] > 1 and t2.stride(0) % 8):
        t2 = t2.contiguous()
    return t2, t2.shape[0], K, (t2.stride(0) if t2.shape[0] > 1 else K)


def softmax_center(t, center, inv_temp):
    _require_cuda(t)
    t2, rows, K, ld = _rows2d(t)
    out = torch.empty(t.shape, dtype=torch.float32, device=t.device)
    c = None if center is None else center.reshape(-1).float().contiguous()
    tk = KERNEL_TIMER.start()
    check(lib().octic_softmax_center(_p(t2), dt_code(t2.dtype), ld, _p(c), float(inv_temp), _p(out), rows, K, _stream(t)))
    KERNEL_TIMER.stop(tk, f"softmax_center_kernel<{_DTN[t2.dtype]}>", rows * K * (2 * t2.element_size() + 4))
    return out


def soft_ce_fwd(s, tprob, inv_temp):
    _require_cuda(s)
    s2, rows, K, ld = _rows2d(s)
    if tprob.dtype != torch.float32 or not tprob.is_contiguous() or tprob.shape[-1] != K:
        raise ValueError("soft_ce_fwd: tprob must be a contiguous f32 [Nt, K] tensor")
    nt = tprob.numel() // K
    loss, lse, tsum = (torch.empty(rows, dtype=torch.float32, device=s.device) for _ in range(3))
    tk = KERNEL_TIMER.start()
    check(lib().octic_soft_ce_fwd(_p(s2), dt_code(s2.dtype), ld, _p(tprob), nt, float(inv_temp), _p(loss), _p(lse), _p(tsum),
                                  rows, K, _stream(s)))
    KERNEL_TIMER.stop(tk, f"soft_ce_fwd_kernel<{_DTN[s2.dtype]}>", rows * K * (s2.element_size() + 4))
    return loss, lse, tsum


def soft_ce_bwd(s, tprob, inv_temp, g, lse, tsum):
    s2, rows, K, ld = _rows2d(s)
    nt = tprob.numel() // K
    ds = torch.empty((rows, K), dtype=s2.dtype, device=s.device)
    g = g.reshape(-1).float().contiguous()
    tk = KERNEL_TIMER.start()
    check(lib().octic_soft_ce_bwd(_p(s2), dt_code(s2.dtype), ld, _p(tprob), nt, float(inv_temp), _p(g), _p(lse), _p(tsum),
                                  _p(ds), K, rows, K, _stream(s)))
    KERNEL_TIMER.stop(tk, f"soft_ce_bwd_kernel<{_DTN[s2.dtype]}>", rows * K * (2 * s2.element_size() + 4))
    return ds.view(s.shape)


def _sinkhorn_rows2d(x):
    _require_cuda(x)
    if x.dim() != 2:
        raise ValueError("sinkhorn passes take 2-D logits [rows, K]")
    if x.data_ptr() % 16:
        x = x.clone(memory_format=torch.contiguous_format)
    return _rows2d(x)


def sinkhorn_rows(x, inv_temp, u=None):
    x2, rows, K, ld = _sinkhorn_rows2d(x)
    rowmax, c = (torch.empty(rows, dtype=torch.float32, device=x.device) for _ in range(2))
    tk = KERNEL_TIMER.start()
    check(lib().octic_sinkhorn_rows(_p(x2), dt_code(x2.dtype), ld, float(inv_temp), _p(u), _p(rowmax), _p(c), rows, K,
                                    _stream(x)))
    KERNEL_TIMER.stop(tk, f"sinkhorn_rows_kernel<{_DTN[x2.dtype]}>", rows * K * x2.element_size())
    return rowmax, c


def sinkhorn_protos(x, inv_temp, shift, weight):
    x2, rows, K, ld = _sinkhorn_rows2d(x)
    slabs = lib().octic_sinkhorn_slabs(rows)
    if slabs < 0:
        check(slabs)
    r = torch.empty(K, dtype=torch.float32, device=x.device)
# ... 976 lines not shown
```

Baseline: 1287 images/s.

## Update residual-stream grads in place and skip branch loads for dropped samples

Adds in-place variants of the dense and octic layernorm backward tail kernels. They reuse the incoming residual gradient buffer as dx and write back only the rows of live (non-dropped) samples, which saves an allocation and a full write for dropped rows. A Python ownership tracker hands the gradient buffer from one block's backward to the next within the same autograd task. The forward residual+layernorm kernel also skips loading the branch output for samples dropped by drop_path. The cost is aliasing risk: correctness depends on the ownership checks in the tracker and on the sample mask.

Measured after the change: 1301 images/s, median of 6. 1.1% higher.

```diff
diff --git a/include/octic_hip.h b/include/octic_hip.h
--- a/include/octic_hip.h
+++ b/include/octic_hip.h
@@ -70,6 +70,10 @@
                                      const float* const alpha[5], const octic_view* dres, const octic_view* dx,
                                      float* partials, int64_t M, int c, const float* rs, int64_t rows_per_scale, void* gcast,
                                      const float* sample_scale, int64_t rows_per_sample, void* stream);
+int octic_layernorm_d8_bwd_cast_inplace(const octic_view* g, const octic_view* x, const float* stats,
+                                        const float* const alpha[5], const octic_view* dx, float* partials, int64_t M, int c,
+                                        const float* rs, int64_t rows_per_scale, void* gcast, const float* sample_scale,
+                                        int64_t rows_per_sample, void* stream);
 int octic_layernorm_d8_bwd_finish(const float* partials, int nblk, int c, float* const dalpha[5], float* dbeta,
                                   void* stream);
 typedef struct octic_ln_finish_job {
@@ -253,6 +257,9 @@
 int octic_dense_resid_layernorm_fwd(const float* x, const void* yb, int yb_dtype, const float* gamma, const float* rs,
                                     int64_t rows_per_scale, float* xout, void* y, int y_dtype, const float* w,
                                     const float* b, float* stats, int64_t rows, int d, float eps, void* stream);
+int octic_dense_resid_layernorm_fwd_skip(const float* x, const void* yb, int yb_dtype, const float* gamma, const float* rs,
+                                         int64_t rows_per_scale, float* xout, void* y, int y_dtype, const float* w,
+                                         const float* b, float* stats, int64_t rows, int d, float eps, void* stream);
 int octic_dense_layernorm_fwd(const float* x, void* y, int y_dtype, const float* w, const float* b, float* stats,
                               int64_t rows, int d, float eps, void* stream);
 int octic_dense_layernorm_bwd(const void* gy, int g_dtype, const float* x, const float* w, const float* stats,
@@ -275,6 +282,10 @@
                                         const float* dres, float* dx, float* partials, const void* yb, const float* gamma,
                                         const float* rs, int64_t rows_per_scale, void* gyb, float* partials2, int64_t rows,
                                         int d, const float* sample_scale, int64_t rows_per_sample, void* stream);
+int octic_dense_layernorm_bwd_tail_inplace(const void* gy, const float* x, const float* w, const float* stats, float* dx,
+                                           float* partials, const void* yb, const float* gamma, const float* rs,
+                                           int64_t rows_per_scale, void* gyb, float* partials2, int64_t rows, int d,
+                                           const float* sample_scale, int64_t rows_per_sample, void* stream);
 int octic_dense_gelu_blocks(void);
 int octic_dense_gelu_bwd(const void* h, const void* g, void* dh, float* partials, int64_t rows, int d, void* stream);
 int octic_dense_colsum(const void* g, int64_t rows, int d, int64_t ld, float* partials, void* stream);
diff --git a/octic_vits_amd/_lib.py b/octic_vits_amd/_lib.py
--- a/octic_vits_amd/_lib.py
+++ b/octic_vits_amd/_lib.py
@@ -48,6 +48,8 @@
                                             c_void_p]),
     "octic_layernorm_d8_bwd_cast_skip": (c_int, [VP, VP, c_void_p, c_void_p, VP, VP, c_void_p, c_i64, c_int, c_void_p, c_i64,
                                                  c_void_p, c_void_p, c_i64, c_void_p]),
+    "octic_layernorm_d8_bwd_cast_inplace": (c_int, [VP, VP, c_void_p, c_void_p, VP, c_void_p, c_i64, c_int, c_void_p, c_i64,
+                                                    c_void_p, c_void_p, c_i64, c_void_p]),
     "octic_layernorm_d8_bwd_finish": (c_int, [c_void_p, c_int, c_int, c_void_p, c_void_p, c_void_p]),
     "octic_layernorm_d8_bwd_finish_batch": (c_int, [c_void_p, c_int, c_void_p]),
     "octic_sample_blocks": (c_int, [c_void_p, c_void_p, c_void_p, c_i64, c_i64, c_int, c_void_p]),
@@ -85,11 +87,15 @@
                                           c_float, c_void_p]),
     "octic_dense_resid_layernorm_fwd": (c_int, [c_void_p, c_void_p, c_int, c_void_p, c_void_p, c_i64, c_void_p, c_void_p, c_int,
                                                 c_void_p, c_void_p, c_void_p, c_i64, c_int, c_float, c_void_p]),
+    "octic_dense_resid_layernorm_fwd_skip": (c_int, [c_void_p, c_void_p, c_int, c_void_p, c_void_p, c_i64, c_void_p, c_void_p,
+                                                     c_int, c_void_p, c_void_p, c_void_p, c_i64, c_int, c_float, c_void_p]),
     "octic_dense_layernorm_bwd": (c_int, [c_void_p, c_int, c_void_p, c_void_p, c_void_p, c_void_p, c_void_p, c_void_p,
                                           c_i64, c_int, c_void_p]),
     "octic_dense_layernorm_bwd_tail": (c_int, [c_void_p] * 10 + [c_i64, c_void_p, c_void_p, c_i64, c_int, c_void_p]),
     "octic_dense_layernorm_bwd_tail_skip": (c_int, [c_void_p] * 10 + [c_i64, c_void_p, c_void_p, c_i64, c_int, c_void_p, c_i64,
                                                                       c_void_p]),
+    "octic_dense_layernorm_bwd_tail_inplace": (c_int, [c_void_p] * 9 + [c_i64, c_void_p, c_void_p, c_i64, c_int, c_void_p, c_i64,
+                                                                        c_void_p]),
     "octic_dense_finish": (c_int, [c_void_p, c_int, c_int, c_void_p, c_void_p, c_void_p, c_void_p]),
     "octic_dense_finish_batch": (c_int, [c_void_p, c_int, c_void_p]),
     "octic_dense_gelu_blocks": (c_int, []),
diff --git a/octic_vits_amd/csrc/dense.hip b/octic_vits_amd/csrc/dense.hip
--- a/octic_vits_amd/csrc/dense.hip
+++ b/octic_vits_amd/csrc/dense.hip
@@ -80,7 +80,7 @@
   }
 }
 
-template <typename TY, typename TOUT, int NV>
+template <typename TY, typename TOUT, int NV, bool SKIPY = false>
 __global__ __launch_bounds__(256) void dense_resid_ln_fwd_kernel(const float* __restrict__ x, const TY* __restrict__ yb,
                                                                  const float* __restrict__ gamma, const float* __restrict__ rs,
                                                                  long rps, float* __restrict__ xout, TOUT* __restrict__ y,
@@ -106,12 +106,19 @@
     f32x4 xv[NV];
     float s = 0.f;
     const float rsv = rs ? rs[r / rps] : 1.f;
+    bool tail = true;
+    if constexpr (SKIPY) tail = mask_live(rsv);
     if (NV <= 6 && d == NV * 256) {
       typename Row4<TY>::vec yv[NV];
 #pragma unroll
       for (int i = 0; i < NV; ++i) xv[i] = *(const f32x4*)(xr + (i * 64 + lane) * 4);
-#pragma unroll
-      for (int i = 0; i < NV; ++i) yv[i] = Row4<TY>::load_raw(yr_in + (i * 64 + lane) * 4);
+      if (tail) {
+#pragma unroll
+        for (int i = 0; i < NV; ++i) yv[i] = Row4<TY>::load_raw(yr_in + (i * 64 + lane) * 4);
+      } else {
+#pragma unroll
+        for (int i = 0; i < NV; ++i) yv[i] = typename Row4<TY>::vec{};
+      }
 #pragma unroll
       for (int i = 0; i < NV; ++i) {
         f32x4 sc = gm[i];
@@ -128,7 +135,13 @@
           const int col = (i * 64 + lane) * 4;
           f32x4 sc = gm[i];
           if (rs) sc *= rsv;
-          xv[i] = *(const f32x4*)(xr + col) + sc * Row4<TY>::load(yr_in + col);
+          if constexpr (SKIPY) {
+            typename Row4<TY>::vec yv = typename Row4<TY>::vec{};
+            if (tail) yv = Row4<TY>::load_raw(yr_in + col);
+            xv[i] = *(const f32x4*)(xr + col) + sc * Row4<TY>::widen(yv);
+          } else {
+            xv[i] = *(const f32x4*)(xr + col) + sc * Row4<TY>::load(yr_in + col);
+          }
           *(f32x4*)(xo + col) = xv[i];
         }
         s += hsum(xv[i]);
@@ -285,13 +298,16 @@
   if (partials) slab_reduce<NV>(lds, partials + (long)blockIdx.x * 2 * d, pw, pb, ok, d);
 }
 
-template <typename TG, int NV, bool SKIP = false, typename... MASK>
+template <bool INPLACE> struct StreamPtr { typedef float* __restrict__ type; };
+template <> struct StreamPtr<true> { typedef float* type; };
+template <typename TG, int NV, bool SKIP = false, bool INPLACE = false, typename... MASK>
 __global__ __launch_bounds__(512, 2) void dense_ln_bwd_tail_kernel(
     const TG* __restrict__ gy, const float* __restrict__ x, const float* __restrict__ w,
-    const float* __restrict__ stats, const float* __restrict__ dres, float* __restrict__ dx,
+    const float* __restrict__ stats, const float* __restrict__ dres, typename StreamPtr<INPLACE>::type dx,
     float* __restrict__ partials, const TG* __restrict__ yb, const float* __restrict__ gamma,
     const float* __restrict__ rs, long rps, TG* __restrict__ gyb, float* __restrict__ partials2, long rows, int d,
     MASK... mask) {
+  static_assert(SKIP || !INPLACE, "only the sample mask tells which rows keep their dres");
   extern __shared__ float lds[];
   const float* __restrict__ ns = mask_scale(mask...);
   const long nrps = mask_rows(mask...);
@@ -335,8 +351,18 @@
         gr[i] = typename Row4<TG>::vec{};
       }
     }
-#pragma unroll
-    for (int i = 0; i < NV; ++i) dr[i] = dres ? *(const f32x4*)(dres + o + i * 256) : f32x4{0.f, 0.f, 0.f, 0.f};
+    if constexpr (INPLACE) {
+      if (live || tail) {
+#pragma unroll
+        for (int i = 0; i < NV; ++i) dr[i] = *(const f32x4*)(dx + o + i * 256);
+      } else {
+#pragma unroll
+        for (int i = 0; i < NV; ++i) dr[i] = f32x4{0.f, 0.f, 0.f, 0.f};
+      }
+    } else {
+#pragma unroll
+      for (int i = 0; i < NV; ++i) dr[i] = dres ? *(const f32x4*)(dres + o + i * 256) : f32x4{0.f, 0.f, 0.f, 0.f};
+    }
     if (tail) {
 #pragma unroll
       for (int i = 0; i < NV; ++i) yr[i] = Row4<TG>::load_raw(yb + o + i * 256);
@@ -364,12 +390,21 @@
 #pragma unroll
     for (int i = 0; i < NV; ++i) {
       f32x4 v = (g[i] - m1 - xh[i] * m2) * rstd;
-      if (dres) v += dr[i];
-      *(f32x4*)(dx + o + i * 256) = v;
+      if (INPLACE || dres) v += dr[i];
+      if constexpr (INPLACE) g[i] = v;
+      else *(f32x4*)(dx + o + i * 256) = v;
       const f32x4 t = v * sc;
       p1[i] += t;
       p0[i] += t * Row4<TG>::widen(yr[i]);
       Row4<TG>::store(gyb + o + i * 256, t * *(const f32x4*)(gl + (i * 64 + lane) * 4));
+    }
+    if constexpr (INPLACE) {
+#pragma unroll
+      for (int i = 0; i < NV; ++i) asm volatile("" : "+v"(pw[i]), "+v"(pb[i]), "+v"(p0[i]), "+v"(p1[i]));
+      if (live) {
+#pragma unroll
+        for (int i = 0; i < NV; ++i) *(f32x4*)(dx + o + i * 256) = g[i];
+      }
     }
   }
   if (partials) slab_reduce<NV>(lds, partials + (long)blockIdx.x * 2 * d, pw, pb, ok, d);
@@ -695,6 +730,61 @@
 
 using namespace octic;
 
+template <bool SKIPY>
+static int resid_ln_fwd_impl(const float* x, const void* yb, int yb_dtype, const float* gamma, const float* rs,
+                             int64_t rows_per_scale, float* xout, void* y, int y_dtype, const float* w, const float* b,
+                             float* stats, int64_t rows, int d, float eps, void* stream) {
+  if (rows == 0) return OCTIC_OK;
+  if (!x || !yb || !xout || !y || !stats) return OCTIC_ENULL;
+  if (int e = dense_check(rows, d)) return e;
+  if ((yb_dtype != OCTIC_F32 && yb_dtype != OCTIC_BF16) || (y_dtype != OCTIC_F32 && y_dtype != OCTIC_BF16)) return OCTIC_EDTYPE;
+  if (rs && rows_per_scale <= 0) return OCTIC_ESHAPE;
+  long blocks = (rows + 7) / 8;
+  if (blocks > 8192) blocks = 8192;
+  hipStream_t s = (hipStream_t)stream;
+  const long rps = rs ? rows_per_scale : 1;
+#define OCTIC_RLN(TYB, TO) \
+  DENSE_NV_SWITCH(dense_nv(d), (dense_resid_ln_fwd_kernel<TYB, TO, NV, SKIPY><<<dim3((unsigned)blocks), dim3(256), 0, s>>>( \
+      x, (const TYB*)yb, gamma, rs, rps, xout, (TO*)y, w, b, stats, rows, d, eps)))
+  if (yb_dtype == OCTIC_BF16 && y_dtype == OCTIC_BF16) { OCTIC_RLN(bf16, bf16); }
+  else if (yb_dtype == OCTIC_BF16) { OCTIC_RLN(bf16, float); }
+  else if (y_dtype == OCTIC_BF16) { OCTIC_RLN(float, bf16); }
+  else { OCTIC_RLN(float, float); }
+#undef OCTIC_RLN
+  return launch_status();
+}
+
+static int ln_bwd_tail_impl(const void* gy, const float* x, const float* w, const float* stats, const float* dres,
+                            float* dx, float* partials, const void* yb, const float* gamma, const float* rs,
+                            int64_t rows_per_scale, void* gyb, float* partials2, int64_t rows, int d,
+                            const float* sample_scale, int64_t rows_per_sample, bool inplace, void* stream) {
+  if (sample_scale && (rows_per_sample <= 0 || rows % rows_per_sample)) return OCTIC_ESHAPE;
+  if (rows == 0) return OCTIC_OK;
+  if (!gy || !x || !stats || !dx || !yb || !gyb) return OCTIC_ENULL;
+  if (int e = dense_check(rows, d)) return e;
+  if (d != dense_nv(d) * 256 || dense_nv(d) > 5) return OCTIC_ESHAPE;
+  if (rs && rows_per_scale <= 0) return OCTIC_ESHAPE;
+  const int blocks = dense_blocks(rows);
+  const size_t lds = (size_t)4 * d * sizeof(float);
+  hipStream_t s = (hipStream_t)stream;
+  const long rps = rs ? rows_per_scale : 1;
+  if (inplace) {
+    DENSE_NV_SWITCH(dense_nv(d), (dense_ln_bwd_tail_kernel<bf16, NV, true, true><<<dim3(blocks), dim3(512), lds, s>>>(
+        (const bf16*)gy, x, w, stats, nullptr, dx, partials, (const bf16*)yb, gamma, rs, rps, (bf16*)gyb, partials2, rows, d,
+        sample_scale, (long)rows_per_sample)));
+    return launch_status();
+  }
+  if (sample_scale) {
+    DENSE_NV_SWITCH(dense_nv(d), (dense_ln_bwd_tail_kernel<bf16, NV, true><<<dim3(blocks), dim3(512), lds, s>>>(
+        (const bf16*)gy, x, w, stats, dres, dx, partials, (const bf16*)yb, gamma, rs, rps, (bf16*)gyb, partials2, rows, d,
+        sample_scale, (long)rows_per_sample)));
+    return launch_status();
+  }
+  DENSE_NV_SWITCH(dense_nv(d), (dense_ln_bwd_tail_kernel<bf16, NV><<<dim3(blocks), dim3(512), lds, s>>>(
+      (const bf16*)gy, x, w, stats, dres, dx, partials, (const bf16*)yb, gamma, rs, rps, (bf16*)gyb, partials2, rows, d)));
+  return launch_status();
+}
+
 extern "C" {
 
 int octic_dense_layernorm_fwd(const float* x, void* y, int y_dtype, const float* w, const float* b, float* stats,
@@ -722,24 +812,14 @@
 int octic_dense_resid_layernorm_fwd(const float* x, const void* yb, int yb_dtype, const float* gamma, const float* rs,
                                     int64_t rows_per_scale, float* xout, void* y, int y_dtype, const float* w,
                                     const float* b, float* stats, int64_t rows, int d, float eps, void* stream) {
-  if (rows == 0) return OCTIC_OK;
-  if (!x || !yb || !xout || !y || !stats) return OCTIC_ENULL;
-  if (int e = dense_check(rows, d)) return e;
-  if ((yb_dtype != OCTIC_F32 && yb_dtype != OCTIC_BF16) || (y_dtype != OCTIC_F32 && y_dtype != OCTIC_BF16)) return OCTIC_EDTYPE;
-  if (rs && rows_per_scale <= 0) return OCTIC_ESHAPE;
-  long blocks = (rows + 7) / 8;
-  if (blocks > 8192) blocks = 8192;
-  hipStream_t s = (hipStream_t)stream;
-  const long rps = rs ? rows_per_scale : 1;
-#define OCTIC_RLN(TYB, TO) \
-  DENSE_NV_SWITCH(dense_nv(d), (dense_resid_ln_fwd_kernel<TYB, TO, NV><<<dim3((unsigned)blocks), dim3(256), 0, s>>>( \
-      x, (const TYB*)yb, gamma, rs, rps, xout, (TO*)y, w, b, stats, rows, d, eps)))
-  if (yb_dtype == OCTIC_BF16 && y_dtype == OCTIC_BF16) { OCTIC_RLN(bf16, bf16); }
-  else if (yb_dtype == OCTIC_BF16) { OCTIC_RLN(bf16, float); }
-  else if (y_dtype == OCTIC_BF16) { OCTIC_RLN(float, bf16); }
-  else { OCTIC_RLN(float, float); }
-#undef OCTIC_RLN
-  return launch_status();
+  return resid_ln_fwd_impl<false>(x, yb, yb_dtype, gamma, rs, rows_per_scale, xout, y, y_dtype, w, b, stats, rows, d, eps, stream);
+}
+
+int octic_dense_resid_layernorm_fwd_skip(const float* x, const void* yb, int yb_dtype, const float* gamma, const float* rs,
+                                         int64_t rows_per_scale, float* xout, void* y, int y_dtype, const float* w,
+                                         const float* b, float* stats, int64_t rows, int d, float eps, void* stream) {
+  if (!rs) return OCTIC_ENULL;
+  return resid_ln_fwd_impl<true>(x, yb, yb_dtype, gamma, rs, rows_per_scale, xout, y, y_dtype, w, b, stats, rows, d, eps, stream);
 }
 
 int octic_dense_blocks(int64_t rows) { return dense_blocks(rows); }
@@ -790,27 +870,18 @@
                                         const float* dres, float* dx, float* partials, const void* yb, const float* gamma,
                                         const float* rs, int64_t rows_per_scale, void* gyb, float* partials2, int64_t rows,
                                         int d, const float* sample_scale, int64_t rows_per_sample, void* stream) {
-  if (sample_scale && (rows_per_sample <= 0 || rows % rows_per_sample)) return OCTIC_ESHAPE;
-  if (rows == 0) return OCTIC_OK;
-  if (!gy || !x || !stats || !dx || !yb || !gyb) return OCTIC_ENULL;
-  if (int e = dense_check(rows, d)) return e;
-  if (d != dense_nv(d) * 256 || dense_nv(d) > 5) return OCTIC_ESHAPE;
-  if (rs && rows_per_scale <= 0) return OCTIC_ESHAPE;
-  const int blocks = dense_blocks(rows);
-  const size_t lds = (size_t)4 * d * sizeof(float);
-  hipStream_t s = (hipStream_t)stream;
-  const long rps = rs ? rows_per_scale : 1;
-  if (sample_scale) {
-    DENSE_NV_SWITCH(dense_nv(d), (dense_ln_bwd_tail_kernel<bf16, NV, true><<<dim3(blocks), dim3(512), lds, s>>>(
-        (const bf16*)gy, x, w, stats, dres, dx, partials, (const bf16*)yb, gamma, rs, rps, (bf16*)gyb, partials2, rows, d,
-        sample_scale, (long)rows_per_sample)));
-    return launch_status();
-  }
-  DENSE_NV_SWITCH(dense_nv(d), (dense_ln_bwd_tail_kernel<bf16, NV><<<dim3(blocks), dim3(512), lds, s>>>(
-      (const bf16*)gy, x, w, stats, dres, dx, partials, (const bf16*)yb, gamma, rs, rps, (bf16*)gyb, partials2, rows, d)));
-  return launch_status();
-}
-
+  return ln_bwd_tail_impl(gy, x, w, stats, dres, dx, partials, yb, gamma, rs, rows_per_scale, gyb, partials2, rows, d,
+                          sample_scale, rows_per_sample, false, stream);
+}
+
+int octic_dense_layernorm_bwd_tail_inplace(const void* gy, const float* x, const float* w, const float* stats, float* dx,
+                                           float* partials, const void* yb, const float* gamma, const float* rs,
+                                           int64_t rows_per_scale, void* gyb, float* partials2, int64_t rows, int d,
+                                           const float* sample_scale, int64_t rows_per_sample, void* stream) {
+  if (!sample_scale) return OCTIC_ENULL;
+  return ln_bwd_tail_impl(gy, x, w, stats, nullptr, dx, partials, yb, gamma, rs, rows_per_scale, gyb, partials2, rows, d,
+                          sample_scale, rows_per_sample, true, stream);
+}
 int octic_dense_finish(const float* partials, int nblocks, int d, float* out0, float* out1, const float* scale1,
                        void* stream) {
   if (!partials) return OCTIC_ENULL;
diff --git a/octic_vits_amd/csrc/layernorm.hip b/octic_vits_amd/csrc/layernorm.hip
--- a/octic_vits_amd/csrc/layernorm.hip
+++ b/octic_vits_amd/csrc/layernorm.hip
@@ -385,14 +385,17 @@
 #ifndef OCTIC_LNBWD_WIDE
 #define OCTIC_LNBWD_WIDE 1
 #endif
-template <typename TG, int NV, bool WIDE = false, bool SKIP = false, typename... MASK>
+template <bool INPLACE> struct LnStreamPtr { typedef float* __restrict__ type; };
+template <> struct LnStreamPtr<true> { typedef float* type; };
+template <typename TG, int NV, bool WIDE = false, bool SKIP = false, bool INPLACE = false, typename... MASK>
 __global__ __launch_bounds__(kLnBwdWaves * 64, WIDE ? 2 : OCTIC_LNBWD_OCC) void ln_bwd_g8_kernel(
     const TG* __restrict__ g, int64_t ldg, const float* __restrict__ x, int64_t ldx, const float* __restrict__ stats,
     const float* a0, const float* a1, const float* a2, const float* a3, const float* a4,
-    const float* __restrict__ dres, int64_t ldr, float* __restrict__ dx, int64_t ldd, float* __restrict__ partials,
+    const float* __restrict__ dres, int64_t ldr, typename LnStreamPtr<INPLACE>::type dx, int64_t ldd, float* __restrict__ partials,
     int64_t M, int c, const float* __restrict__ crs = nullptr, int64_t crps = 1, bf16* __restrict__ cg = nullptr,
     int64_t ldc = 0, MASK... mask) {
   static_assert(WIDE || !SKIP, "the sample mask exists in the wide kernel only");
+  static_assert(SKIP || !INPLACE, "only the sample mask tells which rows keep their dres");
   const float* __restrict__ ns = mask_scale(mask...);
   const int64_t nrps = mask_rows(mask...);
   extern __shared__ __attribute__((aligned(16))) float smem[];
@@ -445,9 +448,19 @@
           gr[i] = graw{};
         }
       }
-#pragma unroll
-      for (int i = 0; i < NV; ++i)
-        dr[i] = dres ? *(const f32x4*)(dres + m * ldr + lg.col0 + i * lg.step4) : f32x4{0.f, 0.f, 0.f, 0.f};
+      if constexpr (INPLACE) {
+        if (live || (crs ? mask_live(crs[m / crps]) : true)) {
+#pragma unroll
+          for (int i = 0; i < NV; ++i) dr[i] = *(const f32x4*)(dx + m * ldd + lg.col0 + i * lg.step4);
+        } else {
+#pragma unroll
+          for (int i = 0; i < NV; ++i) dr[i] = f32x4{0.f, 0.f, 0.f, 0.f};
+        }
+      } else {
+#pragma unroll
+        for (int i = 0; i < NV; ++i)
+          dr[i] = dres ? *(const f32x4*)(dres + m * ldr + lg.col0 + i * lg.step4) : f32x4{0.f, 0.f, 0.f, 0.f};
+      }
     }
     float dot = 0.f, t = 0.f;
 #pragma unroll
@@ -475,7 +488,21 @@
     const float coef = coefw * dS;
 #pragma unroll
     for (int i = 0; i < NV; ++i) {
-      f32x4 o = (gh[i] - mg) * rstd + xc[i] * coef;
+      f32x4 o;
+      if constexpr (INPLACE) {
+        const f32x4 u = gh[i] - mg;
+        if constexpr (NV == 1) {
+          const f32x4 t = xc[i] * coef;
+          o = f32x4{__builtin_fmaf(u[0], rstd, t[0]), __builtin_fmaf(u[1], rstd, t[1]), __builtin_fmaf(u[2], rstd, t[2]),
+                    __builtin_fmaf(u[3], rstd, t[3])};
+        } else {
+          const f32x4 t = u * rstd;
+          o = f32x4{__builtin_fmaf(xc[i][0], coef, t[0]), __builtin_fmaf(xc[i][1], coef, t[1]),
+                    __builtin_fmaf(xc[i][2], coef, t[2]), __builtin_fmaf(xc[i][3], coef, t[3])};
+        }
+      } else {
+        o = (gh[i] - mg) * rstd + xc[i] * coef;
+      }
       if constexpr (WIDE) {
         o += dr[i];
         if (cg) {
@@ -486,7 +513,14 @@
       } else {
         if (dres) o += *(const f32x4*)(dres + m * ldr + lg.col0 + i * lg.step4);
       }
-      *(f32x4*)(dx + m * ldd + lg.col0 + i * lg.step4) = o;
+      if constexpr (INPLACE) gh[i] = o;
+      else *(f32x4*)(dx + m * ldd + lg.col0 + i * lg.step4) = o;
+    }
+    if constexpr (INPLACE) {
+      if (live) {
+#pragma unroll
+        for (int i = 0; i < NV; ++i) *(f32x4*)(dx + m * ldd + lg.col0 + i * lg.step4) = gh[i];
+      }
     }
   }
   for (int w = 0; w < kLnBwdWaves; ++w) {
@@ -603,8 +637,9 @@
 static int ln_bwd_impl(const octic_view* g, const octic_view* x, const float* stats, const float* const alpha[5],
                        const octic_view* dres, const octic_view* dx, float* partials, int64_t M, int c, int g_dtype,
                        void* stream, const float* crs, int64_t crps, void* cg, const float* ns = nullptr,
-                       int64_t nrps = 0) {
+                       int64_t nrps = 0, bool inplace = false) {
   int e;
+  if (inplace && (!ns || !cg || dres)) return OCTIC_ENULL;
   if (ns && (nrps <= 0 || M % nrps)) return OCTIC_ESHAPE;
   if ((e = check_c(c)) || (e = check_view(g, c, g_dtype)) || (e = check_view(x, c, OCTIC_F32)) ||
       (e = check_view(dx, c, OCTIC_F32)))
@@ -638,6 +673,12 @@
     if (OCTIC_LNBWD_WIDE && g_dtype == OCTIC_BF16 && c / 32 <= 5) {
 #define LN_BWD_G8W(N) ln_bwd_g8_kernel<bf16, N, true><<<grid, kLnBwdWaves * 64, smem_g8, s>>>((const bf16*)vg.p[0], vg.ld[0], (const float*)vx.p[0], vx.ld[0], stats, a[0], a[1], a[2], a[3], a[4], rp, vr.ld[0], (float*)vd.p[0], vd.ld[0], partials, M, c, crs, crs ? crps : 1, (bf16*)cg, (int64_t)8 * c)
 #define LN_BWD_G8S(N) ln_bwd_g8_kernel<bf16, N, true, true><<<grid, kLnBwdWaves * 64, smem_g8, s>>>((const bf16*)vg.p[0], vg.ld[0], (const float*)vx.p[0], vx.ld[0], stats, a[0], a[1], a[2], a[3], a[4], rp, vr.ld[0], (float*)vd.p[0], vd.ld[0], partials, M, c, crs, crs ? crps : 1, (bf16*)cg, (int64_t)8 * c, ns, nrps)
+#define LN_BWD_G8I(N) ln_bwd_g8_kernel<bf16, N, true, true, true><<<grid, kLnBwdWaves * 64, smem_g8, s>>>((const bf16*)vg.p[0], vg.ld[0], (const float*)vx.p[0], vx.ld[0], stats, a[0], a[1], a[2], a[3], a[4], nullptr, 0, (float*)vd.p[0], vd.ld[0], partials, M, c, crs, crs ? crps : 1, (bf16*)cg, (int64_t)8 * c, ns, nrps)
+      if (inplace) {
+        switch (c / 32) { case 1: LN_BWD_G8I(1); break; case 2: LN_BWD_G8I(2); break; case 3: LN_BWD_G8I(3); break;
+                          case 4: LN_BWD_G8I(4); break; default: LN_BWD_G8I(5); break; }
+        return launch_status();
+      }
       if (ns) {
         switch (c / 32) { case 1: LN_BWD_G8S(1); break; case 2: LN_BWD_G8S(2); break; case 3: LN_BWD_G8S(3); break;
                           case 4: LN_BWD_G8S(4); break; default: LN_BWD_G8S(5); break; }
@@ -645,15 +686,16 @@
       }
       switch (c / 32) { case 1: LN_BWD_G8W(1); break; case 2: LN_BWD_G8W(2); break; case 3: LN_BWD_G8W(3); break;
                         case 4: LN_BWD_G8W(4); break; default: LN_BWD_G8W(5); break; }
+#undef LN_BWD_G8I
 #undef LN_BWD_G8S
 #undef LN_BWD_G8W
       return launch_status();
     }
-    if (cg) return OCTIC_ESHAPE;
+    if (cg || inplace) return OCTIC_ESHAPE;
     if (g_dtype == OCTIC_F32) { LN_BWD_G8_NV(float) } else { LN_BWD_G8_NV(bf16) }
     return launch_status();
   }
-  if (cg) return OCTIC_ESHAPE;
+  if (cg || inplace) return OCTIC_ESHAPE;
   if (g_dtype == OCTIC_F32) {
     if (pk) launch_ln_bwd<float, true>(nv, grid, smem, s, vg, vx, stats, a, vr, hd, vd, partials, M, c);
     else launch_ln_bwd<float, false>(nv, grid, smem, s, vg, vx, stats, a, vr, hd, vd, partials, M, c);
@@ -695,6 +737,18 @@
                      sample_scale, rows_per_sample);
 }
 
+int octic_layernorm_d8_bwd_cast_inplace(const octic_view* g, const octic_view* x, const float* stats,
+                                        const float* const alpha[5], const octic_view* dx, float* partials, int64_t M, int c,
+                                        const float* rs, int64_t rows_per_scale, void* gcast, const float* sample_scale,
+                                        int64_t rows_per_sample, void* stream) {
+  if (!gcast || !sample_scale) return OCTIC_ENULL;
+  if (rs && rows_per_scale <= 0) return OCTIC_ESHAPE;
+  if (((uintptr_t)gcast) & 15) return OCTIC_EALIGN;
+  if (c % 32 || c > 160) return OCTIC_ESHAPE;
+  return ln_bwd_impl(g, x, stats, alpha, nullptr, dx, partials, M, c, OCTIC_BF16, stream, rs, rows_per_scale, gcast,
+                     sample_scale, rows_per_sample, true);
+}
+
 int octic_layernorm_d8_bwd_finish(const float* partials, int nblk, int c, float* const dalpha[5], float* dbeta,
                                   void* stream) {
   if (!partials) return OCTIC_ENULL;
diff --git a/octic_vits_amd/functional.py b/octic_vits_amd/functional.py
--- a/octic_vits_amd/functional.py
+++ b/octic_vits_amd/functional.py
@@ -325,13 +325,16 @@
             dres = None if dy is None else _c(dy.float())
             gn = _c(dyn)
             ns, nrps = row_skip_get(ctx, M)
+            mine = dres is not None and STREAM_GRADS.take(dres)
             if ops.layernorm_bwd_cast_ok(gn, y, cout) and dtype == torch.bfloat16:
                 dy, dal_, dbeta, g = ops.layernorm_bwd_cast(gn, y, stats, alpha, dres, cout, rs32, rps,
-                                                            want_param_grads=has_affine, sample_scale=ns, rows_per_sample=nrps)
+                                                            want_param_grads=has_affine, sample_scale=ns, rows_per_sample=nrps,
+                                                            inplace=mine and ns is not None)
             else:
                 dy, dal_, dbeta = ops.layernorm_bwd(gn, y, stats, alpha, dres, cout, want_param_grads=has_affine,
                                                     sample_scale=ns, rows_per_sample=nrps)
             dal = dal_ if dal_ is not None else dal
+            STREAM_GRADS.offer(dy)
         dy = _c(dy)
         if g is None:
             g = ops.cast_rowscale(_c(dy.float()), rs32, rps, dtype, cout)
@@ -482,6 +485,40 @@
 def row_skip_get(ctx, rows):
     slot = getattr(ctx, "row_skip", None)
     return (None, 0) if slot is None else slot.get(rows)
+
+
+ROW_INPLACE = _skip_from_env("OCTIC_ROW_INPLACE")
+
+
+class OwnedStreamGrad:
+    __slots__ = ("task", "ptr", "numel", "storage", "armed")
+
+    def __init__(self):
+        self.task, self.ptr, self.numel, self.storage, self.armed = -1, 0, 0, None, -1
+
+    def clear(self):
+        self.task, self.ptr, self.numel, self.storage = -1, 0, 0, None
+
+    def offer(self, dx):
+        if dx is None or not (ROW_INPLACE and ROW_SKIP_DROPPED and ops._in_backward()):
+            return
+        task = torch._C._current_graph_task_id()
+        self.task, self.ptr, self.numel, self.storage = task, dx.data_ptr(), dx.numel(), dx.untyped_storage()
+        if self.armed != task:
+            self.armed = task
+            torch.autograd.Variable._execution_engine.queue_callback(self.clear)
+
+    def take(self, g):
+        st, ptr, numel, task = self.storage, self.ptr, self.numel, self.task
+        if st is None:
+            return False
+        self.clear()
+        return (ROW_INPLACE and ROW_SKIP_DROPPED and ops._in_backward() and task == torch._C._current_graph_task_id()
+                and g.dtype == torch.float32 and g.is_contiguous() and g.data_ptr() == ptr and g.numel() == numel
+                and g.untyped_storage().data_ptr() == st.data_ptr())
+
+
+STREAM_GRADS = OwnedStreamGrad()
 
 
 class AttnPackedFn(torch.autograd.Function):
@@ -961,7 +998,8 @@
     br = _gemm_fwd(tag, a2, wb, b, cache, tag, tokens, ds, rps, drop)
     if neps is not None:
         nw32, nb32 = _f32(nw), _f32(nb)
-        out, yn, stats = ops.dense_resid_layernorm_fwd(x2, br, g32, rs32, rps, nw32, nb32, neps, torch.bfloat16)
+        out, yn, stats = ops.dense_resid_layernorm_fwd(x2, br, g32, rs32, rps, nw32, nb32, neps, torch.bfloat16,
+                                                       skip_yb=ROW_INPLACE and ROW_SKIP_DROPPED)
         ctx.set_materialize_grads(False)
         yn = yn.view(x.shape)
         row_skip_attach(ctx, yn)
@@ -986,9 +1024,11 @@
             g2 = _c(gyn).view(out.shape)
             if LN_TAIL_FUSED and ops.dense_ln_bwd_tail_ok(g2, br, out.shape[-1]):
                 ns, nrps = row_skip_get(ctx, g2.shape[0])
+                mine = dres is not None and STREAM_GRADS.take(dres)
                 gout, dnw, dnb, gbr, dgamma, colsum = ops.dense_layernorm_bwd_tail(
                     g2, out, nw32, stats, dres, br, g32, rs32, rps, want_param_grads=want, want_gamma=has_gamma,
-                    want_colsum=has_b, sample_scale=ns, rows_per_sample=nrps)
+                    want_colsum=has_b, sample_scale=ns, rows_per_sample=nrps, inplace=mine and ns is not None)
+                STREAM_GRADS.offer(gout)
             else:
                 gout, dnw, dnb = ops.dense_layernorm_bwd(g2, out, nw32, stats, dres, want_param_grads=want)
             dnw, dnb = (dnw if has_nw else None), (dnb if has_nb else None)
diff --git a/octic_vits_amd/ops.py b/octic_vits_amd/ops.py
--- a/octic_vits_amd/ops.py
+++ b/octic_vits_amd/ops.py
@@ -255,19 +255,30 @@
     return g.dtype == torch.bfloat16 and x.dtype == torch.float32 and c % 32 == 0 and c <= 160
 
 
-def layernorm_bwd_cast(g, x, stats, alpha5, dres, c, rs, rps, want_param_grads=True, sample_scale=None, rows_per_sample=0):
+def layernorm_bwd_cast(g, x, stats, alpha5, dres, c, rs, rps, want_param_grads=True, sample_scale=None, rows_per_sample=0,
+                       inplace=False):
     M = x.numel() // (8 * c)
     ss, srps = _sample_scale(sample_scale, rows_per_sample, M, x, "layernorm_bwd_cast")
-    dx = torch.empty_like(x)
+    if inplace:
+        if ss is None or dres is None or dres.dtype != torch.float32 or not dres.is_contiguous() or dres.numel() != x.numel():
+            raise ValueError("layernorm_bwd_cast(inplace=True) needs a sample mask and a contiguous float32 dres of x's size")
+        dx = dres
+    else:
+        dx = torch.empty_like(x)
     gc = torch.empty(x.shape, dtype=torch.bfloat16, device=x.device)
     nblk = lib().octic_layernorm_d8_bwd_blocks(M)
     partials = torch.empty((nblk, 2, 8 * c), dtype=torch.float32, device=x.device)
     gv, xv, dv = pview(g, c), pview(x, c), pview(dx, c)
     rv = pview(dres, c) if dres is not None else None
     t = KERNEL_TIMER.start()
-    check(lib().octic_layernorm_d8_bwd_cast_skip(ctypes.byref(gv), ctypes.byref(xv), _p(stats), _arr5(alpha5),
-                                                 ctypes.byref(rv) if rv is not None else None, ctypes.byref(dv), _p(partials),
-                                                 M, c, _p(rs), int(rps), _p(gc), _p(ss), srps, _stream(x)))
+    if inplace:
+        check(lib().octic_layernorm_d8_bwd_cast_inplace(ctypes.byref(gv), ctypes.byref(xv), _p(stats), _arr5(alpha5),
+                                                        ctypes.byref(dv), _p(partials), M, c, _p(rs), int(rps), _p(gc), _p(ss),
+                                                        srps, _stream(x)))
+    else:
+        check(lib().octic_layernorm_d8_bwd_cast_skip(ctypes.byref(gv), ctypes.byref(xv), _p(stats), _arr5(alpha5),
+                                                     ctypes.byref(rv) if rv is not None else None, ctypes.byref(dv),
+                                                     _p(partials), M, c, _p(rs), int(rps), _p(gc), _p(ss), srps, _stream(x)))
     KERNEL_TIMER.stop(t, "ln_bwd_kernel<bf16>", M * 8 * c * (2 + 8 + (4 if dres is not None else 0) + 2))
     if not want_param_grads or alpha5 is None:
         return dx, None, None, gc
@@ -860,7 +871,7 @@
     return dw, db
 
 
-def dense_resid_layernorm_fwd(x, yb, gamma, rs, rps, w, b, eps, out_dtype):
+def dense_resid_layernorm_fwd(x, yb, gamma, rs, rps, w, b, eps, out_dtype, skip_yb=False):
     _require_cuda(x)
     d = x.shape[-1]
     rows = x.numel() // d
@@ -868,8 +879,9 @@
     y = torch.empty(x.shape, dtype=out_dtype, device=x.device)
     stats = torch.empty((rows, 2), dtype=torch.float32, device=x.device)
     t = KERNEL_TIMER.start()
-    check(lib().octic_dense_resid_layernorm_fwd(_p(x), _p(yb), dt_code(yb.dtype), _p(gamma), _p(rs), int(rps), _p(xout), _p(y),
-                                                dt_code(out_dtype), _p(w), _p(b), _p(stats), rows, d, float(eps), _stream(x)))
+    fn = lib().octic_dense_resid_layernorm_fwd_skip if (skip_yb and rs is not None) else lib().octic_dense_resid_layernorm_fwd
+    check(fn(_p(x), _p(yb), dt_code(yb.dtype), _p(gamma), _p(rs), int(rps), _p(xout), _p(y), dt_code(out_dtype), _p(w), _p(b),
+             _p(stats), rows, d, float(eps), _stream(x)))
     KERNEL_TIMER.stop(t, f"dense_resid_ln_fwd_kernel<{_DTN[out_dtype]}>", rows * d * (8 + yb.element_size() + y.element_size()))
     return xout, y, stats
 
@@ -898,19 +910,29 @@
 
 
 def dense_layernorm_bwd_tail(gy, x, w, stats, dres, yb, gamma, rs, rps, want_param_grads=True, want_gamma=True,
-                             want_colsum=True, sample_scale=None, rows_per_sample=0):
+                             want_colsum=True, sample_scale=None, rows_per_sample=0, inplace=False):
     d = x.shape[-1]
     rows = x.numel() // d
     ss, srps = _sample_scale(sample_scale, rows_per_sample, rows, x, "dense_layernorm_bwd_tail")
-    dx = torch.empty_like(x)
+    if inplace:
+        if ss is None or dres is None or dres.dtype != torch.float32 or not dres.is_contiguous() or dres.numel() != x.numel():
+            raise ValueError("dense_layernorm_bwd_tail(inplace=True) needs a sample mask and a contiguous float32 dres of x's size")
+        dx = dres
+    else:
+        dx = torch.empty_like(x)
     gyb = torch.empty(x.shape, dtype=yb.dtype, device=x.device)
     nblk = lib().octic_dense_blocks(rows)
     p1 = torch.empty((nblk, 2, d), dtype=torch.float32, device=x.device) if want_param_grads else None
     want2 = want_gamma or want_colsum
     p2 = torch.empty((nblk, 2, d), dtype=torch.float32, device=x.device) if want2 else None
     t = KERNEL_TIMER.start()
-    check(lib().octic_dense_layernorm_bwd_tail_skip(_p(gy), _p(x), _p(w), _p(stats), _p(dres), _p(dx), _p(p1), _p(yb), _p(gamma),
-                                                    _p(rs), int(rps), _p(gyb), _p(p2), rows, d, _p(ss), srps, _stream(x)))
+    if inplace:
+        check(lib().octic_dense_layernorm_bwd_tail_inplace(_p(gy), _p(x), _p(w), _p(stats), _p(dx), _p(p1), _p(yb), _p(gamma),
+                                                           _p(rs), int(rps), _p(gyb), _p(p2), rows, d, _p(ss), srps, _stream(x)))
+    else:
+        check(lib().octic_dense_layernorm_bwd_tail_skip(_p(gy), _p(x), _p(w), _p(stats), _p(dres), _p(dx), _p(p1), _p(yb),
+                                                        _p(gamma), _p(rs), int(rps), _p(gyb), _p(p2), rows, d, _p(ss), srps,
+                                                        _stream(x)))
     KERNEL_TIMER.stop(t, "dense_ln_bwd_tail_kernel<bf16>", rows * d * (2 + 8 + (4 if dres is not None else 0) + 4))
     dw = db = dgamma = colsum = None
     if want_param_grads:
```
